# adam-kerrigan/pybader

Measured on AMD Instinct MI355X. Metric: Mvoxels/s neargrid assign+refine on 512^3 grid, higher is better.
Workload: dtype f64; 1 GPU; 512^3 synthetic 8-Gaussian-atom cubic cell (BASELINE config 3), neargrid assign + neargrid edge refinement changed:2, density resident in HBM; method=neargrid, device_driven_slab_step=False, basins=8

## Files before the change

### include/bader_hip.h

```cpp
#ifndef BADER_HIP_H
#define BADER_HIP_H

#include <stdint.h>

#ifdef __cplusplus
extern "C" {
#endif

typedef struct xb_ctx xb_ctx;

enum { XB_OK = 0, XB_E_ARG = -1, XB_E_HIP = -2, XB_E_STATE = -3, XB_E_LIMIT = -4, XB_E_COMM = -5,
       XB_E_SHORT = -6  };

enum { XB_I8 = 1, XB_I16 = 2, XB_I32 = 4, XB_I64 = 8 };

enum { XB_METHOD_ONGRID = 0, XB_METHOD_NEARGRID = 1 };
enum { XB_REFINE_ALL = 0, XB_REFINE_CHANGED = 1 };

const char *xb_last_error(void);
int xb_device_count(void);
int xb_create(int device, xb_ctx **out);
void xb_destroy(xb_ctx *c);
int xb_sync(xb_ctx *c);
void *xb_stream(xb_ctx *c);
// ... 55 lines not shown
int xb_walkers_fetch(xb_ctx *c, int64_t *walkers, int64_t *results);
int xb_walkers_continue(xb_ctx *c, const int64_t *walkers, int64_t n);
int xb_walkers_apply(xb_ctx *c, const int64_t *results, int64_t n, int64_t *changed, int64_t *stuck);
int xb_edge_check(xb_ctx *c, int64_t *checked, int64_t *edges);
int xb_edge_check_local(xb_ctx *c, int64_t *n_out);
int xb_edge_check_local_fetch(xb_ctx *c, int64_t *idx_out, int8_t *cls_out);
int xb_edge_check_global(xb_ctx *c, const int64_t *idx, const int8_t *cls, int64_t n, int64_t *checked, int64_t *edges);
int xb_refine(xb_ctx *c, int mode, int64_t iters, int64_t *log, int64_t log_capacity, int64_t *n_iters);
int xb_assign_refine(xb_ctx *c, int method, int mode, int64_t iters, int64_t *n_maxima, int64_t *log, int64_t log_capacity, int64_t *n_iters);

int xb_charge_sum(xb_ctx *c, double voxel_volume, int64_t n_labels, double *charge, double *volume);
int xb_moment_sum(xb_ctx *c, const double lattice[9], const double *centres_cart, int64_t n, double voxel_volume,
                  double *moments , double *volume );
int xb_adjacency(xb_ctx *c, const int32_t *dirs , int n_dirs, int64_t n, int64_t *n_pairs);
int xb_adjacency_fetch(xb_ctx *c, int32_t *a, int32_t *b, int64_t *facets , double *saddle,
                       int64_t *saddle_facet, int64_t capacity);
int xb_adjacency_release(xb_ctx *c);
int xb_weight_sum(xb_ctx *c, const double alpha[27], double voxel_volume, const double *q_host, int64_t *n_maxima);
int xb_weight_sum_device(xb_ctx *c, const double alpha[27], double voxel_volume, const void *dev_ptr, int dtype,
                         const int64_t stride[3], void *stream, int64_t *n_maxima);
int xb_weight_fetch(xb_ctx *c, int64_t *max_idx, double *charge, double *volume, int64_t capacity);
int xb_weight_stats(xb_ctx *c, int64_t out[7]);
int xb_weight_release(xb_ctx *c);
int xb_volume_assign(xb_ctx *c, const int64_t *swap, int64_t n_swap);
int xb_atom_assign(const double *bader_max_cart, int64_t n_max, const double *atoms_cart, int64_t n_atoms,
                   const double lattice[9], int64_t *atom_out, double *dist_out);

int xb_surface_distance(xb_ctx *c, const double lattice[9], const double *atoms_cart, int64_t n_atoms,
                        double *min_d2, int64_t *edges);
int xb_volume_mask(xb_ctx *c, int64_t vol_num, double *out_host);
int xb_label_sum(xb_ctx *c, int64_t value, double *sum, int64_t *count);

int xb_set_table_window(xb_ctx *c, int64_t margin);
int xb_table_build(xb_ctx *c, int64_t *n_local_seeds);
int xb_table_local_seeds(xb_ctx *c, int64_t *out, int64_t capacity);
int xb_brick_masks(xb_ctx *c, void **dev_ptr, int64_t *n_bricks, int64_t *own_first, int64_t *own_count);
int xb_table_ties(xb_ctx *c, int64_t *has_ties);
int xb_table_finish(xb_ctx *c, const int64_t *seeds, int64_t n_seeds, int64_t any_ties);

void *xb_labels_ptr(xb_ctx *c);
void *xb_known_ptr(xb_ctx *c);
void *xb_density_ptr(xb_ctx *c);
int64_t xb_plane_elems(xb_ctx *c);
int xb_copy_planes(xb_ctx *c, int which , int to_device, void *host, int64_t xa, int64_t xb);
int xb_label_wire(xb_ctx *c, int widen_to, int *wire_out);
int xb_brick_masks_copy(xb_ctx *c, int to_device, int32_t *host, int64_t first, int64_t count);
int xb_set_halo(xb_ctx *c, int64_t halo);

int xb_slab_supported(xb_ctx *c, int nranks, int64_t *ok);
int xb_slab_assign_masks(xb_ctx *c, int rank, int nranks);
int xb_slab_assign_trace(xb_ctx *c);
int xb_slab_assign_finish(xb_ctx *c, int64_t *n_maxima, int64_t *status);
int xb_slab_refine_pass(xb_ctx *c);
int xb_slab_walkers_round(xb_ctx *c, int src, int last);
int xb_slab_walk_layout(xb_ctx *c, int64_t out[5]);
int xb_slab_walk_send(xb_ctx *c, int64_t walkers);
enum {
    XB_XC_EDGES = 0,
    XB_XC_CHANGED = 1,
    XB_XC_ESCAPED = 2,
    XB_XC_TRAVELLING = 3,
    XB_XC_SLOW = 4,
    XB_XC_LOST = 5,
    XB_XC_MINE = 6,
    XB_XC_ROUNDS = 7,
    XB_XC_COUNT = 8
};
int xb_slab_refine_counts(xb_ctx *c, int64_t *local, int64_t *global);
int xb_slab_block(xb_ctx *c, int which, void **dev_ptr, int64_t *bytes_total, int64_t *own_offset, int64_t *own_bytes);
int xb_slab_block_copy(xb_ctx *c, int which, int to_device, void *host, int64_t off, int64_t bytes);
int xb_host_waits(int64_t *n);

int xb_kernel_time(xb_ctx *c, int which, double *ms_total, int64_t *launches);
int xb_kernel_time_reset(xb_ctx *c);
int xb_enable_timing(xb_ctx *c, int on);
int xb_set_option(xb_ctx *c, int key, int value);
int xb_host_alloc(int64_t bytes, void **out);
int xb_host_free(void *p);
int xb_memory_stats(xb_ctx *c, int64_t *bytes_total, int64_t *bytes_table, int64_t *bytes_scratch);
int xb_box_stats(xb_ctx *c, int64_t *n_boxes, int64_t *box_voxels);
int xb_brick_labels(xb_ctx *c, int32_t *out, int64_t capacity, int64_t dims[3]);
int xb_slow_path_stats(xb_ctx *c, int64_t *assign_total, int64_t *refine_total);
int xb_deferred_stats(xb_ctx *c, int64_t *refine_total);
int xb_growth_stats(xb_ctx *c, int64_t *retries, int64_t *kill_launches);

int xb_comm_unique_id(uint8_t id_out[128]);
int xb_comm_init(xb_ctx *c, int rank, int nranks, const uint8_t id_in[128]);
int xb_comm_destroy(xb_ctx *c);
int xb_comm_exchange_planes(xb_ctx *c, int which, int n_send, const int32_t *send_peer, const int64_t *send_xa,
                            const int64_t *send_xb, int n_recv, const int32_t *recv_peer, const int64_t *recv_xa,
                            const int64_t *recv_xb);
int xb_comm_allreduce_i64(xb_ctx *c, int64_t *inout, int64_t n, int op);
int xb_comm_allgather_i64(xb_ctx *c, const int64_t *in, int64_t n, int64_t *out);
int xb_comm_share_brick_masks(xb_ctx *c, const int64_t *first, const int64_t *count);
int xb_comm_allgather_block(xb_ctx *c, int which, const int64_t *first, const int64_t *count);
int xb_comm_allreduce_block(xb_ctx *c);
int xb_comm_info(xb_ctx *c, int64_t out[4]);
int xb_comm_stats(xb_ctx *c, int64_t *bytes_sent);

#ifdef __cplusplus
}
#endif
#endif
```

### pybader_amd/_lib.py

```python
import ctypes as C
import threading
import os

import numpy as np

HERE = os.path.dirname(os.path.abspath(__file__))
LIB_PATH = os.environ.get('XB_LIBRARY') or os.path.join(HERE, 'libbader_hip.so')

METHODS = {'ongrid': 0, 'neargrid': 1}
REFINE_MODES = {'all': 0, 'changed': 1}
DTYPE_CODE = {np.dtype(np.int8): 1, np.dtype(np.int16): 2, np.dtype(np.int32): 4, np.dtype(np.int64): 8}
(XB_XC_EDGES, XB_XC_CHANGED, XB_XC_ESCAPED, XB_XC_TRAVELLING, XB_XC_SLOW, XB_XC_LOST, XB_XC_MINE, XB_XC_ROUNDS,
 XB_XC_COUNT) = range(9)

_vp, _i64, _dbl, _int = C.c_void_p, C.c_int64, C.c_double, C.c_int
_pi64, _pdbl = C.POINTER(C.c_int64), C.POINTER(C.c_double)
SYMBOLS = {
    'xb_last_error': (C.c_char_p, []),
    'xb_device_count': (_int, []),
    'xb_create': (_int, [_int, C.POINTER(_vp)]),
    'xb_destroy': (None, [_vp]),
    'xb_sync': (_int, [_vp]),
    'xb_stream': (_vp, [_vp]),
    'xb_set_grid': (_int, [_vp, _pi64, _pdbl, _pdbl, _i64, _i64]),
# ... 2 lines not shown
    'xb_parse_density_text': (_int, [_vp, _vp, _i64, _dbl, _pi64, _pi64]),
    'xb_parse_cube_text': (_int, [_vp, _vp, _i64, _i64, _i64, _int, _dbl, _pi64, _pi64]),
    'xb_download_density': (_int, [_vp, _vp]),
    'xb_format_begin': (_int, [_vp, _vp, _pi64, _int, _dbl, _int, _int, _vp, _i64, _i64, _pi64]),
    'xb_format_host_values': (_int, [_vp, _vp, _vp]),
    'xb_format_set_host_text': (_int, [_vp, _vp, _vp]),
    'xb_format_next': (_int, [_vp, C.POINTER(_vp), _pi64]),
    'xb_format_times': (_int, [_vp, _pdbl, _pdbl]),
    'xb_format_end': (_int, [_vp]),
    'xb_upload_labels': (_int, [_vp, _vp, _int]),
    'xb_download_labels': (_int, [_vp, _vp, _int]),
    'xb_import_density': (_int, [_vp, _vp, _int, _pi64, _vp]),
    'xb_import_labels': (_int, [_vp, _vp, _int, _vp]),
    'xb_export_labels': (_int, [_vp, _vp, _int, _vp]),
    'xb_export_volume': (_int, [_vp, _i64, _vp, _int, _vp]),
    'xb_device_alloc': (_int, [_int, _i64, C.POINTER(_vp)]),
    'xb_device_free': (_int, [_vp]),
    'xb_device_read': (_int, [_vp, _vp, _vp, _i64, _vp]),
    'xb_upload_known': (_int, [_vp, _vp]),
    'xb_download_known': (_int, [_vp, _vp]),
    'xb_vacuum_assign': (_int, [_vp, _dbl, _dbl, _pdbl, _pdbl]),
    'xb_assign': (_int, [_vp, _int, _pi64]),
    'xb_get_maxima': (_int, [_vp, _vp, _i64]),
    'xb_assign_trace': (_int, [_vp, _int, _pi64]),
    'xb_assign_local_table': (_int, [_vp, _vp, _vp, _i64]),
    'xb_assign_finish': (_int, [_vp, _vp, _i64]),
    'xb_prepare_refine': (_int, [_vp]),
    'xb_edge_find': (_int, [_vp, _pi64]),
    'xb_refine_trace': (_int, [_vp, _pi64, _pi64]),
    'xb_refine_trace_escaped': (_int, [_vp, _pi64, _pi64]),
    'xb_escaped_paths': (_int, [_vp, _i64, _pi64, _pi64]),
    'xb_escaped_paths_fetch': (_int, [_vp, _vp, _vp, _vp, _vp]),
    'xb_gather_voxels': (_int, [_vp, _vp, _i64, _vp, _vp]),
    'xb_scatter_voxels': (_int, [_vp, _vp, _i64, _vp, _vp]),
    'xb_walkers_count': (_int, [_vp, _pi64, _pi64]),
    'xb_walkers_fetch': (_int, [_vp, _vp, _vp]),
    'xb_walkers_continue': (_int, [_vp, _vp, _i64]),
    'xb_walkers_apply': (_int, [_vp, _vp, _i64, _pi64, _pi64]),
    'xb_edge_check': (_int, [_vp, _pi64, _pi64]),
    'xb_edge_check_local': (_int, [_vp, _pi64]),
    'xb_edge_check_local_fetch': (_int, [_vp, _vp, _vp]),
    'xb_edge_check_global': (_int, [_vp, _vp, _vp, _i64, _pi64, _pi64]),
    'xb_refine': (_int, [_vp, _int, _i64, _vp, _i64, _pi64]),
    'xb_assign_refine': (_int, [_vp, _int, _int, _i64, _pi64, _vp, _i64, _pi64]),
    'xb_charge_sum': (_int, [_vp, _dbl, _i64, _vp, _vp]),
    'xb_moment_sum': (_int, [_vp, _pdbl, _pdbl, _i64, _dbl, _pdbl, _pdbl]),
    'xb_adjacency': (_int, [_vp, _vp, _int, _i64, _pi64]),
    'xb_adjacency_fetch': (_int, [_vp, _vp, _vp, _vp, _vp, _vp, _i64]),
    'xb_adjacency_release': (_int, [_vp]),
    'xb_weight_sum': (_int, [_vp, _pdbl, _dbl, _vp, _pi64]),
    'xb_weight_sum_device': (_int, [_vp, _pdbl, _dbl, _vp, _int, _pi64, _vp, _pi64]),
    'xb_weight_fetch': (_int, [_vp, _vp, _vp, _vp, _i64]),
    'xb_weight_stats': (_int, [_vp, _pi64]),
    'xb_weight_release': (_int, [_vp]),
    'xb_volume_assign': (_int, [_vp, _vp, _i64]),
    'xb_atom_assign': (_int, [_vp, _i64, _vp, _i64, _vp, _vp, _vp]),
    'xb_surface_distance': (_int, [_vp, _vp, _vp, _i64, _vp, _pi64]),
    'xb_volume_mask': (_int, [_vp, _i64, _vp]),
    'xb_label_sum': (_int, [_vp, _i64, _pdbl, _pi64]),
    'xb_set_table_window': (_int, [_vp, _i64]),
    'xb_table_build': (_int, [_vp, _pi64]),
    'xb_table_local_seeds': (_int, [_vp, _vp, _i64]),
    'xb_brick_masks': (_int, [_vp, C.POINTER(_vp), _pi64, _pi64, _pi64]),
    'xb_table_ties': (_int, [_vp, _pi64]),
    'xb_table_finish': (_int, [_vp, _vp, _i64, _i64]),
    'xb_labels_ptr': (_vp, [_vp]),
    'xb_known_ptr': (_vp, [_vp]),
    'xb_density_ptr': (_vp, [_vp]),
    'xb_plane_elems': (_i64, [_vp]),
    'xb_copy_planes': (_int, [_vp, _int, _int, _vp, _i64, _i64]),
    'xb_label_wire': (_int, [_vp, _int, _vp]),
    'xb_host_alloc': (_int, [_i64, _vp]),
    'xb_host_free': (_int, [_vp]),
    'xb_brick_masks_copy': (_int, [_vp, _int, _vp, _i64, _i64]),
    'xb_set_halo': (_int, [_vp, _i64]),
    'xb_kernel_time': (_int, [_vp, _int, _pdbl, _pi64]),
    'xb_kernel_time_reset': (_int, [_vp]),
    'xb_enable_timing': (_int, [_vp, _int]),
    'xb_set_option': (_int, [_vp, _int, _int]),
    'xb_box_stats': (_int, [_vp, _pi64, _pi64]),
    'xb_brick_labels': (_int, [_vp, _vp, _i64, _pi64]),
    'xb_slow_path_stats': (_int, [_vp, _pi64, _pi64]),
    'xb_deferred_stats': (_int, [_vp, _pi64]),
    'xb_growth_stats': (_int, [_vp, _pi64, _pi64]),
    'xb_comm_unique_id': (_int, [_vp]),
    'xb_comm_init': (_int, [_vp, _int, _int, _vp]),
    'xb_comm_destroy': (_int, [_vp]),
    'xb_comm_exchange_planes': (_int, [_vp, _int, _int, _vp, _pi64, _pi64, _int, _vp, _pi64, _pi64]),
    'xb_comm_allreduce_i64': (_int, [_vp, _pi64, C.c_int64, _int]),
    'xb_comm_allgather_i64': (_int, [_vp, _pi64, C.c_int64, _pi64]),
    'xb_comm_share_brick_masks': (_int, [_vp, _pi64, _pi64]),
    'xb_comm_allgather_block': (_int, [_vp, _int, _pi64, _pi64]),
    'xb_comm_allreduce_block': (_int, [_vp]),
    'xb_slab_supported': (_int, [_vp, _int, _pi64]),
    'xb_slab_assign_masks': (_int, [_vp, _int, _int]),
    'xb_slab_assign_trace': (_int, [_vp]),
    'xb_slab_assign_finish': (_int, [_vp, _pi64, _pi64]),
    'xb_slab_refine_pass': (_int, [_vp]),
    'xb_slab_walkers_round': (_int, [_vp, _int, _int]),
    'xb_slab_walk_layout': (_int, [_vp, _pi64]),
    'xb_slab_walk_send': (_int, [_vp, _i64]),
    'xb_slab_refine_counts': (_int, [_vp, _pi64, _pi64]),
    'xb_slab_block': (_int, [_vp, _int, C.POINTER(_vp), _pi64, _pi64, _pi64]),
    'xb_slab_block_copy': (_int, [_vp, _int, _int, _vp, _i64, _i64]),
    'xb_host_waits': (_int, [_pi64]),
    'xb_comm_stats': (_int, [_vp, _pi64]),
    'xb_comm_info': (_int, [_vp, _pi64]),
    'xb_memory_stats': (_int, [_vp, _pi64, _pi64, _pi64]),
}

_lib = None


class BaderHipError(RuntimeError):
    code = None


XB_E_ARG = -1
XB_E_STATE = -3
XB_E_LIMIT = -4
XB_E_SHORT = -6


def load():
    global _lib
    if _lib is None:
        if not os.path.exists(LIB_PATH):
            raise BaderHipError(f"{LIB_PATH} is missing: build it with `python -m pybader_amd.build` "
                                "(hipcc, gfx950); pybader_amd has no CPU fallback")
        lib = C.CDLL(LIB_PATH)
        for name, (res, args) in SYMBOLS.items():
            fn = getattr(lib, name)
            fn.restype = res
            fn.argtypes = args
        _lib = lib
    return _lib


_POOL_KEEP = 4
_POOL_MAX_BYTES = 4 << 30


class _PinnedBuf:
    __slots__ = ('ptr', 'nbytes', '__weakref__')

    def __init__(self, ptr, nbytes):
        self.ptr, self.nbytes = ptr, nbytes

    @property
    def __array_interface__(self):
        return {'shape': (self.nbytes,), 'typestr': '|u1', 'data': (self.ptr, False), 'version': 3}


_pool = {}
_pool_bytes = 0
_pool_lock = threading.Lock()


def _host_free(ptr):
    if _lib is not None:
        _lib.xb_host_free(C.c_void_p(ptr))


def _pool_evict(need):
    global _pool_bytes
    for size in list(_pool):
# ... 658 lines not shown
    def slab_refine_counts(self):
        loc, glo = np.zeros(XB_XC_COUNT, np.int64), np.zeros(XB_XC_COUNT, np.int64)
        check(self.lib.xb_slab_refine_counts(self.h, loc.ctypes.data_as(_pi64), glo.ctypes.data_as(_pi64)))
        return loc, glo

    def slab_block(self, which):
        p, a, b, d = _vp(), C.c_int64(0), C.c_int64(0), C.c_int64(0)
        check(self.lib.xb_slab_block(self.h, int(which), C.byref(p), C.byref(a), C.byref(b), C.byref(d)))
        return int(p.value or 0), int(a.value), int(b.value), int(d.value)

    def slab_block_copy(self, which, host, off, to_device):
        assert host.dtype == np.uint8 and host.flags.c_contiguous
        check(self.lib.xb_slab_block_copy(self.h, int(which), 1 if to_device else 0, _ptr(host), int(off), host.nbytes))

    def comm_allgather_block(self, which, first, count):
        f, n = np.array(first, np.int64), np.array(count, np.int64)
        check(self.lib.xb_comm_allgather_block(self.h, int(which), f.ctypes.data_as(_pi64), n.ctypes.data_as(_pi64)))

    def comm_allreduce_block(self):
        check(self.lib.xb_comm_allreduce_block(self.h))

    def host_waits(self):
        a = C.c_int64(0)
        check(self.lib.xb_host_waits(C.byref(a)))
        return int(a.value)

    def memory_stats(self):
        a, b, d = C.c_int64(0), C.c_int64(0), C.c_int64(0)
        check(self.lib.xb_memory_stats(self.h, C.byref(a), C.byref(b), C.byref(d)))
        return int(a.value), int(b.value), int(d.value)

    def comm_info(self):
        out = (C.c_int64 * 4)()
        check(self.lib.xb_comm_info(self.h, out))
        return {'nccl_comm_count': int(out[0]), 'nccl_user_rank': int(out[1]), 'nccl_device': int(out[2]), 'rccl_version': int(out[3])}

    def comm_bytes_sent(self):
        n = C.c_int64(0)
        check(self.lib.xb_comm_stats(self.h, C.byref(n)))
        return int(n.value)

    def enable_timing(self, on=True, only=None):
        mask = int(bool(on)) if only is None else sum(2 << int(k) for k in only)
        check(self.lib.xb_enable_timing(self.h, mask))

    def kernel_time(self, which):
        ms, n = C.c_double(), C.c_int64()
        check(self.lib.xb_kernel_time(self.h, int(which), C.byref(ms), C.byref(n)))
        return ms.value, n.value

    def kernel_time_reset(self):
        check(self.lib.xb_kernel_time_reset(self.h))

    def set_option(self, key, value):
        check(self.lib.xb_set_option(self.h, int(key), int(value)))

    def box_stats(self):
        a, b = C.c_int64(), C.c_int64()
        check(self.lib.xb_box_stats(self.h, C.byref(a), C.byref(b)))
        return a.value, b.value

    def brick_labels(self):
        dims = (C.c_int64 * 3)()
        check(self.lib.xb_brick_labels(self.h, None, 0, dims))
        out = np.zeros(tuple(int(d) for d in dims), np.int32)
        check(self.lib.xb_brick_labels(self.h, _ptr(out), out.size, dims))
        return out

    def slow_path_stats(self):
        a, b = C.c_int64(), C.c_int64()
        check(self.lib.xb_slow_path_stats(self.h, C.byref(a), C.byref(b)))
        return a.value, b.value

    def growth_stats(self):
        a, b = C.c_int64(), C.c_int64()
        check(self.lib.xb_growth_stats(self.h, C.byref(a), C.byref(b)))
        return a.value, b.value

    def deferred_stats(self):
        a = C.c_int64()
        check(self.lib.xb_deferred_stats(self.h, C.byref(a)))
        return a.value

    def sync(self):
        check(self.lib.xb_sync(self.h))


def atom_assign(bader_max_cart, atoms_cart, lattice):
    lib = load()
    bm, at, lat = _f64(bader_max_cart).reshape(-1, 3), _f64(atoms_cart).reshape(-1, 3), _f64(lattice).reshape(9)
    a, d = np.zeros(bm.shape[0], np.int64), np.zeros(bm.shape[0], np.float64)
    check(lib.xb_atom_assign(_ptr(bm), bm.shape[0], _ptr(at), at.shape[0], _ptr(lat), _ptr(a), _ptr(d)))
    return a, d


_default_ctx = {}


def default_context(device=None):
    if device is None:
        device = int(os.environ.get('PYBADER_AMD_DEVICE', os.environ.get('LOCAL_RANK', '0')))
        if load().xb_device_count() == 1:
            device = 0
    if device not in _default_ctx:
        _default_ctx[device] = Context(device)
    return _default_ctx[device]
```

### pybader_amd/csrc/bader_hip.hip

```cpp
#include "bader_kernels.h"
#include "../../include/bader_hip.h"

#include <algorithm>
#include <cmath>
#include <cstdarg>
#include <cstdio>
#include <cstring>
#include <string>
#include <thread>
#include <vector>

static thread_local long long xb_waits = 0;
static inline hipError_t xb_counted_sync(hipStream_t s) { xb_waits++; return (hipStreamSynchronize)(s); }
#define hipStreamSynchronize(s) xb_counted_sync(s)

#include "k_common.h"
#include "k_masks.h"
#include "k_fused.h"
#include "k_trace.h"
#include "k_ongrid.h"
#include "k_edges.h"
#include "k_sums.h"
#include "k_text.h"
#include "k_format.h"
// ... 25 lines not shown
    long long launches = 0;
};

namespace xbcomm { struct State; }
struct xb_ctx {
    int device = 0;
    xbcomm::State *comm = nullptr;
    struct FmtState *fmt = nullptr;
    hipStream_t stream = nullptr;
    Grid g{};
    bool has_grid = false;
    long long N = 0;
    int halo = 0;
    double *rho = nullptr;
    GradRec *grad = nullptr;
    long long grad_cap = 0;
    long long list_cap = 0;
    int *ec_buf = nullptr;
    long long ec_buf_cap = 0;
    double *dist_dev = nullptr;
    int *boxbuf = nullptr;
    int *box_max_tab = nullptr;
    int n_boxes = 0;
    long long box_voxels = 0;
    int opt_boxes = 1;
    int opt_bricks = 1;
    int opt_dbg = 0;
    int opt_ec_groups = 256;
    int opt_ec_share = 1;
    int *ec_share = nullptr;
    int opt_ec_qcap = EC_Q;
    std::vector<int64_t> esc_starts, esc_offsets, esc_vox;
    unsigned long long *ec_pend = nullptr;
    int8_t *ec_pflag = nullptr;
    std::vector<int8_t> esc_complete;
    bool has_vacuum = true;
    bool vac_by_tol = false;
    double vac_tol = 0.;
    bool regions_pending = false;
    bool buni_valid = false;
    bool buni_halo_safe = false;
    bool regions_neargrid = false;
    bool regions_labels = false;
    int n_walk = 0;
    int *walk = nullptr;
    int table_margin = -1;
    bool table_prebuilt = false;
    int table_stage = 0;
    std::vector<int> window_seeds;
    bool window_ties = true;
    bool slab_sparse = false;
    int ec_local_n = 0;
    int walk_n_out = 0;
    void *walk_out_dev = nullptr;
    std::vector<int64_t> walk_host, res_host;
    int walk_n_res = 0;
    void *walk_in = nullptr, *walk_out2 = nullptr, *walk_res = nullptr;
    long long walk_cap = 0;
    long long stat_deferred = 0;
    long long stat_ovf_assign = 0, stat_ovf_refine = 0;
    int *bres_last = nullptr;
    int *blab = nullptr;
    int nbk[3] = {0, 0, 0};
    bool grad_valid = false;
    bool brick_max_valid = false;
    int grad_cover = 0;
    unsigned char *brick_rec = nullptr;
    void *xbuf = nullptr;
    int slab_rank = 0, slab_nranks = 0, slab_stage = 0;
    void *wbuf[2] = {nullptr, nullptr};
    void *wk_in = nullptr;
    int wbuf_ranks = 0, walk_last = -1, walk_round = 0, wcap = 0;
    int walk_send = 0;
    int opt_async_comm = 0;
    int opt_tile_dilate = 1;
    int opt_self_exchange = 0;
    int opt_mask_diag = 1;
    int opt_narrow_halo = 1;
    int grow_kill_launches = 6;
    long long stat_grow_retries = 0;
    bool defer_wait = false;
    bool pending_assign = false;
    int64_t pending_n_maxima = 0;
    int opt_lean = 1;
    int opt_mirror = 1;
    int grad_rule = 0;
    int *labels = nullptr;
    int8_t *known = nullptr;
    int *first = nullptr;
    int *list = nullptr;
    int8_t *st = nullptr;
    void *stage = nullptr;
    size_t stage_bytes = 0;
    int *max_list = nullptr;
    int *max_aux = nullptr;
    int max_cap = 0;
    int *ovf_list = nullptr;
    int ovf_cap = 0;
    int *counters = nullptr;
    int *fs = nullptr;
    int *blab_buf = nullptr;
    long long blab_alloc = 0;
    bool labels_zero_pending = false;
    int zero_outside[3] = {-1, -1, -1};
    static constexpr int trace_waves = 8192;
    unsigned long long *counters64 = nullptr;
    double *dsum = nullptr;
    int *host_ints = nullptr;
    char *big_pin[2] = {nullptr, nullptr};
    hipEvent_t big_ev[2] = {nullptr, nullptr};
    hipEvent_t io_ev = nullptr;
    int opt_io_tiled = 1;
    char *pin = nullptr;
    size_t pin_bytes = 0;
    std::vector<int> maxima_sorted;
    int label_wire = 4;
    std::vector<int> local_max, local_first;
    bool first_clean = false;
    int chg_n = -1;
    int list_n = 0;
    bool list_valid = false;
    unsigned timing = 0;
    TimedKernel tk[10];
    long long n_alloc = 0;
    bool thin = false;
    double *w_A = nullptr, *w_V = nullptr, *w_S = nullptr;
    unsigned char *w_pending = nullptr;
    int *w_list[2] = {nullptr, nullptr};
    int *w_state = nullptr;
    long long w_cap = 0;
    long long w_stat[6] = {0, 0, 0, 0, 0, 0};
    bool w_have = false;
    bool w_ignore_labels = false;
    std::vector<int64_t> w_idx;
    std::vector<double> w_charge, w_volume;
    double *m_buf = nullptr;
    size_t m_cap = 0;
    unsigned long long *aj_buf = nullptr;
    size_t aj_bytes = 0;
    bool aj_have = false;
    int aj_dirs = 0;
    std::vector<int32_t> aj_a, aj_b;
    std::vector<int64_t> aj_facets, aj_sfacet;
    std::vector<double> aj_saddle;
    bool have_rho = false, have_labels = false;
};

static inline int label_wire_for(long long n) { return 2 * n <= 255 ? 1 : (2 * n <= 65535 ? 2 : 4); }
static inline int labels_fit_wire(const int32_t *lab, long long n) {
    int32_t lo = 0, hi = 0;
    for (long long i = 0; i < n; i++) { lo = std::min(lo, lab[i]); hi = std::max(hi, lab[i]); }
    return (lo >= -128 && hi <= 127) ? 1 : ((lo >= -32768 && hi <= 32767) ? 2 : 4);
}
static inline unsigned nblocks(long long n) { return (unsigned)((n + TPB - 1) / TPB); }
static GridL light(const Grid &g) {
    GridL l;
    l.nx = g.nx; l.ny = g.ny; l.nz = g.nz; l.nyz = g.nyz;
    l.x0 = g.x0; l.x1 = g.x1; l.vx0 = g.vx0; l.vlen = g.vlen;
    l.wx0 = g.wx0; l.wlen = g.wlen; l.wbase = g.wbase; l.ntot = g.ntot;
    l.use24 = ((long long)g.nx * g.ny < (1 << 24)) && g.nz < (1 << 24);
    l.main_ties = g.main_ties;
    return l;
}

template <typename T>
struct DevBuf {
// ... 11 lines not shown
    s.main_ties = g.main_ties;
    for (int k = 0; k < 9; k++) s.T[k] = g.T[k];
    auto at = [&](int idx) {
        const int ix = idx / 9, iy = (idx / 3) % 3, iz = idx % 3;
        return g.dist[((ix + 2) % 3) * 9 + ((iy + 2) % 3) * 3 + ((iz + 2) % 3)];
    };
    for (int idx = 0; idx <= 13; idx++) {
        const double a = at(idx), b = at(26 - idx);
        if (std::memcmp(&a, &b, sizeof a) != 0) return false;
        s.dsym[idx] = a;
    }
    return true;
}

static void mirror_prefilter(const Grid &g, int &mirror, double &mu_scale) {
    mirror = 0;
    double dmin = 0.;
    bool first = true;
    for (int i = 0; i < 27; i++)
        if (i != 0) { dmin = first ? g.dist[i] : std::min(dmin, g.dist[i]); first = false; }
    if (!(dmin > 0.) || !std::isfinite(dmin)) { mu_scale = 0.; return; }
    for (int ax = 0; ax < 3; ax++) {
        bool ok = true;
        for (int u = 0; u < 3 && ok; u++)
            for (int v = 0; v < 3 && ok; v++) {
                int ip[3], im[3];
                ip[ax] = 1; im[ax] = 2;
                ip[(ax + 1) % 3] = im[(ax + 1) % 3] = u;
                ip[(ax + 2) % 3] = im[(ax + 2) % 3] = v;
                const double a = g.dist[ip[0] * 9 + ip[1] * 3 + ip[2]], b = g.dist[im[0] * 9 + im[1] * 3 + im[2]];
                ok = std::memcmp(&a, &b, sizeof a) == 0;
            }
        if (ok) mirror |= 1 << ax;
    }
    mu_scale = std::ldexp(1. + 1. / dmin, -48);
}

struct ScopedTimer {
    xb_ctx *c;
    int which;
    hipEvent_t a = nullptr, b = nullptr;
    ScopedTimer(xb_ctx *c_, int w) : c(c_), which(w) {
        if ((c->timing >> which) & 1u) {
            hipEventCreate(&a);
            hipEventCreate(&b);
            hipEventRecord(a, c->stream);
        }
    }
    ~ScopedTimer() {
        if ((c->timing >> which) & 1u) {
            hipEventRecord(b, c->stream);
            c->tk[which].pending.push_back({a, b});
        }
    }
};

extern "C" {

const char *xb_last_error(void) { return g_err.c_str(); }

#include "host_context.h"
#include "host_stages.h"
#include "host_format.h"
#include "host_assign.h"
#include "host_refine.h"
#include "host_sums.h"
#include "host_slab_table.h"
#include "host_interop.h"
#include "host_weight.h"
#include "host_moments.h"
#include "host_adjacency.h"

int xb_set_option(xb_ctx *c, int key, int value) {
    if (!c) return fail(XB_E_ARG, "null ctx");
    if (key == 1) { c->opt_boxes = value & 1; c->opt_bricks = (value >> 1) & 1; }
    else if (key == 2) {
        c->opt_mirror = !(value & 1);
        c->opt_lean = !(value & 2);
        c->opt_mask_diag = !(value & 4);
        c->opt_tile_dilate = !(value & 8);
        c->opt_narrow_halo = !(value & 16);
        c->opt_ec_share = !(value & 32);
        c->opt_io_tiled = !(value & 64);
    }
    else if (key == 3) c->opt_dbg = value;
    else if (key == 4 && value >= 1 && value <= 4096) c->opt_ec_groups = value;
    else if (key == 5 && value >= 2 && value <= EC_Q) c->opt_ec_qcap = value;
    else if (key == 6) { c->grad_valid = false; if (value == 2) c->brick_max_valid = false; }
    else if (key == 17 && value >= 1) c->grow_kill_launches = value;
    else if (key == 19) c->opt_self_exchange = value != 0;
    else if (key == 24) c->opt_async_comm = value != 0;
    else if (key == 30) c->w_ignore_labels = value != 0;
    else return fail(XB_E_ARG, "xb_set_option: unknown key %d", key);
    return XB_OK;
}
int xb_growth_stats(xb_ctx *c, int64_t *retries, int64_t *kill_launches) {
    if (!c) return fail(XB_E_ARG, "null ctx");
    if (retries) *retries = c->stat_grow_retries;
    if (kill_launches) *kill_launches = c->grow_kill_launches;
    return XB_OK;
}
int xb_deferred_stats(xb_ctx *c, int64_t *refine_total) {
    if (!c) return fail(XB_E_ARG, "null ctx");
    if (refine_total) *refine_total = c->stat_deferred;
    return XB_OK;
}
int xb_slow_path_stats(xb_ctx *c, int64_t *assign_total, int64_t *refine_total) {
    if (!c) return fail(XB_E_ARG, "null ctx");
    if (assign_total) *assign_total = c->stat_ovf_assign;
    if (refine_total) *refine_total = c->stat_ovf_refine;
    return XB_OK;
}
int xb_memory_stats(xb_ctx *c, int64_t *bytes_total, int64_t *bytes_table, int64_t *bytes_scratch) {
    if (!c || !c->has_grid) return fail(XB_E_STATE, "xb_memory_stats: no grid");
    const long long N = c->N;
    const long long table = c->grad_cap * (long long)sizeof(GradRec);
    const long long scratch = c->list_cap * 4 + (long long)c->stage_bytes + c->ec_buf_cap * 4 + (c->ec_pend ? 8 * N + 16 : 0) +
                              (c->w_cap ? 25 * c->w_cap + (c->w_S ? 8 * c->w_cap : 0) : 0)  +
                              (long long)c->m_cap * 8  +
                              (long long)c->aj_bytes ;
    const long long fixed = 8 * N  + 4 * N  + (N + 16)  + 4 * N  + N  +
                            2LL * c->max_cap * 4 + (long long)c->ovf_cap * 4 + c->blab_alloc * 5 + (long long)c->walk_cap * 3 * 80 +
                            (1 << 22) ;
    if (bytes_total) *bytes_total = fixed + table + scratch;
    if (bytes_table) *bytes_table = table;
    if (bytes_scratch) *bytes_scratch = scratch;
    return XB_OK;
}
int xb_box_stats(xb_ctx *c, int64_t *n_boxes, int64_t *box_voxels) {
    if (!c) return fail(XB_E_ARG, "null ctx");
    if (n_boxes) *n_boxes = c->n_boxes;
    if (box_voxels) *box_voxels = c->box_voxels;
    return XB_OK;
}
int xb_brick_labels(xb_ctx *c, int32_t *out, int64_t capacity, int64_t dims[3]) {
    if (!c || !c->has_grid) return fail(XB_E_STATE, "xb_brick_labels: no grid");
    if (!c->blab) return fail(XB_E_STATE, "xb_brick_labels: no trapping regions on this context (no neargrid assignment yet)");
    const int64_t nbr = (int64_t)c->nbk[0] * c->nbk[1] * c->nbk[2];
    if (dims) { dims[0] = c->nbk[0]; dims[1] = c->nbk[1]; dims[2] = c->nbk[2]; }
    if (!out) return XB_OK;
    if (capacity < nbr) return fail(XB_E_ARG, "xb_brick_labels: capacity too small");
    HIPCHK(hipSetDevice(c->device));
    HIPCHK(hipMemcpyAsync(out, c->blab, nbr * sizeof(int), hipMemcpyDeviceToHost, c->stream));
    HIPCHK(hipStreamSynchronize(c->stream));
    return XB_OK;
}
#ifdef XB_DEBUG_COUNT
int xb_debug_steps(xb_ctx *c, int on, signed char *host_out) {
    static signed char *buf = nullptr;
    if (host_out && buf) {
        if (hipMemcpy(host_out, buf, (size_t)c->N, hipMemcpyDeviceToHost) != hipSuccess) return XB_E_HIP;
    }
    if (on && !buf && hipMalloc(&buf, (size_t)c->N) != hipSuccess) return XB_E_HIP;
    if (on && hipMemset(buf, 0, (size_t)c->N) != hipSuccess) return XB_E_HIP;
    signed char *p = on ? buf : nullptr;
    return hipMemcpyToSymbol(HIP_SYMBOL(xb_dbg_steps), &p, sizeof p) == hipSuccess ? XB_OK : XB_E_HIP;
}
int xb_debug_counts(unsigned long long *out, int reset) {
    hipDeviceSynchronize();
    if (out && hipMemcpyFromSymbol(out, HIP_SYMBOL(xb_dbg), sizeof(unsigned long long) * 65536) != hipSuccess) return XB_E_HIP;
    if (reset) {
        static unsigned long long z[65536];
        if (hipMemcpyToSymbol(HIP_SYMBOL(xb_dbg), z, sizeof z) != hipSuccess) return XB_E_HIP;
    }
    return XB_OK;
}
#endif
int xb_enable_timing(xb_ctx *c, int on) {
    if (!c) return fail(XB_E_ARG, "null ctx");
    c->timing = on == 0 ? 0u : (on == 1 ? 0xFFFFu : ((unsigned)on >> 1));
    return XB_OK;
}
int xb_kernel_time_reset(xb_ctx *c) {
    if (!c) return fail(XB_E_ARG, "null ctx");
    HIPCHK(hipSetDevice(c->device));
    HIPCHK(hipStreamSynchronize(c->stream));
    for (auto &t : c->tk) {
        for (auto &p : t.pending) { hipEventDestroy(p.first); hipEventDestroy(p.second); }
        t.pending.clear();
        t.ms = 0.;
        t.launches = 0;
    }
    return XB_OK;
}
int xb_kernel_time(xb_ctx *c, int which, double *ms_total, int64_t *launches) {
    if (!c || which < 0 || which > 9) return fail(XB_E_ARG, "xb_kernel_time: bad argument");
    HIPCHK(hipSetDevice(c->device));
// ... 21 lines not shown
```

### pybader_amd/csrc/host_assign.h

```cpp

static GridL light(const Grid &g);

static int ensure_brick_bytes(xb_ctx *c, int nbr) {
    if (c->blab_alloc < nbr) {
        hipFree(c->blab_buf); c->blab_buf = nullptr; c->blab_alloc = 0; c->brick_rec = nullptr; c->brick_max_valid = false;
        if (c->grad_cover) { c->grad_cover = 0; c->grad_valid = false; }
        HIPCHK(hipMalloc(&c->blab_buf, (size_t)nbr * sizeof(int) + (size_t)nbr + 16));
        c->blab_alloc = nbr;
        c->brick_rec = reinterpret_cast<unsigned char *>(c->blab_buf + nbr);
    }
    return XB_OK;
}

static int ensure_grad(xb_ctx *c, bool force, bool boxes, bool main_rule) {
    if (int rc = need_grad(c)) return rc;
    c->g.main_ties = main_rule ? 1 : 0;
    if (c->grad_valid && !force && (c->grad_rule == 2 || c->grad_rule == (main_rule ? 1 : 0))) return XB_OK;
    const Grid &g = c->g;
    if (c->grad_valid && !force && !boxes && c->grad_cover == 1 && c->brick_rec) {
        const int nb1r = (g.ny + BRK - 1) / BRK, nb2r = (g.nz + BRK - 1) / BRK, nbr = ((g.nx + BRK - 1) / BRK) * nb1r * nb2r;
        ScopedTimer t(c, 4);
        launch_brick_records(c, nullptr, nullptr, nbr, nb1r, nb2r);
        HIPCHK(hipGetLastError());
        c->grad_rule = main_rule ? 1 : 0;
// ... 331 lines not shown
    c->buni_valid = false; c->regions_labels = false;
    const bool regions = c->regions_pending && c->blab;
    int buni = BUNI_NONE;
    if (regions && g.x1 - g.x0 == g.nx)
        buni = BUNI_SCAN;
    else if (regions && !c->has_vacuum && g.nx % 8 == 0 && g.ny % 8 == 0 && g.nz % 8 == 0 && g.x0 % 8 == 0 && g.x1 % 8 == 0)
        buni = BUNI_MIXED;
    launch_relabel(c, nullptr, (int)n_global, regions, c->box_max_tab ? c->box_max_tab : c->boxbuf + BB_REGMAX, buni, nullptr);
    HIPCHK(hipGetLastError());
    if (buni != BUNI_NONE) {
        c->buni_valid = true;
        c->buni_halo_safe = buni == BUNI_MIXED;
    }
    c->regions_labels = regions && !c->has_vacuum && c->regions_neargrid;
    c->regions_pending = false;
    HIPCHK(hipStreamSynchronize(c->stream));
    c->first_clean = true;
    return XB_OK;
}


static bool fused_ok(const xb_ctx *c) {
    const Grid &g = c->g;
    return c->opt_boxes && c->opt_bricks && g.x0 == 0 && g.x1 == g.nx && !table_windowed(c) &&
           g.nx >= 16 && g.ny >= 16 && g.nz >= 16;
}
static int assign_neargrid_tail(xb_ctx *c, int64_t *n_maxima);

static int fused_numbering_launch(xb_ctx *c) {
    k_number_maxima<<<1, 1024, 0, c->stream>>>(c->fs, c->first, c->max_list, c->max_cap, c->max_aux, c->fs + FS_TOTAL);
    launch_relabel(c, c->fs, 0, c->regions_pending, c->box_max_tab, BUNI_SCAN, c->bres_last);
    HIPCHK(hipGetLastError());
    return XB_OK;
}
static int number_maxima_big(xb_ctx *c, int nmax) {
    const long long n_words = (c->N + 31) / 32, n_blocks = (n_words + 1023) / 1024;
    const size_t need = (size_t)(2 * n_words + n_blocks) * sizeof(int);
    DevBuf<int> own;
    int *scratch = (int *)c->stage;
    if (!c->stage || c->stage_bytes < need) {
        HIPCHK(own.alloc((size_t)(2 * n_words + n_blocks)));
        scratch = own.p;
    }
    unsigned *bits = reinterpret_cast<unsigned *>(scratch);
    int *wprefix = scratch + n_words, *bsum = scratch + 2 * n_words;
    HIPCHK(hipMemsetAsync(bits, 0, (size_t)n_words * sizeof(int), c->stream));
    k_rank_mark<<<(nmax + 255) / 256, 256, 0, c->stream>>>(c->first, c->max_list, nmax, bits);
    k_rank_scan<<<(unsigned)n_blocks, 1024, 0, c->stream>>>(bits, (int)n_words, wprefix, bsum);
    k_rank_blocks<<<1, 1024, 0, c->stream>>>(bsum, (int)n_blocks);
    k_rank_assign<<<(nmax + 255) / 256, 256, 0, c->stream>>>(c->first, c->max_list, nmax, bits, wprefix, bsum, c->max_aux, c->fs);
    HIPCHK(hipGetLastError());
    launch_relabel(c, c->fs, 0, c->regions_pending, c->box_max_tab, BUNI_SCAN, c->bres_last);
    HIPCHK(hipGetLastError());
    c->maxima_sorted.resize(nmax);
    HIPCHK(hipMemcpyAsync(c->maxima_sorted.data(), c->max_aux, (size_t)nmax * sizeof(int), hipMemcpyDeviceToHost, c->stream));
    HIPCHK(hipStreamSynchronize(c->stream));
    return XB_OK;
}

static int assign_neargrid_fused(xb_ctx *c, int64_t *n_maxima) {
    if (int rc = need_grad(c)) return rc;
    Grid &g = c->g;
    const int nb0 = (g.nx + BRK - 1) / BRK, nb1 = (g.ny + BRK - 1) / BRK, nb2 = (g.nz + BRK - 1) / BRK, nbr = nb0 * nb1 * nb2;
    const bool part = g.nx % BRK || g.ny % BRK || g.nz % BRK;
    if (int rc = ensure_brick_bytes(c, nbr)) return rc;
    int *fs = c->fs;
    int *seed = c->list, *bmask = c->list + nbr, *buf0 = c->list + 2 * nbr, *buf1 = c->list + 3 * nbr, *walk = c->list + 4 * nbr;
    int *box_max = c->boxbuf + BB_REGMAX, *box_first = c->boxbuf + BB_REGFIRST;
    int *bmaxv = walk;
    int *bpot = c->list + 5 * nbr;
    int *bres = nullptr;
    c->box_max_tab = box_max;
    auto stage_done = [&](const char *what) {
        if (c->opt_dbg & 32) {
            const hipError_t e = (hipStreamSynchronize)(c->stream);
            int h16[16] = {0};
            (void)hipMemcpy(h16, fs, sizeof h16, hipMemcpyDeviceToHost);
            fprintf(stderr, "[assign] %s: %s  seeds %d regions %d certain %d walk %d maxima %d ovf %d err %d\n", what, hipGetErrorString(e), h16[FS_N_SEEDS],
                    h16[FS_N_BOXES], h16[FS_N_CERTAIN], h16[FS_N_WALK], h16[FS_N_MAX], h16[FS_N_OVF], h16[FS_ERR]);
            fflush(stderr);
        }
    };
    if (int rc = begin_assignment(c, fs, FS_TOTAL, true)) return rc;
    g.main_ties = 1;
    const GridL gl = light(g);
    {
        ScopedTimer t4(c, 4);
        {
            ScopedTimer t5(c, 5);
            launch_brick_masks(c, part, true, bmask, bmaxv, bpot);
        }
        stage_done("brick masks");
        c->grad_valid = true;
        c->grad_rule = 1;
        c->grad_cover = 1;
        launch_region_growth(c, nb0, nb1, nb2, bmask, bmaxv, bpot, seed, buf0, buf1, box_max, box_first, true);
        HIPCHK(hipGetLastError());
        stage_done("region growth");
    }
    c->blab = c->blab_buf;
    c->regions_neargrid = true;
    c->walk = walk;
    c->nbk[0] = nb0; c->nbk[1] = nb1; c->nbk[2] = nb2;
    const long long own = c->N;
    {
        ScopedTimer t0(c, 0);
        {
            int bits = 0;
            while ((1 << bits) < std::max(std::max(nb0, nb1), nb2)) bits++;
            const unsigned n_codes = 1u << (3 * bits);
            const bool vac = c->has_vacuum && c->vac_by_tol;
            k_brick_walk_list_morton<<<(n_codes + 16 * TPB - 1) / (16 * TPB), TPB, 0, c->stream>>>(nb0, nb1, nb2, n_codes, c->blab, walk,
                                                                                                  fs + FS_N_WALK, fs + FS_GROW_RETRY,
                                                                                                  vac ? bpot : nullptr, c->vac_tol);
        }
        {
            ScopedTimer t7(c, 7);
            launch_brick_records(c, walk, fs + FS_N_WALK, nbr, nb1, nb2);
        }
        stage_done("walk list + records");
        if (c->has_vacuum)
            k_fill_certain<<<nblocks(own), TPB, 0, c->stream>>>(gl, c->blab, nb1, nb2, box_max, c->labels, c->first, c->max_list,
                                                                fs + FS_N_MAX, c->max_cap, fs + FS_GROW_RETRY);
        else {
            k_note_regions<<<1, XB_BOXES_MAX, 0, c->stream>>>(gl, nb1, nb2, fs, box_first, box_max, c->first, c->max_list, fs + FS_N_MAX, c->max_cap);
            c->regions_pending = true;
        }
        {
            ScopedTimer t6(c, 6);
            int *bres_buf = c->has_vacuum ? nullptr : c->list + 6 * nbr;
            if (launch_persistent_trace(c, true, part, box_max, walk, c->has_vacuum ? 1 : 0, bres_buf)) bres = bres_buf;
        }
        HIPCHK(hipGetLastError());
        stage_done("trace");
    }
    c->bres_last = bres;
    if (int rc = fused_numbering_launch(c)) return rc;
    stage_done("numbering + relabel");
    HIPCHK(hipMemcpyAsync(c->host_ints, fs, (FS_TOTAL + XB_SORT_MAX) * sizeof(int), hipMemcpyDeviceToHost, c->stream));
    if (c->defer_wait) {
        g.main_ties = 0;
        c->grad_rule = 2;
        c->regions_pending = false;
        c->buni_valid = !c->has_vacuum;
        c->regions_labels = !c->has_vacuum;
        c->pending_assign = true;
        return XB_OK;
    }
    HIPCHK(hipStreamSynchronize(c->stream));
    return assign_neargrid_tail(c, n_maxima);
}

static int assign_neargrid_tail(xb_ctx *c, int64_t *n_maxima) {
    Grid &g = c->g;
    int *fs = c->fs;
    const int nb1 = c->nbk[1], nb2 = c->nbk[2];
    int *walk = c->walk, *box_max = c->box_max_tab;
    const int *h = c->host_ints;
    g.main_ties = 0;
    const GridL gl = light(g);
    if (h[FS_GROW_RETRY]) {
        c->grow_kill_launches = 1 << 20;
        c->stat_grow_retries++;
        c->grad_valid = false;
        return assign_neargrid_fused(c, n_maxima);
    }
    if (h[FS_TIES] == 0) c->grad_rule = 2;
    c->n_boxes = h[FS_N_BOXES];
    c->box_voxels = (long long)h[FS_N_CERTAIN] * BRK * BRK * BRK;
    c->n_walk = h[FS_N_WALK];
    const int novf = h[FS_N_OVF];
    int nmax = h[FS_N_MAX];
    if (nmax > c->max_cap) return fail(XB_E_LIMIT, "%d maxima exceed the table capacity %d", nmax, c->max_cap);
    c->stat_ovf_assign += novf;
    const int *sorted = h[FS_SORT_OK] && novf == 0 ? h + FS_TOTAL : nullptr;
    if (novf > 0) {
        g.main_ties = 1;
        const GridL glt = light(g);
        const int maxsteps = trace_maxsteps(g);
        int *list2 = (int *)c->stage;
        const int cap2 = (int)std::min<size_t>(c->stage_bytes / sizeof(int), 0x7fffffffu);
        auto two_tiers = [&](int n_listed) -> int {
            c->host_ints[HI_UPLOAD] = n_listed;
            HIPCHK(hipMemcpyAsync(c->counters + CT_MID_LISTED, c->host_ints + HI_UPLOAD, sizeof(int), hipMemcpyHostToDevice, c->stream));
            HIPCHK(hipMemsetAsync(c->counters + CT_MID_LEFT, 0, sizeof(int), c->stream));
            k_ng_trace_list<XB_MID_K><<<512, TPB, 0, c->stream>>>(glt, c->grad, box_max, c->blab, nb1, nb2, c->ovf_list, c->counters + CT_MID_LISTED, c->labels, c->first,
                                                          c->max_list, fs + FS_N_MAX, c->max_cap, list2, c->counters + CT_MID_LEFT, cap2, maxsteps, c->rho, c->dist_dev,
                                                          c->has_vacuum ? 1 : 0);
            HIPCHK(hipGetLastError());
            if (c->opt_dbg & 4) {
                int m2 = 0;
                if (int rc2 = read_counter(c, CT_MID_LEFT, &m2)) return rc2;
                fprintf(stderr, "[assign] %d walkers listed, %d left for the exact slow kernel after the %d-voxel window\n", n_listed, m2, XB_MID_K);
            }
            if (n_listed > cap2) return fail(XB_E_LIMIT, "%d walkers for the exact slow path exceed its list (%d)", n_listed, cap2);
            return run_slow(c, n_listed, 0, fs + FS_N_MAX, nullptr, nullptr, list2, c->counters + CT_MID_LEFT, true);
        };
        int rc = two_tiers(std::min(novf, c->ovf_cap));
        for (int left = novf - c->ovf_cap; !rc && left > 0;) {
            HIPCHK(hipMemsetAsync(c->counters + CT_N_OVF, 0, sizeof(int), c->stream));
            k_list_unfinished<<<4096, TPB, 0, c->stream>>>(gl, walk, fs + FS_N_WALK, nb1, nb2, c->labels, c->ovf_list, c->counters + CT_N_OVF, c->ovf_cap);
            HIPCHK(hipGetLastError());
            int m = 0;
            if ((rc = read_counter(c, CT_N_OVF, &m))) break;
            if (m == 0) break;
            rc = two_tiers(std::min(m, c->ovf_cap));
            left = m - c->ovf_cap;
        }
        g.main_ties = 0;
        if (rc) return rc;
        HIPCHK(hipMemsetAsync(fs + FS_N_OVF, 0, sizeof(int), c->stream));
        if (int rc2 = fused_numbering_launch(c)) return rc2;
        HIPCHK(hipMemcpyAsync(c->host_ints, fs, (FS_TOTAL + XB_SORT_MAX) * sizeof(int), hipMemcpyDeviceToHost, c->stream));
        HIPCHK(hipStreamSynchronize(c->stream));
        nmax = h[FS_N_MAX];
        if (nmax > c->max_cap) return fail(XB_E_LIMIT, "%d maxima exceed the table capacity %d", nmax, c->max_cap);
        if (h[FS_SORT_OK]) sorted = h + FS_TOTAL;
    }
    if (!sorted) {
        if (int rc = number_maxima_big(c, nmax)) return rc;
    }
    numbering_done(c, sorted, nmax, n_maxima);
    c->buni_valid = !c->has_vacuum;
    c->regions_labels = !c->has_vacuum;
    return XB_OK;
}


static bool assign_neargrid_complete(xb_ctx *c, int64_t *n_maxima) {
    c->pending_assign = false;
    const int *h = c->host_ints;
    const int nmax = h[FS_N_MAX];
    if (h[FS_GROW_RETRY] || h[FS_TIES] != 0 || h[FS_N_OVF] != 0 || !h[FS_SORT_OK] || nmax > c->max_cap || nmax > XB_SORT_MAX) return false;
    c->n_boxes = h[FS_N_BOXES];
    c->box_voxels = (long long)h[FS_N_CERTAIN] * BRK * BRK * BRK;
    c->n_walk = h[FS_N_WALK];
    numbering_done(c, h + FS_TOTAL, nmax, n_maxima);
// ... 131 lines not shown
```

### pybader_amd/csrc/host_context.h

```cpp

int xb_device_count(void) {
    int n = 0;
    if (hipGetDeviceCount(&n) != hipSuccess) return 0;
    return n;
}

int xb_create(int device, xb_ctx **out) {
    if (!out) return fail(XB_E_ARG, "xb_create: null out");
    int n = 0;
    hipError_t e = hipGetDeviceCount(&n);
    if (e != hipSuccess || n <= 0)
        return fail(XB_E_HIP, "xb_create: no HIP device visible (%s); libbader_hip has no CPU fallback",
                    e == hipSuccess ? "device count 0" : hipGetErrorString(e));
    if (device < 0 || device >= n) return fail(XB_E_ARG, "xb_create: device %d out of range [0,%d)", device, n);
    HIPCHK(hipSetDevice(device));
    xb_ctx *c = new xb_ctx();
    c->device = device;
    HIPCHK(hipStreamCreate(&c->stream));
    HIPCHK(hipMalloc(&c->counters, (1024 + XB_SORT_MAX) * sizeof(int)));
    c->fs = c->counters + CT_FS;
    HIPCHK(hipMalloc(&c->counters64, 16 * sizeof(unsigned long long)));
    HIPCHK(hipMalloc(&c->dsum, 16 * sizeof(double)));
    HIPCHK(hipMalloc(&c->dist_dev, 36 * sizeof(double)));
    HIPCHK(hipMalloc(&c->boxbuf, (size_t)(1 << 20) * sizeof(int)));
    HIPCHK(hipHostMalloc(&c->host_ints, HI_TOTAL * sizeof(int)));
    *out = c;
    return XB_OK;
}

static void weight_free(xb_ctx *c);
static void moments_free(xb_ctx *c);
static void adjacency_free(xb_ctx *c);
static void free_grid(xb_ctx *c) {
    weight_free(c);
    moments_free(c);
    adjacency_free(c);
    c->have_rho = c->have_labels = false;
    hipFree(c->rho); hipFree(c->grad); hipFree(c->labels); hipFree(c->known); hipFree(c->first); hipFree(c->list);
    hipFree(c->st); hipFree(c->stage); hipFree(c->ec_pend); c->ec_pend = nullptr; hipFree(c->ec_share); c->ec_share = nullptr; hipFree(c->ec_pflag); c->ec_pflag = nullptr; hipFree(c->max_list); hipFree(c->max_aux); hipFree(c->ovf_list);
    hipFree(c->blab_buf); c->blab_buf = nullptr; c->blab_alloc = 0; c->labels_zero_pending = false;
    hipFree(c->ec_buf); c->ec_buf = nullptr; c->ec_buf_cap = 0; c->grad_cap = 0; c->list_cap = 0;
    c->brick_rec = nullptr; c->grad_cover = 0;
    c->rho = nullptr; c->grad = nullptr; c->grad_valid = false; c->brick_max_valid = false; c->labels = nullptr; c->known = nullptr; c->first = nullptr; c->list = nullptr;
    c->st = nullptr; c->stage = nullptr; c->max_list = nullptr; c->max_aux = nullptr; c->ovf_list = nullptr;
    c->n_alloc = 0; c->stage_bytes = 0;
}

int xb_comm_destroy(xb_ctx *c);
static void fmt_release(xb_ctx *c);
void xb_destroy(xb_ctx *c) {
    if (!c) return;
    hipSetDevice(c->device);
    hipStreamSynchronize(c->stream);
    xb_comm_destroy(c);
    fmt_release(c);
    for (auto &t : c->tk)
        for (auto &p : t.pending) { hipEventDestroy(p.first); hipEventDestroy(p.second); }
    free_grid(c);
    hipFree(c->counters); hipFree(c->counters64); hipFree(c->dsum); hipFree(c->dist_dev); hipFree(c->boxbuf);
    hipFree(c->walk_in); hipFree(c->walk_out2); hipFree(c->walk_res); hipFree(c->xbuf); hipFree(c->wbuf[0]); hipFree(c->wbuf[1]); hipFree(c->wk_in);
    hipHostFree(c->host_ints);
    hipHostFree(c->pin);
    for (int k = 0; k < 2; k++) { hipHostFree(c->big_pin[k]); if (c->big_ev[k]) hipEventDestroy(c->big_ev[k]); }
    if (c->io_ev) hipEventDestroy(c->io_ev);
    hipStreamDestroy(c->stream);
    delete c;
}

int xb_sync(xb_ctx *c) {
    HIPCHK(hipSetDevice(c->device));
    HIPCHK(hipStreamSynchronize(c->stream));
    return XB_OK;
}
void *xb_stream(xb_ctx *c) { return (void *)c->stream; }

#define XB_SYNTH_ATOMS_MAX 4096
#define XB_SURFACE_ATOMS_MAX 100000
#define XB_STAGE_FLOOR ((size_t)4 << 20)
static_assert((16 + 5 * (size_t)XB_SYNTH_ATOMS_MAX) * sizeof(double) <= XB_STAGE_FLOOR &&
              (16 + 4 * (size_t)XB_SURFACE_ATOMS_MAX) * sizeof(double) <= XB_STAGE_FLOOR, "stage floor below a documented atom maximum");
static int need_scratch(xb_ctx *c) {
    const Grid &g = c->g;
    const long long N = c->N ? c->N : (long long)g.nx * g.nyz;
    const int own = g.x1 - g.x0;
    long long planes = own + 2LL * (std::max(c->halo, 16) + 16);
    if (own == g.nx || planes >= g.nx) planes = g.nx;
    const long long list_want = planes == g.nx ? N : std::max<long long>(planes * g.nyz, 8 * (N / 512) + 4096);
    const size_t stage_want = planes == g.nx ? std::max<size_t>((size_t)N * 8, XB_STAGE_FLOOR) : std::max<size_t>((size_t)planes * g.nyz * 8, (size_t)64 << 20);
    if (c->list_cap < list_want) {
        HIPCHK(hipStreamSynchronize(c->stream));
        hipFree(c->list); c->list = nullptr; c->list_cap = 0;
        HIPCHK(hipMalloc(&c->list, (size_t)list_want * sizeof(int)));
        c->list_cap = list_want;
        c->list_valid = false; c->chg_n = -1; c->walk = nullptr; c->n_walk = 0;
    }
    if (c->stage_bytes < stage_want) {
        HIPCHK(hipStreamSynchronize(c->stream));
        hipFree(c->stage); c->stage = nullptr; c->stage_bytes = 0;
        HIPCHK(hipMalloc(&c->stage, stage_want));
        c->stage_bytes = stage_want;
    }
    return XB_OK;
// ... 475 lines not shown
```

### pybader_amd/csrc/host_refine.h

```cpp

static void plane_range(const Grid &g, int ext, int &xa, int &np) {
    const int own = g.x1 - g.x0;
    if (own + 2 * ext >= g.nx) { xa = 0; np = g.nx; }
    else { xa = ((g.x0 - ext) % g.nx + g.nx) % g.nx; np = own + 2 * ext; }
}

static int preset_known_planes(xb_ctx *c, int p0, int np) {
    const Grid &g = c->g;
    const int run1 = std::min(np, g.nx - p0);
    HIPCHK(hipMemsetAsync(c->known + (size_t)p0 * g.nyz, 2, (size_t)run1 * g.nyz, c->stream));
    if (np > run1) HIPCHK(hipMemsetAsync(c->known, 2, (size_t)(np - run1) * g.nyz, c->stream));
    return XB_OK;
}
static int *launch_brick_uniformity(xb_ctx *c, const GridL &gl, int b_off, int count, unsigned scan_grid) {
    const Grid &g = c->g;
    const int nb0 = (g.nx + 7) / 8, nb1 = (g.ny + 7) / 8, nb2 = (g.nz + 7) / 8, nbr = nb0 * nb1 * nb2;
    int *buni = reinterpret_cast<int *>(c->st);
    if (!c->buni_valid)
        k_label_uniform_list<<<scan_grid, TPB, 0, c->stream>>>(gl, c->labels, nb1, nb2, nullptr, count, nullptr, nullptr, buni, b_off, nbr);
    k_buni3<<<(nbr + 255) / 256, 256, 0, c->stream>>>(nb0, nb1, nb2, buni, buni + nbr);
    return buni + nbr;
}

static int edge_find_launch(xb_ctx *c, bool *dilate_owned) {
// ... 496 lines not shown
    const int chg_n = c->chg_n;
    c->list_valid = false; c->chg_n = -1;
    c->buni_valid = false;
    if (g.x1 - g.x0 != g.nx) return fail(XB_E_STATE, "xb_edge_check: one slab only; slabs use xb_edge_check_local + xb_edge_check_global");
    int n = 0;
    bool listed = false;
    if (chg_n >= 0) {
        n = chg_n;
        if (n) {
            HIPCHK(hipMemcpyAsync(c->list, (int *)c->stage + c->N, (size_t)n * sizeof(int), hipMemcpyDeviceToDevice, c->stream));
            HIPCHK(hipMemcpyAsync(c->host_ints + HI_EC_CHGLIST, c->fs + FS_N_CHGLIST, sizeof(int), hipMemcpyDeviceToHost, c->stream));
            listed = true;
        }
    } else if (int rc = compact(c, -2, &n)) return rc;
    if (int rc = edge_check_resolve(c, n, nullptr, 0, g.nx, 0, c->N, checked, edges)) return rc;
    if (listed && c->host_ints[HI_EC_CHGLIST] != n) return fail(XB_E_STATE, "xb_edge_check: %d voxels listed for %d relabelled ones", c->host_ints[HI_EC_CHGLIST], n);
    return XB_OK;
}

int xb_edge_check_local(xb_ctx *c, int64_t *n_out) {
    NEED_GRID("xb_edge_check_local");
    c->list_valid = false; c->chg_n = -1;
    int n = 0;
    if (int rc = compact(c, -2, &n)) return rc;
    if (n) {
        k_ec_class<<<nblocks(n), TPB, 0, c->stream>>>(c->g, c->rho, c->labels, c->list, n, c->st);
        HIPCHK(hipGetLastError());
    }
    c->ec_local_n = n;
    if (n_out) *n_out = n;
    return XB_OK;
}
int xb_edge_check_local_fetch(xb_ctx *c, int64_t *idx_out, int8_t *cls_out) {
    NEED_GRID("xb_edge_check_local_fetch");
    const int n = c->ec_local_n;
    if (!n) return XB_OK;
    std::vector<int> tmp(n);
    HIPCHK(hipMemcpyAsync(tmp.data(), c->list, n * sizeof(int), hipMemcpyDeviceToHost, c->stream));
    HIPCHK(hipMemcpyAsync(cls_out, c->st, n, hipMemcpyDeviceToHost, c->stream));
    HIPCHK(hipStreamSynchronize(c->stream));
    for (int i = 0; i < n; i++) idx_out[i] = tmp[i];
    return XB_OK;
}
int xb_edge_check_global(xb_ctx *c, const int64_t *idx, const int8_t *cls, int64_t n, int64_t *checked, int64_t *edges) {
    NEED_GRID("xb_edge_check_global");
    const Grid &g = c->g;
    c->list_valid = false; c->chg_n = -1;
    c->buni_valid = false;
    if (checked) *checked = 0;
    if (edges) *edges = 0;
    if (n < 0 || n > c->N) return fail(XB_E_ARG, "xb_edge_check_global: bad list length");
    if (c->halo < 3 && g.vlen < g.nx) return fail(XB_E_STATE, "xb_edge_check_global: needs a halo of at least 3 planes");
    if (!n) return XB_OK;
    std::vector<int> i32(n);
    for (int64_t k = 0; k < n; k++) {
        if (idx[k] < 0 || idx[k] >= c->N) return fail(XB_E_ARG, "xb_edge_check_global: voxel index out of range");
        i32[k] = (int)idx[k];
    }
    if (g.vlen < g.nx)
        if (int rc = preset_known_planes(c, (g.vx0 + g.vlen) % g.nx, g.nx - g.vlen)) return rc;
    int8_t *dcls = c->st + (c->N - n);
    if (2 * n > c->N || 2 * n > c->list_cap) return fail(XB_E_LIMIT, "xb_edge_check_global: list longer than half the grid / the list buffer");
    if (int rc = upload_pinned(c, c->list, i32.data(), n * sizeof(int))) return rc;
    if (int rc = upload_pinned(c, dcls, cls, n, (n * sizeof(int) + 255) & ~(size_t)255)) return rc;
    k_scatter_byte<<<(unsigned)((n + 255) / 256), 256, 0, c->stream>>>(c->known, c->list, (int)n, (int8_t)-2);
    HIPCHK(hipGetLastError());
    int near_xa = 0, near_np = g.nx;
    if (g.vlen + 4 < g.nx) { near_xa = (g.vx0 - 2 + g.nx) % g.nx; near_np = g.vlen + 4; }
    const int rc = edge_check_resolve(c, (int)n, dcls, near_xa, near_np, (long long)g.x0 * g.nyz, (long long)g.x1 * g.nyz, checked, edges);
    return rc;
}

int xb_prepare_refine(xb_ctx *c) {
    NEED_GRID("xb_prepare_refine");
    return ensure_grad(c, false, false, false);
}

#define XB_STEP_REDO 1000
static int refine_iteration_fused(xb_ctx *c, int64_t *edges, int64_t *changed, bool late_records = false) {
    const Grid &g = c->g;
    int *fs = c->fs;
    c->g.main_ties = 0;
    const GridL gl = light(g);
    static_assert(FS_N_CHGLIST == FS_N_EDGES + 6, "one memset clears the refinement's counters");
    HIPCHK(hipMemsetAsync(fs + FS_N_EDGES, 0, 7 * sizeof(int), c->stream));
    c->chg_n = -1;
    {
        ScopedTimer t(c, 2);
        const int small = small_grid(g);
        int *buni = nullptr;
        int ntiles_listed = 0;
        if (g.nx >= 16 && g.ny >= 16 && g.nz >= 16)
            buni = launch_brick_uniformity(c, gl, 0, ((g.nx + 7) / 8) * ((g.ny + 7) / 8) * ((g.nz + 7) / 8), 4096);
        const unsigned char *brec = (c->grad_valid && c->grad_cover == 1) || late_records ? c->brick_rec : nullptr;
        if (buni) {
            const int ntiles = ((g.nz + ET_Z - 1) / ET_Z) * ((g.ny + ET_Y - 1) / ET_Y) * ((g.nx + ET_X - 1) / ET_X);
            ntiles_listed = ntiles;
            int *tiles = (int *)c->stage;
            HIPCHK(hipMemsetAsync(c->known, 2, (size_t)c->N, c->stream));
            k_edge_tile_list<<<(ntiles + TPB - 1) / TPB, TPB, 0, c->stream>>>(gl, buni, tiles, fs + FS_N_TILES, 0, (g.nx + ET_X - 1) / ET_X,
                                                                              c->pending_assign ? fs : nullptr);
            k_edge_flag_listed<<<std::min(ntiles, 2048), TPB, 0, c->stream>>>(gl, c->rho, c->labels, c->known, c->list, fs + FS_N_EDGES, small,
                                                           c->grad_valid ? c->grad : nullptr, brec, c->has_vacuum ? 0 : 1, tiles, fs + FS_N_TILES);
        } else {
            dim3 grid((g.nz + ET_Z - 1) / ET_Z, (g.ny + ET_Y - 1) / ET_Y, (g.nx + ET_X - 1) / ET_X);
            k_edge_flag_tiled<<<grid, TPB, 0, c->stream>>>(gl, c->rho, c->labels, c->known, 0, g.nx, c->list, fs + FS_N_EDGES, small, buni,
                                                           c->grad_valid ? c->grad : nullptr, brec, c->has_vacuum ? 0 : 1);
        }
        if (buni && c->opt_tile_dilate && g.nz % ET_Z == 0) k_edge_dilate_tiles<<<std::min(ntiles_listed, 4096), TPB, 0, c->stream>>>(gl, c->known, (const int *)c->stage, fs + FS_N_TILES);
        else k_edge_dilate_list<<<nblocks(c->N / 16), TPB, 0, c->stream>>>(gl, c->known, c->list, 0, fs + FS_N_EDGES);
    }
    c->list_valid = false; c->chg_n = -1;
    c->buni_valid = false;
    if (late_records) {
        if (int rc = need_grad(c)) return rc;
        ScopedTimer t(c, 4);
        const int nb0 = (g.nx + 7) / 8, nb1 = (g.ny + 7) / 8, nb2 = (g.nz + 7) / 8, nbr = nb0 * nb1 * nb2;
        unsigned char *band = reinterpret_cast<unsigned char *>(c->blab_buf);
        HIPCHK(hipMemsetAsync(band, 0, (size_t)nbr, c->stream));
        k_flag_band_bricks<<<4096, TPB, 0, c->stream>>>(gl, c->known, (const int *)c->stage, fs + FS_N_TILES, band);
        k_rec_set_bit0<<<(nbr + 255) / 256, 256, 0, c->stream>>>(nbr, c->brick_rec, band);
        launch_brick_records(c, nullptr, nullptr, nbr, nb1, nb2);
        HIPCHK(hipGetLastError());
        c->grad_valid = true;
        c->grad_cover = 1;
        c->grad_rule = 0;
        c->regions_labels = false;
        c->blab = nullptr;
        c->table_stage = 0;
    }
    const unsigned char *brec = c->grad_cover == 1 ? c->brick_rec : nullptr;
    const int regions_ok = c->grad_cover == 1 && c->regions_labels && !c->has_vacuum ? 1 : 0;
    {
        ScopedTimer t(c, 3);
        int *defer = (int *)c->stage;
        WalkerIO wl{};
        constexpr int XB_RT_BLOCK = 128;
        launch_refine_trace<2, false>(c, (unsigned)((c->N / 16 + XB_RT_BLOCK - 1) / XB_RT_BLOCK), XB_RT_BLOCK, c->list, 0, fs + FS_N_EDGES,
                                      fs + FS_CHANGED, fs + FS_ESCAPED, c->ovf_list, fs + FS_R_OVF, c->ovf_cap, brec, defer, fs + FS_R_DEFER,
                                      regions_ok, nullptr, wl);
        if (c->grad_cover == 1 && !regions_ok)
            launch_refine_trace<2, true>(c, 512, TPB, (int *)c->stage, 0, fs + FS_R_DEFER, fs + FS_CHANGED, fs + FS_ESCAPED, c->ovf_list,
                                         fs + FS_R_OVF, c->ovf_cap, c->brick_rec, nullptr, nullptr, 0, nullptr, wl);
    }
    HIPCHK(hipGetLastError());
    int *hr = c->host_ints + HI_REFINE;
    HIPCHK(hipMemcpyAsync(hr, fs + FS_N_EDGES, 7 * sizeof(int), hipMemcpyDeviceToHost, c->stream));
    HIPCHK(hipStreamSynchronize(c->stream));
    if (c->pending_assign && !assign_neargrid_complete(c, &c->pending_n_maxima)) return XB_STEP_REDO;
    *edges = hr[0];
    *changed = hr[1];
    const int novf = hr[3];
    if (novf == 0 && hr[1] > 0 && c->stage_bytes >= 8 * (size_t)c->N && hr[1] <= (int)std::min<long long>(c->N, 0x7fffffffLL)) {
        k_list_changed<<<1024, TPB, 0, c->stream>>>(c->list, fs + FS_N_EDGES, c->known, (int *)c->stage + c->N, fs + FS_N_CHGLIST,
                                                    (int)std::min<long long>(c->N, 0x7fffffffLL), fs + FS_CHANGED);
        HIPCHK(hipGetLastError());
        c->chg_n = hr[1];
    } else if (novf == 0 && hr[1] == 0)
        c->chg_n = 0;
    c->stat_deferred += hr[4];
    if (hr[2]) return fail(XB_E_STATE, "xb_refine: %d traces left the grid", hr[2]);
    if (novf > c->ovf_cap) return fail(XB_E_LIMIT, "%d retraces need the slow path (cap %d)", novf, c->ovf_cap);
    c->stat_ovf_refine += novf;
    if (novf > 0) {
        const int *slow_list = nullptr, *slow_n_dev = nullptr;
        const int n_slow = novf;
        const bool can_defer = c->grad_cover == 1 && !regions_ok;
        if (!can_defer && c->stage_bytes >= sizeof(int) * (size_t)novf) {
            int *list2 = (int *)c->stage;
            HIPCHK(hipMemsetAsync(c->counters + CT_MID_LEFT, 0, sizeof(int), c->stream));
            launch_refine_trace<XB_MID_K, false>(c, nblocks(novf), TPB, c->ovf_list, novf, nullptr, fs + FS_CHANGED, fs + FS_ESCAPED, list2,
                                                 c->counters + CT_MID_LEFT, novf, brec, nullptr, nullptr, regions_ok, nullptr, WalkerIO{});
            HIPCHK(hipGetLastError());
            slow_list = list2;
            slow_n_dev = c->counters + CT_MID_LEFT;
            if (c->opt_dbg & 4) {
                int m2 = 0;
                if (int rc = read_counter(c, CT_MID_LEFT, &m2)) return rc;
                fprintf(stderr, "[refine] %d retraces listed, %d left for the exact slow kernel after the %d-voxel window\n", novf, m2, XB_MID_K);
            }
        }
        if (int rc = run_slow(c, n_slow, 1, nullptr, fs + FS_CHANGED, fs + FS_ESCAPED, slow_list, slow_n_dev, true)) return rc;
        HIPCHK(hipMemcpyAsync(hr, fs + FS_CHANGED, sizeof(int), hipMemcpyDeviceToHost, c->stream));
        HIPCHK(hipStreamSynchronize(c->stream));
        *changed = hr[0];
    }
    return XB_OK;
}

static int refine_impl(xb_ctx *c, int mode, int64_t iters, int64_t *log, int64_t log_capacity, int64_t *n_iters);
int xb_refine(xb_ctx *c, int mode, int64_t iters, int64_t *log, int64_t log_capacity, int64_t *n_iters) {
    const int rc = refine_impl(c, mode, iters, log, log_capacity, n_iters);
    if (c) c->chg_n = -1;
    return rc;
}
static int refine_impl(xb_ctx *c, int mode, int64_t iters, int64_t *log, int64_t log_capacity, int64_t *n_iters) {
    NEED_GRID("xb_refine");
    if (n_iters) *n_iters = 0;
    if (iters == 0) return XB_OK;
    int64_t edges = 0, changed = 0, esc = 0, checked = 0;
    const bool fused = c->g.x0 == 0 && c->g.x1 == c->g.nx && !table_windowed(c);
    const bool late = fused && !c->grad_valid && c->brick_max_valid && !c->has_vacuum && c->brick_rec && c->g.nx >= 16 && c->g.ny >= 16 && c->g.nz >= 16;
    if (!late)
        if (int rc = xb_prepare_refine(c)) return rc;
    int64_t k = 0;
    auto put = [&](int64_t e, int64_t ch) {
        if (log && 2 * k + 1 < log_capacity) { log[2 * k] = e; log[2 * k + 1] = ch; }
        k++;
        if (n_iters) *n_iters = k;
    };
    if (fused) {
        if (int rc = refine_iteration_fused(c, &edges, &changed, late)) return rc;
        if (edges == 0) return XB_OK;
    } else {
        if (int rc = xb_edge_find(c, &edges)) return rc;
        if (edges == 0) return XB_OK;
        if (int rc = xb_refine_trace(c, &changed, &esc)) return rc;
        if (esc) return fail(XB_E_STATE, "xb_refine: %lld traces left the valid slab", (long long)esc);
    }
    put(edges, changed);
    for (int64_t it = 2; iters < 0 || it <= iters; it++) {
        if (fused && mode != XB_REFINE_ALL && changed == 0) {
            put(0, 0);
            break;
        }
        if (fused && mode == XB_REFINE_ALL) {
            if (int rc = refine_iteration_fused(c, &edges, &changed)) return rc;
            put(edges, changed);
            if (changed == 0) break;
            continue;
        }
        if (mode == XB_REFINE_ALL) {
            if (int rc = xb_edge_find(c, &edges)) return rc;
        } else {
            if (int rc = xb_edge_check(c, &checked, &edges)) return rc;
        }
        if (int rc = xb_refine_trace(c, &changed, &esc)) return rc;
        if (esc) return fail(XB_E_STATE, "xb_refine: %lld traces left the valid slab", (long long)esc);
        put(edges, changed);
        if (changed == 0) break;
    }
    return XB_OK;
}

int xb_assign_refine(xb_ctx *c, int method, int mode, int64_t iters, int64_t *n_maxima, int64_t *log, int64_t log_capacity, int64_t *n_iters) {
    NEED_GRID_RAW("xb_assign_refine");
    c->have_labels = true;
    if (n_iters) *n_iters = 0;
    const bool fused = c->g.x0 == 0 && c->g.x1 == c->g.nx && !table_windowed(c);
    if (method == XB_METHOD_NEARGRID && fused && fused_ok(c) && !c->has_vacuum && iters != 0 && (mode == XB_REFINE_ALL || mode == XB_REFINE_CHANGED)) {
        c->labels_zero_pending = false;
        c->defer_wait = true;
        int rc = assign_neargrid_fused(c, nullptr);
        c->defer_wait = false;
        if (rc) { c->pending_assign = false; return rc; }
        rc = refine_impl(c, mode, iters, log, log_capacity, n_iters);
        c->chg_n = -1;
        const bool redo = rc == XB_STEP_REDO || c->pending_assign;
        const bool arrived = rc == XB_STEP_REDO;
        c->pending_assign = false;
        if (!redo) {
            if (n_maxima) *n_maxima = c->pending_n_maxima;
            return rc;
        }
        if (n_iters) *n_iters = 0;
        if (arrived) {
            c->grad_rule = 1;
            c->buni_valid = false; c->regions_labels = false;
            c->regions_pending = true;
            c->list_valid = false;
            if (int rc2 = assign_neargrid_tail(c, n_maxima)) return rc2;
            return xb_refine(c, mode, iters, log, log_capacity, n_iters);
        }
        c->grad_valid = false;
        c->first_clean = false;
        c->buni_valid = false; c->regions_labels = false;
        if (n_iters) *n_iters = 0;
    }
    if (int rc = xb_assign(c, method, n_maxima)) return rc;
    return xb_refine(c, mode, iters, log, log_capacity, n_iters);
}
```

### pybader_amd/csrc/host_stages.h

```cpp

enum { BB_TOTAL = 1 << 20, BB_REGMAX = 1 << 16, BB_REGFIRST = 1 << 17 };

static bool table_windowed(const xb_ctx *c) { return c->g.wlen < c->g.nx; }
static int small_grid(const Grid &g) { return g.nx < 16 || g.ny < 16 || g.nz < 80; }
static int trace_maxsteps(const Grid &g) { return 8 * (g.nx + g.ny + g.nz) + 64; }
static const int *slab_regions_of(const xb_ctx *c) {
    const Grid &g = c->g;
    return (table_windowed(c) && c->blab && c->regions_labels && !c->has_vacuum && (c->grad_rule == 2 || c->slab_sparse) &&
            g.nx % 8 == 0 && g.ny % 8 == 0 && g.nz % 8 == 0) ? c->blab : nullptr;
}

static_assert(CT_REDO == CT_N_MAX + 15, "a host-driven assignment zeroes CT_N_MAX .. CT_REDO at once");
static int begin_assignment(xb_ctx *c, int *counts, int n, bool invalidate) {
    HIPCHK(hipMemsetAsync(counts, 0, n * sizeof(int), c->stream));
    if (!c->first_clean) {
        k_fill<int><<<4096, TPB, 0, c->stream>>>(c->first, XB_INT_MAX, c->N);
        HIPCHK(hipGetLastError());
    }
    c->first_clean = false;
    c->regions_pending = false;
    if (invalidate) {
        c->buni_valid = false; c->regions_labels = false;
        c->list_valid = false; c->chg_n = -1;
    }
    return XB_OK;
}

static void launch_brick_masks(xb_ctx *c, bool part, bool allow_diag, int *bmask, int *bmaxv, int *bpot) {
    const Grid &g = c->g;
    const dim3 grid((g.nz + GT_Z - 1) / GT_Z, (g.ny + GT_Y - 1) / GT_Y, (g.x1 - g.x0 + GT_X - 1) / GT_X);
    GridS gs;
    const bool sym = sym_grid(g, gs);
    int mirror = 0;
    double mu_scale = 0.;
    if (sym && c->opt_mirror) mirror_prefilter(g, mirror, mu_scale);
    const bool diag = allow_diag && c->opt_mask_diag && g.T[1] == 0. && g.T[2] == 0. && g.T[3] == 0. && g.T[5] == 0. && g.T[6] == 0. && g.T[7] == 0.;
    auto launch = [&](auto kernel, const auto &gt) {
        kernel<<<grid, TPB, 0, c->stream>>>(gt, c->rho, small_grid(g), bmask, bmaxv, c->fs + FS_TIES, g.x0, mu_scale, mirror, bpot);
    };
    if (!sym) launch(part ? k_brick_masks<Grid, 1, false, true> : k_brick_masks<Grid, 1, false>, g);
    else if (part) launch(diag ? k_brick_masks<GridS, 1, true, true> : k_brick_masks<GridS, 1, false, true>, gs);
    else launch(diag ? k_brick_masks<GridS, 1, true> : k_brick_masks<GridS, 1, false>, gs);
}

static void launch_brick_records(xb_ctx *c, const int *list, const int *n_dev, int nbr, int nb1, int nb2) {
    const Grid &g = c->g;
    auto launch = [&](auto kernel, const auto &gt) {
        kernel<<<4096, TPB, 0, c->stream>>>(gt, c->rho, c->grad, list, n_dev, nbr, nb1, nb2, c->brick_rec, small_grid(g));
    };
    GridS gs;
    if (sym_grid(g, gs)) launch(k_brick_records<GridS>, gs);
    else launch(k_brick_records<Grid>, g);
}

static void launch_region_growth(xb_ctx *c, int nb0, int nb1, int nb2, int *bmask, int *bmaxv, int *bpot, int *seed, int *buf0,
                                 int *buf1, int *box_max, int *box_first, bool chase) {
    const int nbr = nb0 * nb1 * nb2;
    int *fs = c->fs;
    k_seed_bricks<<<(nbr + 255) / 256, 256, 0, c->stream>>>(nbr, bmask, bmaxv, fs, seed, buf0, box_max, box_first);
    if (chase) {
        k_grow_parent<<<(nbr + TPB - 1) / TPB, TPB, 0, c->stream>>>(nb0, nb1, nb2, bmask, bpot, seed, buf1);
        k_grow_chase<<<(nbr + TPB - 1) / TPB, TPB, 0, c->stream>>>(nbr, buf1, seed, buf0, 4 * (nb0 + nb1 + nb2) + 64, fs);
    } else
        k_seed_finish<<<1, 1, 0, c->stream>>>(fs);
    const int long_schedule = 2 * ((std::max(std::max(nb0, nb1), nb2) + BG - 1) / BG) + 12;
    const int launches = chase ? std::min(long_schedule, c->grow_kill_launches) : long_schedule;
    const dim3 ggrid((nb2 + BG - 1) / BG, (nb1 + BG - 1) / BG, (nb0 + BG - 1) / BG);
    for (int l = 0; l < launches; l++)
        k_brick_grow_dev<<<ggrid, BG * BG * BG, 0, c->stream>>>(nb0, nb1, nb2, bmask, seed, buf0, buf1, fs, BG, 0);
    k_grow_finish<<<64, TPB, 0, c->stream>>>(nbr, seed, buf0, buf1, fs, c->blab_buf, box_first, bmask, c->brick_rec, 0, chase && launches < long_schedule ? 1 : 0);
}

static void launch_window_bricks(xb_ctx *c, int *list, int *count, const int *skip) {
    const Grid &g = c->g;
    const int nb0 = c->nbk[0], per_plane = c->nbk[1] * c->nbk[2], nbr = nb0 * per_plane;
    const int w0 = g.wx0 / BRK, wn = g.wlen / BRK, run1 = std::min(wn, nb0 - w0);
    const unsigned grid = (nbr + 16 * TPB - 1) / (16 * TPB);
    k_brick_walk_list<<<grid, TPB, 0, c->stream>>>(nbr, w0 * per_plane, (w0 + run1) * per_plane, c->blab, list, count, skip);
    if (wn > run1) k_brick_walk_list<<<grid, TPB, 0, c->stream>>>(nbr, 0, (wn - run1) * per_plane, c->blab, list, count, skip);
}

static bool launch_persistent_trace(xb_ctx *c, bool lean_ok, bool part, const int *box_max, const int *walk, int has_vacuum, int *bres) {
    const Grid &g = c->g;
    const int groups = std::max(1, c->trace_waves / XB_TRACE_WAVES);
    const int lean = lean_ok && light(g).use24 && c->opt_lean ? ((long long)g.wlen * g.nyz <= (1LL << 27) ? 4 : 3) : 0;
    const bool window = table_windowed(c);
    int *ovf = window ? (int *)c->stage : c->ovf_list;
    const int ovf_cap = window ? (int)std::min<size_t>(c->stage_bytes / sizeof(int), 0x7fffffffu) : c->ovf_cap;
    auto kernel = !lean ? k_ng_trace_g<2, 0>
                : window ? (lean == 4 ? k_ng_trace_g<2, 4, true> : k_ng_trace_g<2, 3, true>)
                : part ? (lean == 4 ? k_ng_trace_g<2, 4, false, true> : k_ng_trace_g<2, 3, false, true>)
                : (lean == 4 ? k_ng_trace_g<2, 4> : k_ng_trace_g<2, 3>);
    kernel<<<groups, XB_WAVE * XB_TRACE_WAVES, 0, c->stream>>>(light(g), c->grad, box_max, c->blab, c->nbk[1], c->nbk[2], walk, c->fs, c->labels,
                                                               c->first, c->max_list, c->max_cap, ovf, ovf_cap, trace_maxsteps(g), has_vacuum,
                                                               8, 1, lean ? bres : nullptr);
    if (window)
        k_ng_trace_list<2><<<512, TPB, 0, c->stream>>>(light(g), c->grad, box_max, c->blab, c->nbk[1], c->nbk[2], ovf, c->fs + FS_N_OVF, c->labels,
                                                       c->first, c->max_list, c->fs + FS_N_MAX, c->max_cap, c->ovf_list, c->counters + CT_N_OVF,
                                                       c->ovf_cap, trace_maxsteps(g), c->rho, c->dist_dev, has_vacuum);
    return lean != 0;
}

enum { BUNI_NONE, BUNI_SCAN, BUNI_MIXED };
static void launch_relabel(xb_ctx *c, int *fs, int n_maxima, bool regions, const int *box_max, int buni, const int *bres) {
    const Grid &g = c->g;
    const GridL gl = light(g);
    const int nb1 = c->nbk[1], nb2 = c->nbk[2], nbr = c->nbk[0] * nb1 * nb2;
    const int *gate = fs ? fs + FS_SORT_OK : nullptr, *n_walk_dev = fs ? fs + FS_N_WALK : nullptr;
    int *ubuf = reinterpret_cast<int *>(c->st);
    if (regions) {
        const int v = g.nz % 4 == 0 ? 4 : 1;
        (v == 4 ? k_relabel_regions_brick<4> : k_relabel_regions_brick<1>)<<<dim3((g.nz / v + 63) / 64, nb1, (g.x1 - g.x0 + 3) / 4), TPB, 0, c->stream>>>(
            gl, c->labels, c->first, c->blab, nb1, nb2, box_max, fs, gate, fs ? -1 : c->n_boxes);
        if (buni == BUNI_MIXED) k_fill<int><<<(nbr + 4 * TPB - 1) / (4 * TPB), TPB, 0, c->stream>>>(ubuf, XB_MIXED, nbr);
        if (buni != BUNI_NONE && bres)
            k_buni_after_relabel<<<(nbr + 255) / 256, 256, 0, c->stream>>>(nbr, c->blab, box_max, c->first, ubuf, gate, c->walk, n_walk_dev, bres);
        else if (buni != BUNI_NONE) {
            k_buni_after_relabel<<<(nbr + 255) / 256, 256, 0, c->stream>>>(nbr, c->blab, box_max, c->first, ubuf, gate, nullptr, nullptr, nullptr);
            if (fs) k_label_uniform_list<<<2048, TPB, 0, c->stream>>>(gl, c->labels, nb1, nb2, c->walk, 0, n_walk_dev, gate, ubuf);
            else if (c->n_walk)
                k_label_uniform_list<<<(c->n_walk + 3) / 4, TPB, 0, c->stream>>>(gl, c->labels, nb1, nb2, c->walk, c->n_walk, nullptr, nullptr, ubuf);
        }
    } else
        k_relabel<<<nblocks((long long)(g.x1 - g.x0) * g.nyz), TPB, 0, c->stream>>>(g, c->labels, c->first, gate);
    if (fs) k_reset_first<<<8, 256, 0, c->stream>>>(c->first, c->max_aux, 0, fs + FS_N_MAX, gate);
    else if (n_maxima) k_reset_first<<<(unsigned)((n_maxima + 255) / 256), 256, 0, c->stream>>>(c->first, c->max_aux, n_maxima, nullptr, nullptr);
}

static void numbering_done(xb_ctx *c, const int *sorted, int nmax, int64_t *n_maxima) {
    if (sorted) c->maxima_sorted.assign(sorted, sorted + nmax);
    c->label_wire = label_wire_for(nmax);
    c->regions_pending = false;
    c->first_clean = true;
    if (n_maxima) *n_maxima = nmax;
}

extern "C++" template <int K, bool RHO, bool RESUME = false, bool EXPORT = false>
static void launch_refine_trace(xb_ctx *c, unsigned grid, int block, const int *list, int n_host, const int *n_dev, int *changed, int *escaped,
                                int *ovf_list, int *ovf_count, int ovf_cap, const unsigned char *brec, int *defer_list, int *defer_count,
                                int regions_ok, const int *region_blab, const WalkerIO &wio) {
    k_refine_trace<K, RHO, RESUME, EXPORT><<<grid, block, 0, c->stream>>>(light(c->g), c->grad, c->labels, c->known, list, n_host, n_dev, changed,
                                                                           escaped, ovf_list, ovf_count, ovf_cap, trace_maxsteps(c->g), c->rho,
                                                                           c->dist_dev, brec, defer_list, defer_count, regions_ok, region_blab, wio);
}
```

### pybader_amd/csrc/k_edges.h

```cpp
#pragma once

__device__ __forceinline__ void classify27(const Grid &g, const double *__restrict__ rho,
                                           const int *__restrict__ labels, int x, int y, int z, int v,
                                           bool &is_edge, bool &is_max) {
    const int vol_num = labels[v];
    is_edge = false;
    is_max = true;
    int nb[27];
    int k = 0;
#pragma unroll
    for (int ix = -1; ix < 2; ix++) {
        const int tx = wrapi(x + ix, g.nx);
#pragma unroll
        for (int iy = -1; iy < 2; iy++) {
            const int ty = wrapi(y + iy, g.ny);
#pragma unroll
            for (int iz = -1; iz < 2; iz++) {
                const int tz = wrapi(z + iz, g.nz);
                const int l = lin3(g, tx, ty, tz);
                const int nv = labels[l];
                nb[k++] = (nv == -1) ? -1 : l;
                if (nv != -1 && nv != vol_num) is_edge = true;
            }
        }
    }
    if (!is_edge) return;
    const double max_val = rho[v];
    double nr[27];
#pragma unroll
    for (k = 0; k < 27; k++) nr[k] = rho[nb[k] >= 0 ? nb[k] : v];
#pragma unroll
    for (k = 0; k < 27; k++) is_max &= !(nr[k] > max_val);
}

#define XB_MIXED (-2147483647 - 1)
__global__ __launch_bounds__(256) void k_buni_after_relabel(int nbr, const int *__restrict__ blab, const int *__restrict__ box_max,
                                                            const int *__restrict__ rank, int *__restrict__ buni, const int *gate,
                                                            const int *__restrict__ walk, const int *n_walk, const int *__restrict__ bres) {
    if (gate && !*gate) return;
    const int t = blockIdx.x * blockDim.x + threadIdx.x, nt = gridDim.x * blockDim.x;
    for (int b = t; b < nbr; b += nt) {
        const int l = blab[b];
        if (l > 0) buni[b] = rank[box_max[l - 1]];
    }
    if (!bres) return;
    const int n = *n_walk;
    for (int e = t; e < n; e += nt) {
        const int b = walk[e], r = bres[b];
        buni[b] = r == XB_MIXED ? XB_MIXED : rank[r];
    }
}

__global__ void k_buni3(int nb0, int nb1, int nb2, const int *__restrict__ buni, int *__restrict__ buni3) {
    const int b = blockIdx.x * blockDim.x + threadIdx.x;
    if (b >= nb0 * nb1 * nb2) return;
    const int b0 = b / (nb1 * nb2), b1 = (b / nb2) % nb1, b2 = b % nb2;
    const int l = buni[b];
    bool ok = l != XB_MIXED;
#pragma unroll
    for (int k = 0; k < 27; k++) {
        const int q = buni[(wrap_any(b0 + k / 9 - 1, nb0) * nb1 + wrap_any(b1 + (k / 3) % 3 - 1, nb1)) * nb2 + wrap_any(b2 + k % 3 - 1, nb2)];
        ok &= (q == l);
    }
    buni3[b] = ok ? l : XB_MIXED;
}
__global__ __launch_bounds__(TPB) void k_label_uniform_list(GridL g, const int *__restrict__ labels, int nb1, int nb2,
                                                            const int *__restrict__ walk, int n_walk, const int *n_dev,
                                                            const int *gate, int *__restrict__ buni, int b_off = 0, int nbr = 0) {
    if (gate && !*gate) return;
    const int n = n_dev ? *n_dev : n_walk;
    const int lane = threadIdx.x % XB_WAVE;
    for (int e = blockIdx.x * (TPB / XB_WAVE) + threadIdx.x / XB_WAVE; e < n; e += gridDim.x * (TPB / XB_WAVE)) {
        int b;
        if (walk) b = walk[e];
        else { b = e + b_off; if (b >= nbr) b -= nbr; }
        const int b0 = b / (nb1 * nb2), b1 = (b / nb2) % nb1, b2 = b % nb2;
        int lo = 2147483647, hi = XB_MIXED;
#pragma unroll
        for (int k = 0; k < 8; k++) {
            const int t = lane + k * XB_WAVE;
            const int x = b0 * 8 + t / 64, y = b1 * 8 + (t / 8) % 8, z = b2 * 8 + t % 8;
            if (x < g.nx && y < g.ny && z < g.nz) {
                const int l = labels[(x * g.ny + y) * g.nz + z];
                lo = min(lo, l); hi = max(hi, l);
            }
        }
        for (int o = 32; o > 0; o >>= 1) { lo = min(lo, __shfl_xor(lo, o)); hi = max(hi, __shfl_xor(hi, o)); }
        if (lane == 0) buni[b] = (lo == hi) ? lo : XB_MIXED;
    }
}

__global__ __launch_bounds__(TPB) void k_edge_dilate_list(GridL g, int8_t *known, const int *__restrict__ list, int n_host,
                                                          const int *n_dev) {
    const int n = n_dev ? *n_dev : n_host;
  for (int t = blockIdx.x * TPB + threadIdx.x; t < n; t += gridDim.x * TPB) {
    const int v = list[t];
    const int x = v / g.nyz;
    const int r = v - x * g.nyz;
    const int y = r / g.nz, z = r - y * g.nz;
    int row[9];
#pragma unroll
    for (int j = 0; j < 9; j++) row[j] = (wrapi(x + j / 3 - 1, g.nx) * g.ny + wrapi(y + j % 3 - 1, g.ny)) * g.nz;
    if (z >= 1 && z + 2 < g.nz) {
        unsigned int w[9];
#pragma unroll
        for (int j = 0; j < 9; j++) w[j] = *reinterpret_cast<const unsigned int *>(known + row[j] + z - 1);
#pragma unroll
        for (int j = 0; j < 27; j++)
            if (!((w[j / 3] >> (8 * (j % 3) + 7)) & 1u)) known[row[j / 3] + z - 1 + j % 3] = -1;
    } else {
        int8_t k[27];
#pragma unroll
        for (int j = 0; j < 27; j++) k[j] = known[row[j / 3] + wrapi(z + j % 3 - 1, g.nz)];
#pragma unroll
        for (int j = 0; j < 27; j++)
            if (k[j] >= 0) known[row[j / 3] + wrapi(z + j % 3 - 1, g.nz)] = -1;
    }
  }
}

#define ET_X 4
#define ET_Y 8
#define ET_Z 64
__device__ __forceinline__ void edge_tile(const GridL &g, const double *__restrict__ rho, const int *__restrict__ labels,
                                          int8_t *__restrict__ known, int xa, int nplanes, int *__restrict__ list,
                                          int *list_count, int small, const int *__restrict__ buni,
                                          const GradRec *__restrict__ G, const unsigned char *__restrict__ brick_rec,
                                          int no_vacuum, int tx0, int y0, int z0, int salt = 0) {
    const int tid = (int)threadIdx.x + salt;
    __shared__ int tile[ET_X + 2][ET_Y + 2][ET_Z + 2];
    if (buni) {
        __shared__ int s_lab, s_mixed;
        if (tid == 0) { s_lab = XB_MIXED; s_mixed = 0; }
        __syncthreads();
        const int nb1 = (g.ny + 7) >> 3, nb2 = (g.nz + 7) >> 3;
        int X0 = xa + tx0, X1 = xa + min(tx0 + ET_X, nplanes) - 1;
        if (X0 >= g.nx) X0 -= g.nx;
        if (X1 >= g.nx) X1 -= g.nx;
        const int bxa = X0 >> 3, bxb = X1 >> 3, nbz = min(ET_Z / 8, nb2 - (z0 >> 3));
        if ((int)tid < 2 * nbz) {
            const int bx = (tid & 1) ? bxb : bxa;
            const int l = buni[(bx * nb1 + (y0 >> 3)) * nb2 + (z0 >> 3) + (tid >> 1)];
            if (l == XB_MIXED) s_mixed = 1;
            else {
                const int old = atomicCAS(&s_lab, XB_MIXED, l);
                if (old != XB_MIXED && old != l) s_mixed = 1;
            }
        }
        __syncthreads();
        if (!s_mixed) {
            const int8_t o = (s_lab == -1) ? 0 : 2;
            if ((g.nz & 15) == 0 && z0 + ET_Z <= g.nz) {
                if (tid < 128) {
                    const int row = tid >> 2, seg = tid & 3;
                    const int xr = tx0 + (row >> 3), y = y0 + (row & 7);
                    if (xr < nplanes && y < g.ny) {
                        int x = xa + xr;
                        if (x >= g.nx) x -= g.nx;
                        const unsigned w = o ? 0x02020202u : 0u;
                        *reinterpret_cast<uint4 *>(known + ((size_t)(x * g.ny + y) * g.nz + z0 + seg * 16)) = make_uint4(w, w, w, w);
                    }
                }
                return;
            }
            const int tz = tid & 63, tyb = tid >> 6;
#pragma unroll
            for (int k = 0; k < 8; k++) {
                const int xr = tx0 + (k >> 1), y = y0 + tyb + ((k & 1) << 2), z = z0 + tz;
                if (xr < nplanes && y < g.ny && z < g.nz) {
                    int x = xa + xr;
                    if (x >= g.nx) x -= g.nx;
                    known[(x * g.ny + y) * g.nz + z] = o;
                }
            }
            return;
        }
    }
    __shared__ unsigned char s_binfo[ET_X][ET_Z / 8];
    {
        const int wv = __builtin_amdgcn_readfirstlane(tid / XB_WAVE), lane = tid % XB_WAVE;
        constexpr int NROW = (ET_X + 2) * (ET_Y + 2);
        static_assert(ET_Z == XB_WAVE && 2 * NROW <= TPB && TPB / XB_WAVE == 4 && ET_Y + 2 == 10, "tile shape");
        int Zc = z0 + lane;
        if (small) Zc %= g.nz;
        else Zc = wrap_u(Zc, g.nz);
        const int ey0 = wv < 2 ? 3 * wv : 2 * wv + 2, ney = wv < 2 ? 3 : 2;
        int yoff[3];
#pragma unroll
        for (int j = 0; j < 3; j++) {
            int Y = y0 + ey0 + j - 1;
            if (small) Y = ((Y % g.ny) + g.ny) % g.ny;
            else Y = wrap_u(Y, g.ny);
            yoff[j] = Y * g.nz;
        }
        int val[ET_X + 2][3];
#pragma unroll
        for (int ex = 0; ex < ET_X + 2; ex++) {
            int X = xa + tx0 + ex - 1;
            if (small) X = ((X % g.nx) + g.nx) % g.nx;
            else { X = wrap_u(X, g.nx); X = wrap_u(X, g.nx); }
            const int *plane = labels + (size_t)X * g.nyz;
#pragma unroll
            for (int j = 0; j < 3; j++) val[ex][j] = (j < ney) ? plane[yoff[j] + Zc] : 0;
        }
        int hv = 0;
        const int hr = tid >> 1, hside = tid & 1;
        const int hex = hr / (ET_Y + 2), hey = hr - hex * (ET_Y + 2);
        if (tid < 2 * NROW) {
            int X = xa + tx0 + hex - 1, Y = y0 + hey - 1, Z = hside ? z0 + ET_Z : z0 - 1;
            if (small) {
                X = ((X % g.nx) + g.nx) % g.nx; Y = ((Y % g.ny) + g.ny) % g.ny; Z = ((Z % g.nz) + g.nz) % g.nz;
            } else {
                X = wrap_u(X, g.nx); X = wrap_u(X, g.nx); Y = wrap_u(Y, g.ny); Z = wrap_u(Z, g.nz);
            }
            hv = labels[(X * g.ny + Y) * g.nz + Z];
        }
        if (tid >= TPB - ET_X * (ET_Z / 8)) {
            const int i = tid - (TPB - ET_X * (ET_Z / 8)), tx = i / (ET_Z / 8), zb = i % (ET_Z / 8);
            int x = xa + tx0 + tx;
            if (x >= g.nx) x -= g.nx;
            const int nb1 = (g.ny + 7) >> 3, nb2 = (g.nz + 7) >> 3, bz = (z0 >> 3) + zb;
            s_binfo[tx][zb] = (brick_rec && bz < nb2 && y0 < g.ny) ? brick_rec[((x >> 3) * nb1 + (y0 >> 3)) * nb2 + bz] : (unsigned char)1;
        }
#pragma unroll
        for (int ex = 0; ex < ET_X + 2; ex++)
#pragma unroll
            for (int j = 0; j < 3; j++)
                if (j < ney) tile[ex][ey0 + j][lane + 1] = val[ex][j];
        if (tid < 2 * NROW) tile[hex][hey][hside ? ET_Z + 1 : 0] = hv;
    }
    __syncthreads();
    const int tz = tid & 63, tyb = tid >> 6;
    unsigned ymin[ET_X + 2][2];
    int ymax[ET_X + 2][2];
#pragma unroll
    for (int ex = 0; ex < ET_X + 2; ex++) {
        unsigned rmin[6];
        int rmax[6];
#pragma unroll
        for (int r = 0; r < 6; r++) {
            const int ey = tyb + r + (r >= 3 ? 1 : 0);
            const int a = tile[ex][ey][tz], b = tile[ex][ey][tz + 1], c2 = tile[ex][ey][tz + 2];
            rmin[r] = min(min((unsigned)a, (unsigned)b), (unsigned)c2);
            rmax[r] = max(max(a, b), c2);
        }
        ymin[ex][0] = min(min(rmin[0], rmin[1]), rmin[2]); ymax[ex][0] = max(max(rmax[0], rmax[1]), rmax[2]);
        ymin[ex][1] = min(min(rmin[3], rmin[4]), rmin[5]); ymax[ex][1] = max(max(rmax[3], rmax[4]), rmax[5]);
        __builtin_amdgcn_sched_barrier(0);
    }
    unsigned cand = 0, inside = 0, vac = 0;
#pragma unroll
    for (int k = 0; k < 8; k++) {
        const int tx = k >> 1, ty = tyb + ((k & 1) << 2);
        if (tx0 + tx < nplanes && y0 + ty < g.ny && z0 + tz < g.nz) {
            inside |= 1u << k;
            const int lab = tile[tx + 1][ty + 1][tz + 1];
            if (lab == -1) vac |= 1u << k;
            else {
                const unsigned bmin = min(min(ymin[tx][k & 1], ymin[tx + 1][k & 1]), ymin[tx + 2][k & 1]);
                const int bmax = max(max(ymax[tx][k & 1], ymax[tx + 1][k & 1]), ymax[tx + 2][k & 1]);
                if (bmin < (unsigned)lab || bmax > lab) cand |= 1u << k;
            }
        }
    }
    unsigned edges = 0, full = 0;
#pragma unroll 1
    for (int h = 0; h < 2; h++) {
        if (!((cand >> (4 * h)) & 15u)) continue;
        unsigned pend = 0;
        double key[4];
#pragma unroll
        for (int q = 0; q < 4; q++) {
            const int k = 4 * h + q;
            key[q] = 0.;
            if ((cand >> k) & 1u) {
                const int tx = 2 * h + (q >> 1), ty = tyb + ((q & 1) << 2);
                const int binfo = s_binfo[tx][tz >> 3];
                if (brick_rec && no_vacuum && !(binfo & 2)) {
                    edges |= 1u << k;
                } else {
                    int x = xa + tx0 + tx;
                    if (x >= g.nx) x -= g.nx;
                    if (G && plane_in_window(g, x) && (binfo & 1)) {
                        key[q] = G[rec_slot(g, (x * g.ny + y0 + ty) * g.nz + z0 + tz)].key;
                        pend |= 1u << q;
                    } else
                        full |= 1u << k;
                }
            }
        }
#pragma unroll
        for (int q = 0; q < 4; q++)
            if ((pend >> q) & 1u) {
                const int k = 4 * h + q, tx = 2 * h + (q >> 1), ty = tyb + ((q & 1) << 2);
                const int og = key_og(key[q]);
                if (og != XB_OG_SELF && tile[tx + og / 9][ty + (og / 3) % 3][tz + og % 3] != -1) edges |= 1u << k;
                else full |= 1u << k;
            }
    }
#pragma unroll 1
    for (unsigned m = full; m; m &= m - 1) {
        const int k = __ffs(m) - 1;
        const int tx = k >> 1, ty = tyb + ((k & 1) << 2);
        int x = xa + tx0 + tx;
        if (x >= g.nx) x -= g.nx;
        const int y = y0 + ty, z = z0 + tz;
        const int v = (x * g.ny + y) * g.nz + z;
        bool is_max = true;
        const double c = rho[v];
        for (int dx = -1; dx < 2; dx++) {
            const int X = wrapi(x + dx, g.nx);
            for (int dy = -1; dy < 2; dy++) {
                const int Y = wrapi(y + dy, g.ny);
                for (int dz = -1; dz < 2; dz++) {
                    const int Z = wrapi(z + dz, g.nz);
                    if (tile[tx + 1 + dx][ty + 1 + dy][tz + 1 + dz] != -1 && rho[(X * g.ny + Y) * g.nz + Z] > c) is_max = false;
                }
            }
        }
        if (!is_max) edges |= 1u << k;
    }
    int vidx[8];
    int cnt = 0;
#pragma unroll
    for (int k = 0; k < 8; k++) {
        vidx[k] = -1;
        if ((inside >> k) & 1u) {
            const int tx = k >> 1, ty = tyb + ((k & 1) << 2);
            int x = xa + tx0 + tx;
            if (x >= g.nx) x -= g.nx;
            const int v = (x * g.ny + y0 + ty) * g.nz + z0 + tz;
            const bool e = (edges >> k) & 1u;
            known[v] = ((vac >> k) & 1u) ? 0 : (e ? -2 : 2);
            if (e && x >= g.x0 && x < g.x1) { vidx[k] = v; cnt++; }
        }
    }
    int total;
    const int off = block_scan_excl(cnt, total);
    __shared__ int base_s;
    if (tid == 0) base_s = total ? atomicAdd(list_count, total) : 0;
    __syncthreads();
    int w = base_s + off;
#pragma unroll
    for (int k = 0; k < 8; k++)
        if (vidx[k] >= 0) list[w++] = vidx[k];
}

__device__ __forceinline__ unsigned long long bytes_equal_fe(unsigned long long w) {
    const unsigned long long x = w ^ 0xFEFEFEFEFEFEFEFEull, m = 0x7F7F7F7F7F7F7F7Full;
    return ~(((x & m) + m) | x | m);
}
__global__ __launch_bounds__(TPB) void k_edge_dilate_tiles(GridL g, int8_t *known, const int *__restrict__ tiles, const int *n_tiles) {
    constexpr int ROW = ET_Z + 8;
    __shared__ __attribute__((aligned(16))) int8_t s[(ET_X + 2) * (ET_Y + 2) * ROW];
    static_assert(ET_X * ET_Y * (ET_Z / 8) == TPB && (ET_X + 2) * (ET_Y + 2) * 4 <= TPB, "one 8-voxel chunk per thread");
    const int ntz = g.nz / ET_Z, nty = (g.ny + ET_Y - 1) / ET_Y, n = *n_tiles;
    const int n_xcd = (gridDim.x % 8 == 0) ? 8 : 1;
    const int part = (n + n_xcd - 1) / n_xcd, part0 = (int)(blockIdx.x % n_xcd) * part, part1 = min(n, part0 + part);
  for (int item = part0 + blockIdx.x / n_xcd; item < part1; item += gridDim.x / n_xcd) {
    const int t = (int)((unsigned)tiles[item] & 0x7fffffffu);
    const int tx0 = (t / (ntz * nty)) * ET_X, y0 = ((t / ntz) % nty) * ET_Y, z0 = (t % ntz) * ET_Z;
    __syncthreads();
    if (threadIdx.x < (ET_X + 2) * (ET_Y + 2) * 4) {
        const int row = threadIdx.x >> 2, q = threadIdx.x & 3;
        const size_t base = (size_t)(wrapi(tx0 + row / (ET_Y + 2) - 1, g.nx) * g.ny + wrapi(y0 + row % (ET_Y + 2) - 1, g.ny)) * g.nz;
        const uint4 w = *reinterpret_cast<const uint4 *>(known + base + z0 + 16 * q);
        unsigned *d = reinterpret_cast<unsigned *>(s + row * ROW + 4 + 16 * q);
        d[0] = w.x; d[1] = w.y; d[2] = w.z; d[3] = w.w;
        if (q < 2) s[row * ROW + (q ? 4 + ET_Z : 3)] = known[base + wrapi(q ? z0 + ET_Z : z0 - 1, g.nz)];
    }
    __syncthreads();
    const int ex = threadIdx.x / (ET_Y * (ET_Z / 8)), ey = (threadIdx.x / (ET_Z / 8)) % ET_Y, ch = threadIdx.x % (ET_Z / 8);
    unsigned long long e0 = 0, e1 = 0, c0 = 0, c1 = 0;
#pragma unroll
    for (int j = 0; j < 9; j++) {
        const unsigned long long *p = reinterpret_cast<const unsigned long long *>(s + ((ex + j / 3) * (ET_Y + 2) + ey + j % 3) * ROW + 8 * ch);
        const unsigned long long w0 = p[0], w1 = p[1];
        e0 |= bytes_equal_fe(w0); e1 |= bytes_equal_fe(w1);
        if (j == 4) { c0 = w0; c1 = w1; }
    }
    const unsigned long long n0 = e0 | (e0 << 8) | (e0 >> 8) | (e1 << 56), n1 = e1 | (e1 << 8) | (e1 >> 8) | (e0 >> 56);
    unsigned long long old = (c0 >> 32) | (c1 << 32), near = (n0 >> 32) | (n1 << 32);
    const unsigned long long hit = near & ~old & 0x8080808080808080ull;
    if (hit && tx0 + ex < g.nx && y0 + ey < g.ny) {
        const unsigned long long fill = (hit >> 7) * 0xFFull;
        *reinterpret_cast<unsigned long long *>(known + ((size_t)(tx0 + ex) * g.ny + y0 + ey) * g.nz + z0 + 8 * ch) = old | fill;
    }
  }
}

__global__ __launch_bounds__(TPB) void k_edge_flag_tiled(GridL g, const double *__restrict__ rho,
                                                         const int *__restrict__ labels,
                                                         int8_t *__restrict__ known, int xa, int nplanes,
                                                         int *__restrict__ list, int *list_count, int small,
                                                         const int *__restrict__ buni,
                                                         const GradRec *__restrict__ G,
                                                         const unsigned char *__restrict__ brick_rec, int no_vacuum) {
    edge_tile(g, rho, labels, known, xa, nplanes, list, list_count, small, buni, G, brick_rec, no_vacuum, blockIdx.z * ET_X,
              blockIdx.y * ET_Y, blockIdx.x * ET_Z);
}
__global__ __launch_bounds__(TPB) void k_edge_tile_list(GridL g, const int *__restrict__ buni3, int *tiles, int *n_tiles, int tx_lo,
                                                        int tx_n, const int *gate = nullptr) {
    if (gate && (gate[FS_SORT_OK] == 0 || gate[FS_TIES] != 0)) return;
    const int ntz = (g.nz + ET_Z - 1) / ET_Z, nty = (g.ny + ET_Y - 1) / ET_Y, ntx = (g.nx + ET_X - 1) / ET_X;
    const int i = blockIdx.x * TPB + threadIdx.x;
    bool hit = false;
    unsigned entry = 0;
    if (i < tx_n * nty * ntz) {
        int tx = tx_lo + i / (ntz * nty);
        if (tx >= ntx) tx -= ntx;
        const int tz = i % ntz, ty = (i / ntz) % nty;
        const int t = (tx * nty + ty) * ntz + tz;
        const int nb1 = (g.ny + 7) >> 3, nb2 = (g.nz + 7) >> 3;
        const int bxa = (tx * ET_X) >> 3, bxb = (tx * ET_X + ET_X - 1) >> 3, nbz = min(ET_Z / 8, nb2 - ((tz * ET_Z) >> 3));
        int lab = XB_MIXED;
        bool mixed = false;
        for (int k = 0; k < 2 * nbz; k++) {
            const int l = buni3[(((k & 1) ? bxb : bxa) * nb1 + ((ty * ET_Y) >> 3)) * nb2 + ((tz * ET_Z) >> 3) + (k >> 1)];
            if (l == XB_MIXED) mixed = true;
            else if (lab == XB_MIXED) lab = l;
            else if (lab != l) mixed = true;
        }
        hit = mixed || lab == -1;
        entry = (unsigned)t | ((!mixed && lab == -1) ? 0x80000000u : 0u);
    }
    int total;
    const int off = block_scan_excl(hit ? 1 : 0, total);
    __shared__ int base_s;
    if (threadIdx.x == 0) base_s = total ? atomicAdd(n_tiles, total) : 0;
    __syncthreads();
    if (hit) tiles[base_s + off] = (int)entry;
}
__global__ __launch_bounds__(TPB) void k_edge_flag_listed(GridL g, const double *__restrict__ rho, const int *__restrict__ labels,
                                                          int8_t *__restrict__ known, int *__restrict__ list, int *list_count,
                                                          int small, const GradRec *__restrict__ G,
                                                          const unsigned char *__restrict__ brick_rec, int no_vacuum,
                                                          const int *__restrict__ tiles, const int *n_tiles) {
    const int n = *n_tiles;
    const int ntz = (g.nz + ET_Z - 1) / ET_Z, nty = (g.ny + ET_Y - 1) / ET_Y;
    const int n_xcd = (gridDim.x % 8 == 0) ? 8 : 1;
    const int part = (n + n_xcd - 1) / n_xcd, part0 = (int)(blockIdx.x % n_xcd) * part, part1 = min(n, part0 + part);
#pragma unroll 1
    for (int item = part0 + blockIdx.x / n_xcd; item < part1; item += gridDim.x / n_xcd) {
        const unsigned entry = (unsigned)tiles[item];
        const int t = (int)(entry & 0x7fffffffu);
        const int tx0 = (t / (ntz * nty)) * ET_X, y0 = ((t / ntz) % nty) * ET_Y, z0 = (t % ntz) * ET_Z;
        if (entry & 0x80000000u) {
            for (int i = threadIdx.x; i < ET_X * ET_Y * ET_Z; i += TPB) {
                const int z = z0 + (i % ET_Z), y = y0 + (i / ET_Z) % ET_Y, x = tx0 + i / (ET_Z * ET_Y);
                if (z < g.nz && y < g.ny && x < g.nx) known[(x * g.ny + y) * g.nz + z] = 0;
            }
            continue;
        }
        __syncthreads();
        int salt = 0;
        asm volatile("" : "+v"(salt));
        edge_tile(g, rho, labels, known, 0, g.nx, list, list_count, small, nullptr, G, brick_rec, no_vacuum, tx0, y0, z0, salt);
    }
}

__global__ __launch_bounds__(TPB) void k_list_changed(const int *__restrict__ list, const int *n_dev, const int8_t *__restrict__ known,
                                                      int *__restrict__ out, int *out_count, int out_cap, const int *n_changed) {
    __shared__ int s_buf[BlockAppender<1>::CAP], s_n[2];
    if (*n_changed == 0) return;
    BlockAppender<1> app;
    app.init(s_buf, s_n, out, out_count, out_cap);
    const int n = *n_dev;
    for (int base = blockIdx.x * TPB; base < n; base += gridDim.x * TPB) {
        const int t = base + threadIdx.x;
        const int v = t < n ? list[t] : 0;
        const bool hit = t < n && known[v] == -2;
        app.add(hit ? 1 : 0, [&](int) { return v; });
    }
    app.finish();
}
#define CK_CHUNKS 4
__global__ __launch_bounds__(TPB) void k_compact_known16(GridL g, const int8_t *__restrict__ known, int value,
                                                         int *__restrict__ list, int *count) {
    const long long vbeg = (long long)g.x0 * g.nyz, vend = (long long)g.x1 * g.nyz;
    long long base[CK_CHUNKS];
    int8_t b[CK_CHUNKS][16];
#pragma unroll
    for (int c = 0; c < CK_CHUNKS; c++) {
        base[c] = vbeg + (((long long)blockIdx.x * CK_CHUNKS + c) * TPB + threadIdx.x) * 16;
        if (base[c] + 16 <= vend && ((vbeg & 15) == 0)) {
            *reinterpret_cast<uint4 *>(b[c]) = *reinterpret_cast<const uint4 *>(known + base[c]);
        } else {
#pragma unroll
            for (int k = 0; k < 16; k++) b[c][k] = (base[c] + k < vend) ? known[base[c] + k] : (int8_t)(value + 1);
        }
    }
    int cnt = 0;
#pragma unroll
    for (int c = 0; c < CK_CHUNKS; c++)
#pragma unroll
        for (int k = 0; k < 16; k++) cnt += (b[c][k] == value);
    int total;
    const int off = block_scan_excl(cnt, total);
    __shared__ int base_s;
    if (threadIdx.x == 0) base_s = total ? atomicAdd(count, total) : 0;
    __syncthreads();
    int w = base_s + off;
#pragma unroll
    for (int c = 0; c < CK_CHUNKS; c++)
#pragma unroll
        for (int k = 0; k < 16; k++)
            if (b[c][k] == value) list[w++] = (int)(base[c] + k);
}

__global__ __launch_bounds__(TPB) void k_edge_dilate(Grid g, int8_t *known, int xa, int nplanes, int flag) {
    const long long vv = (long long)blockIdx.x * TPB + threadIdx.x;
    if (vv >= (long long)nplanes * g.nyz) return;
    const int xr = (int)(vv / g.nyz);
    const int r = (int)(vv - (long long)xr * g.nyz);
    int x = xa + xr;
    if (x >= g.nx) x -= g.nx;
    const int y = r / g.nz, z = r - y * g.nz;
    const int v = lin3(g, x, y, z);
    if (known[v] < 0) return;
    bool near = false;
#pragma unroll
    for (int ix = -1; ix < 2; ix++) {
        const int tx = wrapi(x + ix, g.nx);
#pragma unroll
        for (int iy = -1; iy < 2; iy++) {
            const int ty = wrapi(y + iy, g.ny);
#pragma unroll
            for (int iz = -1; iz < 2; iz++) {
                const int tz = wrapi(z + iz, g.nz);
                near |= (known[lin3(g, tx, ty, tz)] == flag);
            }
        }
    }
    if (near) known[v] = -1;
}

struct Walker {
    int v, vol_num;
    int lp, lq;
    double dr0, dr1, dr2;
    int widx[2];
    double wval[2];
    double m_old;
    int steps, og_move;
};
struct WalkerIO {
    const Walker *in;
    Walker *out;
    int *out_count;
    int out_cap;
    int *res;
    int *res_count;
    int own0, own1;
};
#define XB_WALKER_STUCK (-2147483647 - 1)

template <int K, bool RHO, bool RESUME = false, bool EXPORT = false>
__global__ __launch_bounds__(TPB) void k_refine_trace(GridL g, const GradRec *__restrict__ G, int *labels,
                                                      int8_t *known, const int *__restrict__ list, int n_host,
                                                      const int *n_dev, int *changed, int *escaped, int *ovf_list,
                                                      int *ovf_count, int ovf_cap, int maxsteps,
                                                      const double *__restrict__ rho, const double *__restrict__ gc,
                                                      const unsigned char *__restrict__ brick_rec, int *defer_list,
                                                      int *defer_count, int regions_ok, const int *__restrict__ region_blab,
                                                      WalkerIO wio) {
    static_assert(!RESUME || (RHO && K == 2), "walkers are carried on by the from-rho kernel");
    const int n = n_dev ? *n_dev : n_host;
    int n_ch = 0, n_es = 0;
  const XcdRange xr = xcd_range((n + (int)blockDim.x - 1) / (int)blockDim.x);
  for (int chunk = xr.begin; chunk < xr.end; chunk += xr.step) {
    const int t = chunk * (int)blockDim.x + threadIdx.x;
    bool valid = t < n;
    int v = (valid && !RESUME) ? list[t] : 0;
    bool moving = false;
    int result = -3;
    int px = 0, py = 0, pz = 0, lp = 0, steps = 0, vol_num = 0;
    double dr0 = 0., dr1 = 0., dr2 = 0.;
    GradRec rec = {0., 0., 0., 0.};
    PathWindow<K> w;
    w.init(0, 0.);
    bool arrive = false, og_in = false;
    int lq_in = 0;
    if (RESUME) {
        if (valid) {
            const Walker wk = wio.in[t];
            const int qx = wk.lq / g.nyz;
            valid = qx >= wio.own0 && qx < wio.own1;
            if (valid) {
                v = wk.v; vol_num = wk.vol_num; lp = wk.lp; lq_in = wk.lq;
                px = lp / g.nyz;
                const int r = lp - px * g.nyz;
                py = r / g.nz;
                pz = r - py * g.nz;
                dr0 = wk.dr0; dr1 = wk.dr1; dr2 = wk.dr2;
                w.idx[0] = wk.widx[0]; w.idx[K - 1] = wk.widx[1];
                w.val[0] = wk.wval[0]; w.val[K - 1] = wk.wval[1];
                w.m_old = wk.m_old;
                steps = wk.steps; og_in = wk.og_move != 0;
                arrive = true; moving = true;
            }
        }
    } else
    if (valid) {
        px = v / g.nyz;
        const int r = v - px * g.nyz;
        py = r / g.nz;
        pz = r - py * g.nz;
        lp = v;
        rec = fetch_rec_w(g, G, v);
        vol_num = labels[v];
        moving = true;
        if (region_blab && region_blab[((px >> 3) * ((g.ny + 7) >> 3) + (py >> 3)) * ((g.nz + 7) >> 3) + (pz >> 3)] > 0) {
            result = v; moving = false;
        } else
        if (!(plane_in_window(g, px) && rec_exists(brick_rec, g, px, py, pz))) {
            if (RHO) rec = make_rec_rho(g, rho, gc, px, py, pz);
            else { result = regions_ok ? v : -5; moving = false; }
        }
        w.init(v, rec.key);
    }
#ifdef XB_DEBUG_COUNT
    int dbg_it = 0;
#endif
    while (__any(moving)) {
        if (moving) {
#ifdef XB_DEBUG_COUNT
            dbg_it++;
#endif
            int qx = 0, qy = 0, qz = 0, lq = 0;
            bool og_move = false;
            if (RESUME && arrive) {
                arrive = false;
                lq = lq_in; og_move = og_in;
                qx = lq / g.nyz;
                const int r = lq - qx * g.nyz;
                qy = r / g.nz;
                qz = r - qy * g.nz;
            } else {
            const int bits = key_bits(rec.key);
            const int code = bits & 63;
            og_move = (code == XB_STAY_CODE);
            if (!og_move) {
                ng_move_t(g, px, py, pz, rec, code, dr0, dr1, dr2, qx, qy, qz);
                lq = lin3f(g, qx, qy, qz);
                og_move = w.contains(lq);
            }
            if (og_move) {
                const int og = (bits >> 6) & 31;
                if (og == XB_OG_SELF) { result = lp; moving = false; }
                else {
                    int ox, oy, oz;
                    og_offsets(og, ox, oy, oz);
                    dr0 = dr1 = dr2 = 0.;
                    qx = wrap_u(px + ox, g.nx); qy = wrap_u(py + oy, g.ny); qz = wrap_u(pz + oz, g.nz);
                    lq = lin3f(g, qx, qy, qz);
                }
// ... 612 lines not shown
```

### pybader_amd/csrc/k_fused.h

```cpp
#pragma once

enum {
    FS_N_SEEDS = 0,
    FS_TIES,
    FS_N_SEEDS_EFF,
    FS_N_BOXES,
    FS_GROW_PHASE,
    FS_GROW_CHANGED,
    FS_GROW_TICKET,
    FS_GROW_CUR,
    FS_GROW_CONVERGED,
    FS_N_CERTAIN,
    FS_N_WALK,
    FS_N_MAX,
    FS_N_OVF,
    FS_SORT_OK,
    FS_ERR,
    FS_N_EDGES,
    FS_CHANGED, FS_ESCAPED, FS_R_OVF,
    FS_R_DEFER,
    FS_N_TILES,
    FS_N_CHGLIST,
    FS_GROW_RETRY,
    FS_N_RECL,
    FS_N_REDO,
    FS_COUNT = 64,
    FS_CURSOR0 = 64, FS_CURSOR_STRIDE = 32,
    FS_TOTAL = FS_CURSOR0 + 8 * FS_CURSOR_STRIDE
};

enum {
    CT_N_MAX = 0,
    CT_N_OVF = 1,
    CT_MID_LEFT = CT_N_OVF,
    CT_CHANGED = 2,
    CT_ESCAPED = 3,
    CT_OG_MOVED = 4,
    CT_N_EDGES = 5,
    CT_N_COMPACT = CT_N_EDGES,
    CT_HALO_EDGES = 6,
    CT_EC_SEEDS_A = CT_HALO_EDGES,
    CT_TEXT_TODO = CT_HALO_EDGES,
    CT_EC_NEW = 7,
    CT_ESC_ERR = 8,
    CT_N_WALK = 13,
    CT_ANY_EQUAL = 14,
    CT_REDO = 15,
    CT_DEFER = CT_REDO,
    CT_MID_LISTED = CT_REDO,
    CT_WALK_OUT = 16,
    CT_WALK_RES = 17,
    CT_WALK_CHANGED = 18,
    CT_WALK_STUCK = 19,
    CT_WALK_LOST = 20,
    CT_WALK_ROUNDS = 21,
    CT_TILES_OWN = 22,
    CT_TILES_HALO = 23,
    CT_EC_SEEDS_B = 24,
    CT_EC_UNDECIDED = 25,
    CT_EC_NEXT = 26,
    CT_EC_DONE = 27,
    CT_COUNT = 28,
    CT_FS = 128
};
static_assert(CT_COUNT <= CT_FS, "fs lies behind the counters");
#define CT_INTS(first, last) ((last) - (first) + 1)
static_assert(CT_ESCAPED == CT_CHANGED + 1 && CT_WALK_RES == CT_WALK_OUT + 1 && CT_WALK_STUCK == CT_WALK_CHANGED + 1 &&
              CT_TILES_HALO == CT_TILES_OWN + 1 && CT_EC_NEXT == CT_EC_UNDECIDED + 1, "slots cleared or read back as a pair");
enum { C64_EC_EDGES = 0, C64_EC_CHECKED = 1 };
static_assert(C64_EC_CHECKED == C64_EC_EDGES + 1, "cleared and read back as a pair");
enum {
    HI_EC_SEEDS0 = 1,
    HI_EC_SHARE_ERR = 2,
    HI_EC_CHGLIST = 8,
    HI_SLAB_DBG = 64,
    HI_REFINE = 3000,
    HI_UPLOAD = 3100,
    HI_TOTAL = 4096
};

#define XB_REGIONS_MAX 65535

#define XB_BOXES_MAX 1024
__global__ __launch_bounds__(BG * BG * BG) void k_brick_grow_dev(int nb0, int nb1, int nb2, const int *__restrict__ bmask,
                                                                 const int *__restrict__ seed, int *buf0, int *buf1, int *fs,
                                                                 int inner, int seeds_fixed) {
    __shared__ int lab[2][BG + 2][BG + 2][BG + 2];
    __shared__ int s_any;
    const int phase = fs[FS_GROW_PHASE];
    if (phase >= 2) return;
    const int curbuf = fs[FS_GROW_CUR];
    const int *in = curbuf ? buf1 : buf0;
    int *out = curbuf ? buf0 : buf1;
    if (threadIdx.x == 0) s_any = 0;
    const int c0 = blockIdx.z * BG, c1 = blockIdx.y * BG, c2 = blockIdx.x * BG;
    for (int i = threadIdx.x; i < (BG + 2) * (BG + 2) * (BG + 2); i += BG * BG * BG) {
        const int e2 = i % (BG + 2), e1 = (i / (BG + 2)) % (BG + 2), e0 = i / ((BG + 2) * (BG + 2));
        const int l = in[(wrap_any(c0 + e0 - 1, nb0) * nb1 + wrap_any(c1 + e1 - 1, nb1)) * nb2 + wrap_any(c2 + e2 - 1, nb2)];
        lab[0][e0][e1][e2] = l;
        lab[1][e0][e1][e2] = l;
    }
    const int t2 = threadIdx.x % BG, t1 = (threadIdx.x / BG) % BG, t0 = threadIdx.x / (BG * BG);
    const int b0 = c0 + t0, b1 = c1 + t1, b2 = c2 + t2;
    const bool active = b0 < nb0 && b1 < nb1 && b2 < nb2;
    const int b = active ? (b0 * nb1 + b1) * nb2 + b2 : 0;
    const int m = active ? bmask[b] : 0;
    const int sd = active ? seed[b] : 0;
    const bool fixed = !active || (phase == 0 && (m >> 27)) || (phase == 1 && seeds_fixed && sd != 0);
    const bool own_seed_ok = !seeds_fixed && sd != 0 && !((m >> 28) & 1);
    __syncthreads();
    const int first = lab[0][t0 + 1][t1 + 1][t2 + 1];
    int l = first, cur = 0;
    for (int it = 0; it < inner; it++) {
        int nl = l;
        if (!fixed) {
            if (phase == 0) {
                if (l == 0) {
                    int best = 0;
                    for (unsigned mm = (unsigned)m & 0x7ffffffu; mm; mm &= mm - 1) {
                        const int k = __ffs(mm) - 1;
                        const int q = lab[cur][t0 + k / 9][t1 + (k / 3) % 3][t2 + k % 3];
                        if (q > 0 && (best == 0 || q < best)) best = q;
                    }
                    nl = best;
                }
            } else if (l > 0) {
                bool ok = !(m >> 27) || (own_seed_ok && sd == l);
                for (unsigned mm = (unsigned)m & 0x7ffffffu; mm && ok; mm &= mm - 1) {
                    const int k = __ffs(mm) - 1;
                    ok = (lab[cur][t0 + k / 9][t1 + (k / 3) % 3][t2 + k % 3] == l);
                }
                if (!ok) nl = 0;
            }
        }
        lab[cur ^ 1][t0 + 1][t1 + 1][t2 + 1] = nl;
        const int any = __syncthreads_or(nl != l);
        l = nl;
        cur ^= 1;
        if (!any) break;
    }
    if (active) out[b] = l;
    if (active && l != first) s_any = 1;
    __syncthreads();
    if (threadIdx.x == 0) {
        const int nblk = gridDim.x * gridDim.y * gridDim.z;
        const int old = atomicAdd(&fs[FS_GROW_TICKET], 1 + (s_any ? 0x10000 : 0));
        if ((old & 0xffff) == nblk - 1) {
// ... 27 lines not shown
}
__global__ __launch_bounds__(TPB) void k_grow_chase(int nbr, const int *__restrict__ parent, const int *__restrict__ seed, int *__restrict__ lab,
                                                    int limit, int *fs) {
    const int b = blockIdx.x * TPB + threadIdx.x;
    if (b == 0) {
        const int n = min(fs[FS_N_SEEDS], XB_REGIONS_MAX);
        fs[FS_N_SEEDS_EFF] = n;
        fs[FS_N_BOXES] = n;
        fs[FS_GROW_PHASE] = n ? 1 : 2;
        fs[FS_GROW_CONVERGED] = 0;
        fs[FS_GROW_CUR] = 0;
    }
    if (b >= nbr) return;
    int p = b, l = 0;
    for (int it = 0; it < limit; it++) {
        const int pp = parent[p];
        if (pp < 0) break;
        if (pp == p) { l = seed[p]; break; }
        p = pp;
    }
    lab[b] = l;
}
__global__ __launch_bounds__(TPB) void k_grow_finish(int nbr, const int *__restrict__ seed, const int *__restrict__ buf0,
                                                     const int *__restrict__ buf1, int *fs, int *__restrict__ blab,
                                                     int *box_first, const int *__restrict__ bmask, unsigned char *brick_rec,
                                                     int seeds_fixed, int verdict) {
    __shared__ int s_first[XB_BOXES_MAX];
    const bool retry = verdict ? (fs[FS_GROW_PHASE] == 1 && !fs[FS_GROW_CONVERGED]) : fs[FS_GROW_RETRY] != 0;
    if (verdict && blockIdx.x == 0 && threadIdx.x == 0) fs[FS_GROW_RETRY] = retry ? 1 : 0;
    if (retry) return;
    const int *src = fs[FS_GROW_CONVERGED] ? (fs[FS_GROW_CUR] ? buf1 : buf0) : seed;
    const int nbx = (fs[FS_GROW_CONVERGED] || seeds_fixed) ? fs[FS_N_BOXES] : 0;
    for (int i = threadIdx.x; i < XB_BOXES_MAX; i += TPB) s_first[i] = XB_INT_MAX;
    __syncthreads();
    int cnt = 0;
    for (int b = blockIdx.x * TPB + threadIdx.x; b < nbr; b += gridDim.x * TPB) {
        const int l = nbx ? src[b] : 0;
        blab[b] = l;
        if (brick_rec) brick_rec[b] = (unsigned char)(((bmask[b] >> 27) & 1) << 1);
        cnt += (l > 0);
        if (l > 0 && l <= XB_BOXES_MAX) { if (s_first[l - 1] > b) atomicMin(&s_first[l - 1], b); }
        else if (l > XB_BOXES_MAX) atomicMin(&box_first[l - 1], b);
    }
    __syncthreads();
    for (int i = threadIdx.x; i < XB_BOXES_MAX; i += TPB)
        if (s_first[i] != XB_INT_MAX) atomicMin(&box_first[i], s_first[i]);
    int total;
    block_scan_excl(cnt, total);
    if (threadIdx.x == 0 && total) atomicAdd(&fs[FS_N_CERTAIN], total);
}
__global__ __launch_bounds__(XB_BOXES_MAX) void k_note_regions(GridL g, int nb1, int nb2, const int *__restrict__ fs, const int *__restrict__ box_first,
                                                     const int *__restrict__ box_max, int *first, int *max_list, int *max_count,
                                                     int max_cap) {
    if (fs[FS_GROW_RETRY]) return;
    for (int t = threadIdx.x; t < fs[FS_N_BOXES]; t += blockDim.x) {
        if (box_first[t] == XB_INT_MAX) continue;
        const int b = box_first[t];
        const int b0 = b / (nb1 * nb2), b1 = (b / nb2) % nb1, b2 = b % nb2;
        note_maximum(box_max[t], ((b0 * 8) * g.ny + b1 * 8) * g.nz + b2 * 8, first, max_list, max_count, max_cap);
    }
}
__global__ void k_seed_bricks(int nbr, const int *__restrict__ bmask, const int *__restrict__ bmaxv, int *fs, int *seed, int *buf0,
                              int *box_max, int *box_first) {
    const int b = blockIdx.x * blockDim.x + threadIdx.x;
    for (int i = b; i < XB_REGIONS_MAX; i += gridDim.x * blockDim.x) box_first[i] = XB_INT_MAX;
    if (b >= nbr) return;
    int id = 0;
    if (((bmask[b] >> 27) & 3) == 1) {
        const int k = atomicAdd(&fs[FS_N_SEEDS], 1);
        if (k < XB_REGIONS_MAX) { id = k + 1; box_max[k] = bmaxv[b]; }
    }
    seed[b] = id;
    buf0[b] = id;
}
__global__ void k_seed_finish(int *fs) {
    const int n = min(fs[FS_N_SEEDS], XB_REGIONS_MAX);
    fs[FS_N_SEEDS_EFF] = n;
    fs[FS_N_BOXES] = n;
    fs[FS_GROW_PHASE] = n ? 0 : 2;
    fs[FS_GROW_CONVERGED] = 0;
}
#define XB_SORT_MAX 2048
static_assert(FS_TOTAL + XB_SORT_MAX <= HI_REFINE && HI_UPLOAD < HI_TOTAL, "host_ints: the far corners lie behind an assignment's block");
__global__ __launch_bounds__(1024) void k_number_maxima(int *fs, int *first, const int *__restrict__ max_list, int max_cap,
                                                        int *sorted, int *sorted2 = nullptr) {
    __shared__ unsigned long long key[XB_SORT_MAX];
    const int n = fs[FS_N_MAX];
    if (n > XB_SORT_MAX || n > max_cap || fs[FS_N_OVF] > 0 || fs[FS_GROW_RETRY]) { if (threadIdx.x == 0) fs[FS_SORT_OK] = 0; return; }
    int len = 64;
    while (len < n) len <<= 1;
    for (int i = threadIdx.x; i < len; i += 1024)
        key[i] = i < n ? ((unsigned long long)(unsigned)first[max_list[i]] << 32) | (unsigned)max_list[i] : ~0ull;
    __syncthreads();
    for (int k = 2; k <= len; k <<= 1)
        for (int j = k >> 1; j > 0; j >>= 1) {
            for (int i = threadIdx.x; i < len; i += 1024) {
                const int p = i ^ j;
                if (p > i) {
                    const unsigned long long a = key[i], b = key[p];
                    const bool up = (i & k) == 0;
                    if ((a > b) == up) { key[i] = b; key[p] = a; }
                }
            }
            __syncthreads();
        }
    for (int i = threadIdx.x; i < n; i += 1024) {
        const int m = (int)(key[i] & 0xffffffffu);
        sorted[i] = m;
        if (sorted2) sorted2[i] = m;
        first[m] = i;
    }
    if (threadIdx.x == 0) fs[FS_SORT_OK] = 1;
}

__global__ void k_rank_mark(const int *__restrict__ first, const int *__restrict__ max_list, int n, unsigned *bits) {
    const int i = blockIdx.x * blockDim.x + threadIdx.x;
    if (i >= n) return;
    const unsigned v = (unsigned)first[max_list[i]];
    atomicOr(&bits[v >> 5], 1u << (v & 31));
}
__device__ __forceinline__ int scan1024_excl(int x, int &total) {
    __shared__ int wsum[1024 / XB_WAVE];
    const int lane = threadIdx.x % XB_WAVE, w = threadIdx.x / XB_WAVE;
    int incl = x;
#pragma unroll
    for (int o = 1; o < XB_WAVE; o <<= 1) {
        const int t = __shfl_up(incl, o);
        if (lane >= o) incl += t;
    }
    if (lane == XB_WAVE - 1) wsum[w] = incl;
    __syncthreads();
    int base = 0;
    total = 0;
#pragma unroll
    for (int q = 0; q < 1024 / XB_WAVE; q++) {
        if (q < w) base += wsum[q];
        total += wsum[q];
    }
    __syncthreads();
    return base + incl - x;
}
__global__ __launch_bounds__(1024) void k_rank_scan(const unsigned *__restrict__ bits, int n_words, int *__restrict__ wprefix, int *__restrict__ bsum) {
    const int w = blockIdx.x * 1024 + threadIdx.x;
    const int cnt = w < n_words ? __popc(bits[w]) : 0;
    int total;
    const int excl = scan1024_excl(cnt, total);
    if (w < n_words) wprefix[w] = excl;
    if (threadIdx.x == 0) bsum[blockIdx.x] = total;
}
__global__ __launch_bounds__(1024) void k_rank_blocks(int *bsum, int n_blocks) {
    int carry = 0;
    for (int base = 0; base < n_blocks; base += 1024) {
        const int i = base + threadIdx.x;
        const int x = i < n_blocks ? bsum[i] : 0;
        int total;
        const int excl = scan1024_excl(x, total);
        if (i < n_blocks) bsum[i] = carry + excl;
        carry += total;
    }
}
__global__ void k_rank_assign(int *first, const int *__restrict__ max_list, int n, const unsigned *__restrict__ bits,
                              const int *__restrict__ wprefix, const int *__restrict__ bsum, int *__restrict__ sorted, int *fs) {
    const int i = blockIdx.x * blockDim.x + threadIdx.x;
    if (i == 0) fs[FS_SORT_OK] = 1;
    if (i >= n) return;
    const int m = max_list[i];
// ... 7 lines not shown
```

### pybader_amd/csrc/k_trace.h

```cpp
#pragma once

__global__ __launch_bounds__(TPB) void k_fill_certain(GridL g, const int *__restrict__ blab, int nb1, int nb2,
                                                      const int *__restrict__ box_max, int *labels, int *first,
                                                      int *max_list, int *max_count, int max_cap, const int *skip = nullptr) {
    if (skip && *skip) return;
    const int vbeg = g.x0 * g.nyz, vend = g.x1 * g.nyz;
    const int v = vbeg + blockIdx.x * TPB + threadIdx.x;
    const bool in = v < vend;
    int result = -1;
    bool has = false;
    if (in) {
        const int x = v / g.nyz;
        const int r = v - x * g.nyz;
        const int y = r / g.nz, z = r - y * g.nz;
        const int b = blab[((x >> 3) * nb1 + (y >> 3)) * nb2 + (z >> 3)];
        if (b > 0 && labels[v] != -1) {
            result = box_max[b - 1];
            if (result != v && labels[result] == -1) result = -1;
            labels[v] = result;
            has = result >= 0;
        }
    }
    note_maximum_wave(has, result, in ? v : 0, first, max_list, max_count, max_cap);
}
// ... 141 lines not shown
        const int lab0 = has_vacuum ? labels[v] : 0;
        int b = (blab && !in_walk) ? blab[((sx >> 3) * nb1 + (sy >> 3)) * nb2 + (sz >> 3)] : 0;
        rec = fetch_rec_w(g, G, v);
        if (lab0 != -1) {
            px = sx; py = sy; pz = sz;
            lp = v;
            if (b <= 0) b = key_box(rec.key);
            if (b > 0) result = box_max[b - 1];
            else { w.init(v, rec.key); moving = true; }
        }
    }
    while (__any(moving)) {
        if (moving) {
            const int bits = key_bits(rec.key);
            const int code = bits & 63;
            int qx, qy, qz, lq = 0;
            bool og_move = (code == XB_STAY_CODE);
            if (!og_move) {
                ng_move_t(g, px, py, pz, rec, code, dr0, dr1, dr2, qx, qy, qz);
                lq = lin3f(g, qx, qy, qz);
                og_move = w.contains(lq);
            }
            if (og_move) {
                const int og = (bits >> 6) & 31;
                if (og == XB_OG_SELF) { result = lp; moving = false; }
                else {
                    int ox, oy, oz;
                    og_offsets(og, ox, oy, oz);
                    dr0 = dr1 = dr2 = 0.;
                    qx = wrap_u(px + ox, g.nx); qy = wrap_u(py + oy, g.ny); qz = wrap_u(pz + oz, g.nz);
                    lq = lin3f(g, qx, qy, qz);
                }
            }
            if (moving) {
                const bool in_win = plane_in_window(g, qx);
                GradRec nr = fetch_rec(G, in_win ? rec_slot(g, lq) : 0);
                const int bl = blab ? blab[((qx >> 3) * nb1 + (qy >> 3)) * nb2 + (qz >> 3)] : 0;
                if (WIN && !in_win && bl <= 0) nr = make_rec_rho(g, rho, gc, qx, qy, qz);
                const int b = bl > 0 ? bl : key_box(nr.key);
                if (bl == XB_NOREC) {
                    result = -2;
                    moving = false;
                } else if (b) {
                    result = box_max[b - 1];
                    moving = false;
                } else if ((!WIN && !in_win) || (!og_move && nr.key <= w.m_old) || ++steps > maxsteps) {
                    result = -2;
                    moving = false;
                } else {
                    w.push(lq, nr.key);
                    px = qx; py = qy; pz = qz; lp = lq; rec = nr;
                }
            }
        }
    }
    if (has_vacuum && valid && result >= 0 && result != v && labels[result] == -1) result = -1;
    if (valid) labels[v] = result;
    note_maximum_wave(valid && result >= 0, result, v, first, max_list, max_count, max_cap);
    if (valid && result == -2) {
        const int k = atomicAdd(ovf_count, 1);
        if (k < ovf_cap) ovf_list[k] = v;
    }
}
__device__ __forceinline__ int wrap3(int q, int n) {
    return (int)min(min((unsigned)q, (unsigned)(q + n)), (unsigned)(q - n));
}
__device__ __forceinline__ int mad24(int a, int b, int c) {
    int r;
    asm("v_mad_u32_u24 %0, %1, %2, %3" : "=v"(r) : "v"(a), "s"(b), "v"(c));
    return r;
}
__device__ __forceinline__ int lin24(const GridL &g, int x, int y, int z) { return mad24(mad24(x, g.ny, y), g.nz, z); }
template <bool OFF32>
__device__ __forceinline__ GradRec fetch_rec_o(const GradRec *__restrict__ G, int l) {
    if (OFF32) return *reinterpret_cast<const GradRec *>(reinterpret_cast<const char *>(G) + ((unsigned)l << 5));
    return fetch_rec(G, l);
}
constexpr int XB_TRACE_WAVES = 4;
__shared__ GradRec xb_s_rec[512];
template <bool OFF32, bool CACHE, bool WINDOW = false>
__device__ __forceinline__ int ng_walk_lean(const GridL &g, const GradRec *__restrict__ G, const int *__restrict__ box_max,
                                             const int *__restrict__ blab, int nb1, int nb2, int sx, int sy, int sz,
                                             int *labels, int *first, int *max_list, int *max_count, int max_cap,
                                             int *ovf_list, int *ovf_count, int ovf_cap, int maxsteps, bool has_vacuum) {
    const int v = lin24(g, sx, sy, sz);
    const int lab0 = has_vacuum ? labels[v] : 0;
    const int ox8 = sx & ~7, oy8 = sy & ~7, oz8 = sz & ~7;
    GradRec rec = CACHE ? xb_s_rec[((sx & 7) << 6) | ((sy & 7) << 3) | (sz & 7)] : fetch_rec_o<OFF32>(G, WINDOW ? rec_slot(g, v) : v);
    int result = -1;
    int px = sx, py = sy, pz = sz, steps = 0;
    double dr0 = 0., dr1 = 0., dr2 = 0.;
    int i0 = v, i1 = -1;
    double k0 = rec.key, k1 = -1.7976931348623157e308, m_old = -1.7976931348623157e308;
#ifdef XB_DEBUG_COUNT
    int dbg_lane_steps = 0;
#endif
    if (lab0 != -1) for (;;) {
        const int bits = key_bits(rec.key);
        const double t0 = dr0 + rec.r0, t1 = dr1 + rec.r1, t2 = dr2 + rec.r2;
        const int id0 = rha_cs(t0), id1 = rha_cs(t1), id2 = rha_cs(t2);
        const int m0 = (bits & 3) + id0 - 1, m1 = ((bits >> 2) & 3) + id1 - 1, m2 = ((bits >> 4) & 3) + id2 - 1;
        px += m0; py += m1; pz += m2;
        dr0 = t0 - (double)id0; dr1 = t1 - (double)id1; dr2 = t2 - (double)id2;
        if (__builtin_amdgcn_ballot_w64((unsigned)px >= (unsigned)g.nx || (unsigned)py >= (unsigned)g.ny || (unsigned)pz >= (unsigned)g.nz) != 0) {
            px = wrap3(px, g.nx); py = wrap3(py, g.ny); pz = wrap3(pz, g.nz);
        }
        int lq = lin24(g, px, py, pz);
        const bool og_move = (bits & 63) == XB_STAY_CODE || lq == i0 || lq == i1;
        bool at_max = false;
        if (__builtin_amdgcn_ballot_w64(og_move) != 0) {
            if (og_move) {
                const int og = (bits >> 6) & 31;
                int ox, oy, oz;
                og_offsets(og, ox, oy, oz);
                at_max = og == XB_OG_SELF;
                dr0 = dr1 = dr2 = 0.;
                px = wrap3(wrap3(px - m0, g.nx) + ox, g.nx);
                py = wrap3(wrap3(py - m1, g.ny) + oy, g.ny);
                pz = wrap3(wrap3(pz - m2, g.nz) + oz, g.nz);
                lq = lin24(g, px, py, pz);
            }
        }
        int bl = 0;
        const bool own = CACHE && (unsigned)((px ^ ox8) | (py ^ oy8) | (pz ^ oz8)) < 8u;
        const bool in_win = !WINDOW || own || plane_in_window(g, px);
        if (own) rec = xb_s_rec[((px & 7) << 6) | ((py & 7) << 3) | (pz & 7)];
        else {
            rec = fetch_rec_o<OFF32>(G, WINDOW ? (in_win ? rec_slot(g, lq) : 0) : lq);
            const unsigned bidx = (unsigned)mad24(mad24(px >> 3, nb1, py >> 3), nb2, pz >> 3);
            bl = *reinterpret_cast<const int *>(reinterpret_cast<const char *>(blab) + (bidx << 2));
        }
        steps++;
#ifdef XB_DEBUG_COUNT
        dbg_lane_steps++;
#endif
        const bool arrived = bl > 0 && !at_max;
        const bool undecided = (!og_move && rec.key <= m_old) || steps > maxsteps || (WINDOW && !in_win) || bl == XB_NOREC;
        if (arrived) result = box_max[bl - 1];
        else if (at_max) result = i0;
        else if (undecided) result = -2;
        if (arrived || at_max || undecided) break;
        m_old = max_raw(m_old, k1);
        i1 = i0; k1 = k0;
        i0 = lq; k0 = rec.key;
    }
#ifdef XB_DEBUG_COUNT
    if (xb_dbg_steps) xb_dbg_steps[v] = (signed char)min(dbg_lane_steps, 127);
#endif
    if (has_vacuum && result >= 0 && result != v && labels[result] == -1) result = -1;
    labels[v] = result;
    note_maximum_wave(result >= 0, result, v, first, max_list, max_count, max_cap);
    if (result == -2) {
        const int k = atomicAdd(ovf_count, 1);
        if (k < ovf_cap) ovf_list[k] = v;
    }
    return result;
}
__device__ __forceinline__ void brick_sub_voxel(int b, int sub, int lane, int nb1, int nb2, int &sx, int &sy, int &sz) {
    const int b0 = b / (nb1 * nb2), b1 = (b / nb2) % nb1, b2 = b % nb2;
    sx = b0 * 8 + ((sub >> 2) << 2) + (lane >> 4);
    sy = b1 * 8 + ((sub & 3) << 1) + ((lane >> 3) & 1);
    sz = b2 * 8 + (lane & 7);
}
template <int K, bool WIN>
__global__ __launch_bounds__(TPB) void k_ng_trace(GridL g, const GradRec *__restrict__ G,
                                                  const int *__restrict__ box_max, const int *__restrict__ blab,
                                                  int nb1, int nb2, const int *__restrict__ walk, int n_walk,
                                                  int *labels, int *first,
                                                  int *max_list, int *max_count, int max_cap, int *ovf_list,
                                                  int *ovf_count, int ovf_cap, int maxsteps, int opt,
                                                  const double *__restrict__ rho, const double *__restrict__ gc, int has_vacuum) {
    int blk = blockIdx.x;
    if (opt & 2) {
        const int per = gridDim.x >> 3;
        if (blk < (per << 3)) blk = (blk & 7) * per + (blk >> 3);
    }
    const int wpb = blockDim.x / XB_WAVE;
    const int wave = blk * wpb + threadIdx.x / XB_WAVE;
    const int lane = threadIdx.x % XB_WAVE;
    int sx, sy, sz;
    if (walk) {
        if ((wave >> 3) >= n_walk) return;
        brick_sub_voxel(walk[wave >> 3], wave & 7, lane, nb1, nb2, sx, sy, sz);
        if (sx < g.x0 || sx >= g.x1) return;
    } else if (opt & 1) {
        const int bz_n = (g.nz + 3) >> 2, by_n = (g.ny + 3) >> 2;
        const int bx = wave / (by_n * bz_n);
        const int brem = wave - bx * (by_n * bz_n);
        const int by = brem / bz_n, bz = brem - by * bz_n;
        sx = g.x0 + bx * 4 + (lane >> 4); sy = by * 4 + ((lane >> 2) & 3); sz = bz * 4 + (lane & 3);
    } else {
        const int rz_n = (g.nz + 63) >> 6;
        const int row = wave / rz_n;
        sz = (wave - row * rz_n) * 64 + lane;
        sx = g.x0 + row / g.ny;
        sy = row - (row / g.ny) * g.ny;
    }
    ng_walk_wave<K, WIN>(g, G, box_max, blab, nb1, nb2, walk != nullptr, sx, sy, sz, labels, first, max_list, max_count,
                         max_cap, ovf_list, ovf_count, ovf_cap, maxsteps, rho, gc, has_vacuum != 0);
}
template <int K>
__global__ __launch_bounds__(TPB) void k_ng_trace_list(GridL g, const GradRec *__restrict__ G, const int *__restrict__ box_max,
                                                       const int *__restrict__ blab, int nb1, int nb2,
                                                       const int *__restrict__ vox, const int *n_dev, int *labels, int *first,
                                                       int *max_list, int *max_count, int max_cap, int *ovf_list,
                                                       int *ovf_count, int ovf_cap, int maxsteps,
                                                       const double *__restrict__ rho, const double *__restrict__ gc, int has_vacuum) {
    const int n = *n_dev;
    for (int base = blockIdx.x * TPB; base < n; base += gridDim.x * TPB) {
        const int t = base + threadIdx.x;
        int sx = g.x1, sy = 0, sz = 0;
        if (t < n) {
            const int v = vox[t];
            sx = v / g.nyz;
            const int r = v - sx * g.nyz;
            sy = r / g.nz;
            sz = r - sy * g.nz;
        }
        ng_walk_wave<K, true>(g, G, box_max, blab, nb1, nb2, true, sx, sy, sz, labels, first, max_list, max_count, max_cap,
                              ovf_list, ovf_count, ovf_cap, maxsteps, rho, gc, has_vacuum != 0);
    }
}
__device__ __forceinline__ int xcc_id() {
    int x;
    asm volatile("s_getreg_b32 %0, hwreg(HW_REG_XCC_ID)" : "=s"(x));
    return x & 7;
}

template <int K, int LEAN, bool WINDOW = false, bool PART = false>
__global__ __launch_bounds__(XB_WAVE * XB_TRACE_WAVES, 8) void k_ng_trace_g(GridL g, const GradRec *__restrict__ G, const int *__restrict__ box_max,
                                                       const int *__restrict__ blab, int nb1, int nb2,
                                                       const int *__restrict__ walk, int *fs, int *labels, int *first,
                                                       int *max_list, int max_cap, int *ovf_list, int ovf_cap, int maxsteps,
                                                       int has_vacuum, int CH, int xcd_split, int *__restrict__ bres = nullptr) {
    __shared__ int s_base, s_next;
    __shared__ int s_w[8], s_mixed;
    constexpr bool CACHE = LEAN >= 3;
    int prev_brick = -1;
#ifdef XB_DEBUG_COUNT
    const long long pr_t0 = clock64();
    long long pr_walk = 0, pr_wait = 0, pr_load = 0;
    int pr_bricks = 0;
    const unsigned long long pr_e0 = wall_clock64();
#endif
    const int n_items = fs[FS_N_WALK] * 8;
    const int per = (((n_items + 7) >> 3) + 7) & ~7;
    const int home = xcd_split ? xcc_id() : (blockIdx.x & 7);
    const int lane = threadIdx.x & (XB_WAVE - 1);
    auto verdict = [&]() {
        if (CACHE && bres && prev_brick >= 0) {
            int r0 = s_mixed ? -1 : s_w[0];
#pragma unroll
            for (int k = 1; k < 8; k++) r0 = (s_w[k] == r0) ? r0 : -1;
            bres[prev_brick] = r0 >= 0 ? r0 : (-2147483647 - 1);
        }
        prev_brick = -1;
    };
    for (int r = 0; r < 8; r++) {
        const int q = (home + r) & 7;
        const int beg = q * per, end = min(beg + per, n_items);
        for (;;) {
#ifdef XB_DEBUG_COUNT
            const long long pr_a = clock64();
#endif
            __syncthreads();
#ifdef XB_DEBUG_COUNT
            pr_wait += clock64() - pr_a;
#endif
            if (threadIdx.x == 0) {
                verdict();
                s_mixed = 0;
                s_base = beg + atomicAdd(&fs[FS_CURSOR0 + q * FS_CURSOR_STRIDE], CH);
                s_next = 0;
            }
            __syncthreads();
            const int base = s_base;
            if (base >= end) break;
            const int stop = min(base + CH, end);
#ifdef XB_DEBUG_COUNT
            const long long pr_b = clock64();
            pr_bricks++;
#endif
            if (CACHE) {
                constexpr int PER = 512 / (XB_WAVE * XB_TRACE_WAVES);
                const int b = walk[base >> 3];
                prev_brick = b;
                const int b0 = b / (nb1 * nb2), b1 = (b / nb2) % nb1, b2 = b % nb2;
                GradRec tmp[PER];
#pragma unroll
                for (int k = 0; k < PER; k++) {
                    const int t = threadIdx.x + k * XB_WAVE * XB_TRACE_WAVES;
                    int cx = b0 * 8 + (t >> 6), cy = b1 * 8 + ((t >> 3) & 7), cz = b2 * 8 + (t & 7);
                    if (PART) { cx = min(cx, g.nx - 1); cy = min(cy, g.ny - 1); cz = min(cz, g.nz - 1); }
                    const int lt = lin24(g, cx, cy, cz);
                    tmp[k] = fetch_rec(G, WINDOW ? rec_slot(g, lt) : lt);
                }
#pragma unroll
                for (int k = 0; k < PER; k++) xb_s_rec[threadIdx.x + k * XB_WAVE * XB_TRACE_WAVES] = tmp[k];
                __syncthreads();
            }
#ifdef XB_DEBUG_COUNT
            pr_load += clock64() - pr_b;
#endif
            for (;;) {
                int i = 0;
                if (lane == 0) i = atomicAdd(&s_next, 1);
                const int item = base + __builtin_amdgcn_readfirstlane(i);
                if (item >= stop) break;
                int sx, sy, sz;
                brick_sub_voxel(walk[item >> 3], item & 7, lane, nb1, nb2, sx, sy, sz);
                if (PART) { sx = min(sx, g.nx - 1); sy = min(sy, g.ny - 1); sz = min(sz, g.nz - 1); }
                if (LEAN) {
#ifdef XB_DEBUG_COUNT
                    const long long pr_c = clock64();
#endif
                    const int res = ng_walk_lean<LEAN == 4, CACHE, WINDOW>(g, G, box_max, blab, nb1, nb2, sx, sy, sz, labels, first, max_list, &fs[FS_N_MAX],
                                                                max_cap, ovf_list, &fs[FS_N_OVF], ovf_cap, maxsteps, has_vacuum != 0);
#ifdef XB_DEBUG_COUNT
                    pr_walk += clock64() - pr_c;
#endif
                    if (CACHE && bres) {
                        volatile int *w = s_w;
                        if (lane == 0) w[item - base] = res;
                        if (w[item - base] != res) *(volatile int *)&s_mixed = 1;
                    }
                }
                else
                    ng_walk_wave<K, false>(g, G, box_max, blab, nb1, nb2, true, sx, sy, sz, labels, first, max_list, &fs[FS_N_MAX],
                                           max_cap, ovf_list, &fs[FS_N_OVF], ovf_cap, maxsteps, nullptr, nullptr, has_vacuum != 0);
            }
        }
    }
#ifdef XB_DEBUG_COUNT
    if (lane == 0 && blockIdx.x < 2048) {
        unsigned long long *o = xb_dbg + 64 + 6 * (blockIdx.x * XB_TRACE_WAVES + (threadIdx.x >> 6));
        o[0] = (unsigned long long)pr_walk; o[1] = (unsigned long long)(clock64() - pr_t0); o[2] = (unsigned long long)pr_wait;
        o[3] = (unsigned long long)pr_load; o[4] = pr_e0; o[5] = (unsigned long long)wall_clock64();
        if (threadIdx.x == 0) xb_dbg[64 + 6 * 8192 + blockIdx.x] = (unsigned long long)pr_bricks;
    }
#endif
    if (CACHE && bres) {
        __syncthreads();
        if (threadIdx.x == 0) verdict();
    }
}

__global__ __launch_bounds__(TPB) void k_list_unfinished(GridL g, const int *__restrict__ walk, const int *n_walk, int nb1, int nb2,
                                                         const int *__restrict__ labels, int *out, int *out_count, int out_cap) {
    __shared__ int s_buf[BlockAppender<2>::CAP], s_n[2];
    BlockAppender<2> app;
    app.init(s_buf, s_n, out, out_count, out_cap);
    const int n = *n_walk;
    for (int e = blockIdx.x; e < n; e += gridDim.x) {
        const int b = walk[e];
        const int b0 = b / (nb1 * nb2), b1 = (b / nb2) % nb1, b2 = b % nb2;
        int v[2];
        int cnt = 0;
#pragma unroll
        for (int k = 0; k < 2; k++) {
            const int t = threadIdx.x + k * TPB;
            const int x = b0 * 8 + (t >> 6), y = b1 * 8 + ((t >> 3) & 7), z = b2 * 8 + (t & 7);
            if (x < g.nx && y < g.ny && z < g.nz) {
                const int l = (x * g.ny + y) * g.nz + z;
                if (labels[l] == -2) v[cnt++] = l;
            }
        }
        app.add(cnt, [&](int k) { return v[k]; });
    }
    app.finish();
}

__global__ void k_path_pack(const int *__restrict__ path, int lmax, const int *__restrict__ off, const int *__restrict__ len,
                            const int *__restrict__ first, int *__restrict__ packed) {
    const int t = blockIdx.x;
    const int *P = path + (size_t)t * lmax;
    if (threadIdx.x == 0) packed[off[t]] = P[0];
    for (int k = first[t] + threadIdx.x; k < len[t]; k += blockDim.x) packed[off[t] + 1 + k - first[t]] = P[k];
}
template <bool SCATTER>
__global__ void k_move_voxels(const int *__restrict__ idx, int n, int *labels, int8_t *known, int *lab_buf, int8_t *kn_buf) {
    const int t = blockIdx.x * blockDim.x + threadIdx.x;
    if (t >= n) return;
    if (SCATTER) { labels[idx[t]] = lab_buf[t]; known[idx[t]] = kn_buf[t]; }
    else { lab_buf[t] = labels[idx[t]]; kn_buf[t] = known[idx[t]]; }
}

__global__ void k_trace_slow(Grid g, const double *__restrict__ rho, int *labels, const int8_t *known_ro,
                             int8_t *known, const int *list, int n, int *path, int lmax, int refine, int *first,
                             int *max_list, int *max_count, int max_cap, int *changed, int *escaped, int *err,
                             int *lens, int has_vacuum = 1, long long sk = 1, long long st = -1, int *retry = nullptr, int *retry_count = nullptr,
                             const int *n_dev = nullptr) {
    const int t = blockIdx.x * blockDim.x + threadIdx.x;
    if (t >= n || (n_dev && t >= *n_dev)) return;
    const int v = list[t];
    if (st < 0) st = lmax;
    int *P0 = path + (size_t)t * st;
#define P(k) P0[(size_t)(k) * sk]
    int np = 0;
    int px = v / g.nyz;
    int r = v - px * g.nyz;
// ... 57 lines not shown
```

Before: 42560 Mvoxels/s.

## Bin refinement edge voxels by assign-trace step count to balance retrace work

During the assign trace, each voxel's walk length is recorded as a byte hint in spare stage memory. Edge flagging then sorts edge voxels into per-partition, per-bin sub-lists keyed on that hint. The refine-trace kernel reads these sub-lists so that wavefronts hold voxels with similar walk lengths, which is meant to reduce lane divergence in the retrace. In exchange it adds a byte store per traced voxel, per-block shared and global atomics during flagging, segmented list handling in the dilate and changed-list kernels, and a full redo of the refinement iteration when a bin overflows.

```diff
diff --git a/include/bader_hip.h b/include/bader_hip.h
--- a/include/bader_hip.h
+++ b/include/bader_hip.h
@@ -161,6 +161,7 @@
 int xb_brick_labels(xb_ctx *c, int32_t *out, int64_t capacity, int64_t dims[3]);
 int xb_slow_path_stats(xb_ctx *c, int64_t *assign_total, int64_t *refine_total);
 int xb_deferred_stats(xb_ctx *c, int64_t *refine_total);
+int xb_retrace_bin_stats(xb_ctx *c, int64_t *binned_total, int64_t *redo_total);
 int xb_growth_stats(xb_ctx *c, int64_t *retries, int64_t *kill_launches);
 
 int xb_comm_unique_id(uint8_t id_out[128]);
diff --git a/pybader_amd/_lib.py b/pybader_amd/_lib.py
--- a/pybader_amd/_lib.py
+++ b/pybader_amd/_lib.py
@@ -108,6 +108,7 @@
     'xb_brick_labels': (_int, [_vp, _vp, _i64, _pi64]),
     'xb_slow_path_stats': (_int, [_vp, _pi64, _pi64]),
     'xb_deferred_stats': (_int, [_vp, _pi64]),
+    'xb_retrace_bin_stats': (_int, [_vp, _pi64, _pi64]),
     'xb_growth_stats': (_int, [_vp, _pi64, _pi64]),
     'xb_comm_unique_id': (_int, [_vp]),
     'xb_comm_init': (_int, [_vp, _int, _int, _vp]),
@@ -932,6 +933,11 @@
         check(self.lib.xb_deferred_stats(self.h, C.byref(a)))
         return a.value
 
+    def retrace_bin_stats(self):
+        a, b = C.c_int64(), C.c_int64()
+        check(self.lib.xb_retrace_bin_stats(self.h, C.byref(a), C.byref(b)))
+        return a.value, b.value
+
     def sync(self):
         check(self.lib.xb_sync(self.h))
 
diff --git a/pybader_amd/csrc/bader_hip.hip b/pybader_amd/csrc/bader_hip.hip
--- a/pybader_amd/csrc/bader_hip.hip
+++ b/pybader_amd/csrc/bader_hip.hip
@@ -131,6 +131,9 @@
     bool defer_wait = false;
     bool pending_assign = false;
     int64_t pending_n_maxima = 0;
+    int opt_bins = 1;
+    unsigned char *hint = nullptr;
+    long long stat_bin_steps = 0, stat_bin_redo = 0;
     int opt_lean = 1;
     int opt_mirror = 1;
     int grad_rule = 0;
@@ -308,6 +311,7 @@
         c->opt_narrow_halo = !(value & 16);
         c->opt_ec_share = !(value & 32);
         c->opt_io_tiled = !(value & 64);
+        c->opt_bins = !(value & 128);
     }
     else if (key == 3) c->opt_dbg = value;
     else if (key == 4 && value >= 1 && value <= 4096) c->opt_ec_groups = value;
@@ -329,6 +333,12 @@
 int xb_deferred_stats(xb_ctx *c, int64_t *refine_total) {
     if (!c) return fail(XB_E_ARG, "null ctx");
     if (refine_total) *refine_total = c->stat_deferred;
+    return XB_OK;
+}
+int xb_retrace_bin_stats(xb_ctx *c, int64_t *binned_total, int64_t *redo_total) {
+    if (!c) return fail(XB_E_ARG, "null ctx");
+    if (binned_total) *binned_total = c->stat_bin_steps;
+    if (redo_total) *redo_total = c->stat_bin_redo;
     return XB_OK;
 }
 int xb_slow_path_stats(xb_ctx *c, int64_t *assign_total, int64_t *refine_total) {
diff --git a/pybader_amd/csrc/host_assign.h b/pybader_amd/csrc/host_assign.h
--- a/pybader_amd/csrc/host_assign.h
+++ b/pybader_amd/csrc/host_assign.h
@@ -437,6 +437,7 @@
         }
     };
     if (int rc = begin_assignment(c, fs, FS_TOTAL, true)) return rc;
+    c->hint = nullptr;
     g.main_ties = 1;
     const GridL gl = light(g);
     {
@@ -484,7 +485,8 @@
         {
             ScopedTimer t6(c, 6);
             int *bres_buf = c->has_vacuum ? nullptr : c->list + 6 * nbr;
-            if (launch_persistent_trace(c, true, part, box_max, walk, c->has_vacuum ? 1 : 0, bres_buf)) bres = bres_buf;
+            unsigned char *hint = c->defer_wait && c->opt_bins && !c->has_vacuum && c->stage_bytes >= 8 * (size_t)c->N ? (unsigned char *)c->stage + 4 * (size_t)c->N : nullptr;
+            if (launch_persistent_trace(c, true, part, box_max, walk, c->has_vacuum ? 1 : 0, bres_buf, hint)) { bres = bres_buf; c->hint = hint; }
         }
         HIPCHK(hipGetLastError());
         stage_done("trace");
@@ -508,6 +510,7 @@
 
 static int assign_neargrid_tail(xb_ctx *c, int64_t *n_maxima) {
     Grid &g = c->g;
+    c->hint = nullptr;
     int *fs = c->fs;
     const int nb1 = c->nbk[1], nb2 = c->nbk[2];
     int *walk = c->walk, *box_max = c->box_max_tab;
diff --git a/pybader_amd/csrc/host_context.h b/pybader_amd/csrc/host_context.h
--- a/pybader_amd/csrc/host_context.h
+++ b/pybader_amd/csrc/host_context.h
@@ -17,7 +17,7 @@
     xb_ctx *c = new xb_ctx();
     c->device = device;
     HIPCHK(hipStreamCreate(&c->stream));
-    HIPCHK(hipMalloc(&c->counters, (1024 + XB_SORT_MAX) * sizeof(int)));
+    HIPCHK(hipMalloc(&c->counters, CT_TOTAL * sizeof(int)));
     c->fs = c->counters + CT_FS;
     HIPCHK(hipMalloc(&c->counters64, 16 * sizeof(unsigned long long)));
     HIPCHK(hipMalloc(&c->dsum, 16 * sizeof(double)));
diff --git a/pybader_amd/csrc/host_refine.h b/pybader_amd/csrc/host_refine.h
--- a/pybader_amd/csrc/host_refine.h
+++ b/pybader_amd/csrc/host_refine.h
@@ -602,9 +602,16 @@
     int *fs = c->fs;
     c->g.main_ties = 0;
     const GridL gl = light(g);
-    static_assert(FS_N_CHGLIST == FS_N_EDGES + 6, "one memset clears the refinement's counters");
-    HIPCHK(hipMemsetAsync(fs + FS_N_EDGES, 0, 7 * sizeof(int), c->stream));
+    static_assert(FS_BIN_OVF == FS_N_EDGES + 7, "one memset clears the refinement's counters");
+    HIPCHK(hipMemsetAsync(fs + FS_N_EDGES, 0, 8 * sizeof(int), c->stream));
     c->chg_n = -1;
+    const unsigned char *hint = c->hint;
+    c->hint = nullptr;
+    const int bin_cap = (int)std::min<long long>(c->list_cap / (XB_RB_PARTS * XB_RB_BINS), (c->opt_dbg & 128) ? 16 : 0x7fffffff / (XB_RB_PARTS * XB_RB_BINS));
+    const bool bins = hint && c->pending_assign && c->opt_bins && !late_records && c->grad_valid && c->grad_cover == 1 && c->brick_rec && bin_cap >= 1 &&
+                      g.nx >= 16 && g.ny >= 16 && g.nz >= 16;
+    int *bin_counts = c->counters + CT_BINS;
+    if (bins) HIPCHK(hipMemsetAsync(bin_counts, 0, XB_RB_PARTS * XB_RB_BINS * CT_BIN_STRIDE * sizeof(int), c->stream));
     {
         ScopedTimer t(c, 2);
         const int small = small_grid(g);
@@ -620,6 +627,10 @@
             HIPCHK(hipMemsetAsync(c->known, 2, (size_t)c->N, c->stream));
             k_edge_tile_list<<<(ntiles + TPB - 1) / TPB, TPB, 0, c->stream>>>(gl, buni, tiles, fs + FS_N_TILES, 0, (g.nx + ET_X - 1) / ET_X,
                                                                               c->pending_assign ? fs : nullptr);
+            if (bins)
+                k_edge_flag_listed<true><<<std::min(ntiles, 2048), TPB, 0, c->stream>>>(gl, c->rho, c->labels, c->known, c->list, nullptr, small, c->grad, brec,
+                                                               c->has_vacuum ? 0 : 1, tiles, fs + FS_N_TILES, EdgeBins{hint, bin_counts, fs + FS_BIN_OVF, bin_cap});
+            else
             k_edge_flag_listed<<<std::min(ntiles, 2048), TPB, 0, c->stream>>>(gl, c->rho, c->labels, c->known, c->list, fs + FS_N_EDGES, small,
                                                            c->grad_valid ? c->grad : nullptr, brec, c->has_vacuum ? 0 : 1, tiles, fs + FS_N_TILES);
         } else {
@@ -628,6 +639,7 @@
                                                            c->grad_valid ? c->grad : nullptr, brec, c->has_vacuum ? 0 : 1);
         }
         if (buni && c->opt_tile_dilate && g.nz % ET_Z == 0) k_edge_dilate_tiles<<<std::min(ntiles_listed, 4096), TPB, 0, c->stream>>>(gl, c->known, (const int *)c->stage, fs + FS_N_TILES);
+        else if (bins) k_edge_dilate_list<<<nblocks(c->N / 16), TPB, 0, c->stream>>>(gl, c->known, c->list, 0, bin_counts, XB_RB_PARTS * XB_RB_BINS, bin_cap, CT_BIN_STRIDE);
         else k_edge_dilate_list<<<nblocks(c->N / 16), TPB, 0, c->stream>>>(gl, c->known, c->list, 0, fs + FS_N_EDGES);
     }
     c->list_valid = false; c->chg_n = -1;
@@ -656,7 +668,13 @@
         int *defer = (int *)c->stage;
         WalkerIO wl{};
         constexpr int XB_RT_BLOCK = 128;
-        launch_refine_trace<2, false>(c, (unsigned)((c->N / 16 + XB_RT_BLOCK - 1) / XB_RT_BLOCK), XB_RT_BLOCK, c->list, 0, fs + FS_N_EDGES,
+        const unsigned rt_grid = (unsigned)((c->N / 16 + XB_RT_BLOCK - 1) / XB_RT_BLOCK);
+        if (bins)
+            launch_refine_trace<2, false, false, false, true>(c, (rt_grid + XB_RB_PARTS - 1) / XB_RB_PARTS * XB_RB_PARTS, XB_RT_BLOCK, c->list, 0, nullptr,
+                                                              fs + FS_CHANGED, fs + FS_ESCAPED, c->ovf_list, fs + FS_R_OVF, c->ovf_cap, brec, defer, fs + FS_R_DEFER,
+                                                              regions_ok, nullptr, wl, RetraceBins{bin_counts, fs + FS_BIN_OVF, fs + FS_N_EDGES, bin_cap});
+        else
+        launch_refine_trace<2, false>(c, rt_grid, XB_RT_BLOCK, c->list, 0, fs + FS_N_EDGES,
                                       fs + FS_CHANGED, fs + FS_ESCAPED, c->ovf_list, fs + FS_R_OVF, c->ovf_cap, brec, defer, fs + FS_R_DEFER,
                                       regions_ok, nullptr, wl);
         if (c->grad_cover == 1 && !regions_ok)
@@ -665,13 +683,22 @@
     }
     HIPCHK(hipGetLastError());
     int *hr = c->host_ints + HI_REFINE;
-    HIPCHK(hipMemcpyAsync(hr, fs + FS_N_EDGES, 7 * sizeof(int), hipMemcpyDeviceToHost, c->stream));
+    HIPCHK(hipMemcpyAsync(hr, fs + FS_N_EDGES, 8 * sizeof(int), hipMemcpyDeviceToHost, c->stream));
     HIPCHK(hipStreamSynchronize(c->stream));
     if (c->pending_assign && !assign_neargrid_complete(c, &c->pending_n_maxima)) return XB_STEP_REDO;
+    if (bins && hr[7]) {
+        c->stat_bin_redo++;
+        return refine_iteration_fused(c, edges, changed, late_records);
+    }
+    if (bins) c->stat_bin_steps++;
     *edges = hr[0];
     *changed = hr[1];
     const int novf = hr[3];
     if (novf == 0 && hr[1] > 0 && c->stage_bytes >= 8 * (size_t)c->N && hr[1] <= (int)std::min<long long>(c->N, 0x7fffffffLL)) {
+        if (bins)
+            k_list_changed<<<1024, TPB, 0, c->stream>>>(c->list, bin_counts, c->known, (int *)c->stage + c->N, fs + FS_N_CHGLIST,
+                                                        (int)std::min<long long>(c->N, 0x7fffffffLL), fs + FS_CHANGED, XB_RB_PARTS * XB_RB_BINS, bin_cap, CT_BIN_STRIDE);
+        else
         k_list_changed<<<1024, TPB, 0, c->stream>>>(c->list, fs + FS_N_EDGES, c->known, (int *)c->stage + c->N, fs + FS_N_CHGLIST,
                                                     (int)std::min<long long>(c->N, 0x7fffffffLL), fs + FS_CHANGED);
         HIPCHK(hipGetLastError());
@@ -776,6 +803,7 @@
         if (rc) { c->pending_assign = false; return rc; }
         rc = refine_impl(c, mode, iters, log, log_capacity, n_iters);
         c->chg_n = -1;
+        c->hint = nullptr;
         const bool redo = rc == XB_STEP_REDO || c->pending_assign;
         const bool arrived = rc == XB_STEP_REDO;
         c->pending_assign = false;
diff --git a/pybader_amd/csrc/host_stages.h b/pybader_amd/csrc/host_stages.h
--- a/pybader_amd/csrc/host_stages.h
+++ b/pybader_amd/csrc/host_stages.h
@@ -80,7 +80,8 @@
     if (wn > run1) k_brick_walk_list<<<grid, TPB, 0, c->stream>>>(nbr, 0, (wn - run1) * per_plane, c->blab, list, count, skip);
 }
 
-static bool launch_persistent_trace(xb_ctx *c, bool lean_ok, bool part, const int *box_max, const int *walk, int has_vacuum, int *bres) {
+static bool launch_persistent_trace(xb_ctx *c, bool lean_ok, bool part, const int *box_max, const int *walk, int has_vacuum, int *bres,
+                                    unsigned char *hint = nullptr) {
     const Grid &g = c->g;
     const int groups = std::max(1, c->trace_waves / XB_TRACE_WAVES);
     const int lean = lean_ok && light(g).use24 && c->opt_lean ? ((long long)g.wlen * g.nyz <= (1LL << 27) ? 4 : 3) : 0;
@@ -93,7 +94,7 @@
                 : (lean == 4 ? k_ng_trace_g<2, 4> : k_ng_trace_g<2, 3>);
     kernel<<<groups, XB_WAVE * XB_TRACE_WAVES, 0, c->stream>>>(light(g), c->grad, box_max, c->blab, c->nbk[1], c->nbk[2], walk, c->fs, c->labels,
                                                                c->first, c->max_list, c->max_cap, ovf, ovf_cap, trace_maxsteps(g), has_vacuum,
-                                                               8, 1, lean ? bres : nullptr);
+                                                               8, 1, lean ? bres : nullptr, lean ? hint : nullptr);
     if (window)
         k_ng_trace_list<2><<<512, TPB, 0, c->stream>>>(light(g), c->grad, box_max, c->blab, c->nbk[1], c->nbk[2], ovf, c->fs + FS_N_OVF, c->labels,
                                                        c->first, c->max_list, c->fs + FS_N_MAX, c->max_cap, c->ovf_list, c->counters + CT_N_OVF,
@@ -135,11 +136,11 @@
     if (n_maxima) *n_maxima = nmax;
 }
 
-extern "C++" template <int K, bool RHO, bool RESUME = false, bool EXPORT = false>
+extern "C++" template <int K, bool RHO, bool RESUME = false, bool EXPORT = false, bool BINS = false>
 static void launch_refine_trace(xb_ctx *c, unsigned grid, int block, const int *list, int n_host, const int *n_dev, int *changed, int *escaped,
                                 int *ovf_list, int *ovf_count, int ovf_cap, const unsigned char *brec, int *defer_list, int *defer_count,
-                                int regions_ok, const int *region_blab, const WalkerIO &wio) {
-    k_refine_trace<K, RHO, RESUME, EXPORT><<<grid, block, 0, c->stream>>>(light(c->g), c->grad, c->labels, c->known, list, n_host, n_dev, changed,
+                                int regions_ok, const int *region_blab, const WalkerIO &wio, const RetraceBins &rb = RetraceBins{}) {
+    k_refine_trace<K, RHO, RESUME, EXPORT, BINS><<<grid, block, 0, c->stream>>>(light(c->g), c->grad, c->labels, c->known, list, n_host, n_dev, changed,
                                                                            escaped, ovf_list, ovf_count, ovf_cap, trace_maxsteps(c->g), c->rho,
-                                                                           c->dist_dev, brec, defer_list, defer_count, regions_ok, region_blab, wio);
+                                                                           c->dist_dev, brec, defer_list, defer_count, regions_ok, region_blab, wio, rb);
 }
diff --git a/pybader_amd/csrc/k_edges.h b/pybader_amd/csrc/k_edges.h
--- a/pybader_amd/csrc/k_edges.h
+++ b/pybader_amd/csrc/k_edges.h
@@ -91,10 +91,11 @@
 }
 
 __global__ __launch_bounds__(TPB) void k_edge_dilate_list(GridL g, int8_t *known, const int *__restrict__ list, int n_host,
-                                                          const int *n_dev) {
-    const int n = n_dev ? *n_dev : n_host;
+                                                          const int *n_dev, int nseg = 1, int seg_cap = 0, int seg_stride = 0) {
+ for (int sg = 0; sg < nseg; sg++) {
+    const int n = n_dev ? n_dev[sg * seg_stride] : n_host;
   for (int t = blockIdx.x * TPB + threadIdx.x; t < n; t += gridDim.x * TPB) {
-    const int v = list[t];
+    const int v = list[(size_t)sg * seg_cap + t];
     const int x = v / g.nyz;
     const int r = v - x * g.nyz;
     const int y = r / g.nz, z = r - y * g.nz;
@@ -117,16 +118,28 @@
             if (k[j] >= 0) known[row[j / 3] + wrapi(z + j % 3 - 1, g.nz)] = -1;
     }
   }
+ }
 }
 
 #define ET_X 4
 #define ET_Y 8
 #define ET_Z 64
+struct EdgeBins {
+    const unsigned char *hint;
+    int *counts, *ovf;
+    int cap;
+};
+__device__ __forceinline__ int retrace_bin(int h) {
+    return (h >= 2) + (h >= 4) + (h >= 6) + (h >= 8) + (h >= 12) + (h >= 16) + (h >= 24);
+}
+static_assert(XB_RB_BINS == 8, "retrace_bin has seven thresholds");
+template <bool BINS = false>
 __device__ __forceinline__ void edge_tile(const GridL &g, const double *__restrict__ rho, const int *__restrict__ labels,
                                           int8_t *__restrict__ known, int xa, int nplanes, int *__restrict__ list,
                                           int *list_count, int small, const int *__restrict__ buni,
                                           const GradRec *__restrict__ G, const unsigned char *__restrict__ brick_rec,
-                                          int no_vacuum, int tx0, int y0, int z0, int salt = 0) {
+                                          int no_vacuum, int tx0, int y0, int z0, int salt = 0, const EdgeBins &eb = EdgeBins{},
+                                          int part = 0) {
     const int tid = (int)threadIdx.x + salt;
     __shared__ int tile[ET_X + 2][ET_Y + 2][ET_Z + 2];
     if (buni) {
@@ -177,6 +190,8 @@
         }
     }
     __shared__ unsigned char s_binfo[ET_X][ET_Z / 8];
+    __shared__ int s_bn[XB_RB_BINS], s_bb[XB_RB_BINS];
+    if (BINS && tid < XB_RB_BINS) s_bn[tid] = 0;
     {
         const int wv = __builtin_amdgcn_readfirstlane(tid / XB_WAVE), lane = tid % XB_WAVE;
         constexpr int NROW = (ET_X + 2) * (ET_Y + 2);
@@ -334,6 +349,35 @@
             known[v] = ((vac >> k) & 1u) ? 0 : (e ? -2 : 2);
             if (e && x >= g.x0 && x < g.x1) { vidx[k] = v; cnt++; }
         }
+    }
+    if (BINS) {
+        int slot[8];
+#pragma unroll
+        for (int k = 0; k < 8; k++) slot[k] = (vidx[k] >= 0 && (s_binfo[k >> 1][tz >> 3] & 1)) ? (int)eb.hint[vidx[k]] : 0;
+#pragma unroll
+        for (int k = 0; k < 8; k++)
+            if (vidx[k] >= 0) {
+                const int b = retrace_bin(slot[k]);
+                slot[k] = (atomicAdd(&s_bn[b], 1) << 3) | b;
+            }
+        __syncthreads();
+        if (tid < XB_RB_BINS) {
+            const int n = s_bn[tid];
+            int base = 0;
+            if (n) {
+                base = atomicAdd(eb.counts + (part * XB_RB_BINS + tid) * CT_BIN_STRIDE, n);
+                if (base + n > eb.cap) *eb.ovf = 1;
+            }
+            s_bb[tid] = base;
+        }
+        __syncthreads();
+#pragma unroll
+        for (int k = 0; k < 8; k++)
+            if (vidx[k] >= 0) {
+                const int b = slot[k] & 7, pos = s_bb[b] + (slot[k] >> 3);
+                if (pos < eb.cap) list[(size_t)(part * XB_RB_BINS + b) * eb.cap + pos] = vidx[k];
+            }
+        return;
     }
     int total;
     const int off = block_scan_excl(cnt, total);
@@ -431,11 +475,12 @@
     __syncthreads();
     if (hit) tiles[base_s + off] = (int)entry;
 }
+template <bool BINS = false>
 __global__ __launch_bounds__(TPB) void k_edge_flag_listed(GridL g, const double *__restrict__ rho, const int *__restrict__ labels,
                                                           int8_t *__restrict__ known, int *__restrict__ list, int *list_count,
                                                           int small, const GradRec *__restrict__ G,
                                                           const unsigned char *__restrict__ brick_rec, int no_vacuum,
-                                                          const int *__restrict__ tiles, const int *n_tiles) {
+                                                          const int *__restrict__ tiles, const int *n_tiles, EdgeBins eb = EdgeBins{}) {
     const int n = *n_tiles;
     const int ntz = (g.nz + ET_Z - 1) / ET_Z, nty = (g.ny + ET_Y - 1) / ET_Y;
     const int n_xcd = (gridDim.x % 8 == 0) ? 8 : 1;
@@ -455,22 +500,27 @@
         __syncthreads();
         int salt = 0;
         asm volatile("" : "+v"(salt));
-        edge_tile(g, rho, labels, known, 0, g.nx, list, list_count, small, nullptr, G, brick_rec, no_vacuum, tx0, y0, z0, salt);
+        edge_tile<BINS>(g, rho, labels, known, 0, g.nx, list, list_count, small, nullptr, G, brick_rec, no_vacuum, tx0, y0, z0, salt, eb,
+                        (int)(blockIdx.x % n_xcd));
     }
 }
 
 __global__ __launch_bounds__(TPB) void k_list_changed(const int *__restrict__ list, const int *n_dev, const int8_t *__restrict__ known,
-                                                      int *__restrict__ out, int *out_count, int out_cap, const int *n_changed) {
+                                                      int *__restrict__ out, int *out_count, int out_cap, const int *n_changed,
+                                                      int nseg = 1, int seg_cap = 0, int seg_stride = 0) {
     __shared__ int s_buf[BlockAppender<1>::CAP], s_n[2];
     if (*n_changed == 0) return;
     BlockAppender<1> app;
     app.init(s_buf, s_n, out, out_count, out_cap);
-    const int n = *n_dev;
-    for (int base = blockIdx.x * TPB; base < n; base += gridDim.x * TPB) {
-        const int t = base + threadIdx.x;
-        const int v = t < n ? list[t] : 0;
-        const bool hit = t < n && known[v] == -2;
-        app.add(hit ? 1 : 0, [&](int) { return v; });
+    for (int sg = 0; sg < nseg; sg++) {
+        const int n = n_dev[sg * seg_stride];
+        const int *seg = list + (size_t)sg * seg_cap;
+        for (int base = blockIdx.x * TPB; base < n; base += gridDim.x * TPB) {
+            const int t = base + threadIdx.x;
+            const int v = t < n ? seg[t] : 0;
+            const bool hit = t < n && known[v] == -2;
+            app.add(hit ? 1 : 0, [&](int) { return v; });
+        }
     }
     app.finish();
 }
@@ -555,7 +605,12 @@
 };
 #define XB_WALKER_STUCK (-2147483647 - 1)
 
-template <int K, bool RHO, bool RESUME = false, bool EXPORT = false>
+struct RetraceBins {
+    const int *counts, *ovf;
+    int *n_total;
+    int cap;
+};
+template <int K, bool RHO, bool RESUME = false, bool EXPORT = false, bool BINS = false>
 __global__ __launch_bounds__(TPB) void k_refine_trace(GridL g, const GradRec *__restrict__ G, int *labels,
                                                       int8_t *known, const int *__restrict__ list, int n_host,
                                                       const int *n_dev, int *changed, int *escaped, int *ovf_list,
@@ -563,15 +618,46 @@
                                                       const double *__restrict__ rho, const double *__restrict__ gc,
                                                       const unsigned char *__restrict__ brick_rec, int *defer_list,
                                                       int *defer_count, int regions_ok, const int *__restrict__ region_blab,
-                                                      WalkerIO wio) {
+                                                      WalkerIO wio, RetraceBins rb = RetraceBins{}) {
     static_assert(!RESUME || (RHO && K == 2), "walkers are carried on by the from-rho kernel");
-    const int n = n_dev ? *n_dev : n_host;
+    static_assert(!BINS || (!RHO && !RESUME && !EXPORT), "the hinted sub-lists are the lean one-GPU kernel's");
+    int n = 0;
+    XcdRange xr;
+    const int *part_counts = nullptr;
+    if (BINS) {
+        if (*rb.ovf) return;
+        if (blockIdx.x == gridDim.x - 1 && threadIdx.x == 0) {
+            int sum = 0;
+            for (int s = 0; s < XB_RB_PARTS * XB_RB_BINS; s++) sum += rb.counts[s * CT_BIN_STRIDE];
+            *rb.n_total = sum;
+        }
+        part_counts = rb.counts + (int)(blockIdx.x % XB_RB_PARTS) * (XB_RB_BINS * CT_BIN_STRIDE);
+#pragma unroll
+        for (int b = 0; b < XB_RB_BINS; b++) n += part_counts[b * CT_BIN_STRIDE];
+        xr.begin = (int)(blockIdx.x / XB_RB_PARTS);
+        xr.end = (n + (int)blockDim.x - 1) / (int)blockDim.x;
+        xr.step = (int)(gridDim.x / XB_RB_PARTS);
+    } else {
+        n = n_dev ? *n_dev : n_host;
+        xr = xcd_range((n + (int)blockDim.x - 1) / (int)blockDim.x);
+    }
     int n_ch = 0, n_es = 0;
-  const XcdRange xr = xcd_range((n + (int)blockDim.x - 1) / (int)blockDim.x);
   for (int chunk = xr.begin; chunk < xr.end; chunk += xr.step) {
     const int t = chunk * (int)blockDim.x + threadIdx.x;
     bool valid = t < n;
-    int v = (valid && !RESUME) ? list[t] : 0;
+    int v = 0;
+    if (BINS) {
+        int idx = -1, rem = t;
+#pragma unroll
+        for (int b = XB_RB_BINS - 1; b >= 0; b--) {
+            const int nb = part_counts[b * CT_BIN_STRIDE];
+            if ((unsigned)rem < (unsigned)nb) idx = ((int)(blockIdx.x % XB_RB_PARTS) * XB_RB_BINS + b) * rb.cap + rem;
+            rem -= nb;
+        }
+        valid = idx >= 0;
+        if (valid) v = list[idx];
+    } else
+        v = (valid && !RESUME) ? list[t] : 0;
     bool moving = false;
     int result = -3;
     int px = 0, py = 0, pz = 0, lp = 0, steps = 0, vol_num = 0;
diff --git a/pybader_amd/csrc/k_fused.h b/pybader_amd/csrc/k_fused.h
--- a/pybader_amd/csrc/k_fused.h
+++ b/pybader_amd/csrc/k_fused.h
@@ -21,6 +21,7 @@
     FS_R_DEFER,
     FS_N_TILES,
     FS_N_CHGLIST,
+    FS_BIN_OVF,
     FS_GROW_RETRY,
     FS_N_RECL,
     FS_N_REDO,
@@ -61,8 +62,13 @@
     CT_EC_NEXT = 26,
     CT_EC_DONE = 27,
     CT_COUNT = 28,
-    CT_FS = 128
+    CT_FS = 128,
+    CT_BINS = 3072, CT_BIN_STRIDE = 32,
+    CT_TOTAL = CT_BINS + 8 * 8 * CT_BIN_STRIDE
 };
+#define XB_RB_PARTS 8
+#define XB_RB_BINS 8
+static_assert(CT_TOTAL == CT_BINS + XB_RB_PARTS * XB_RB_BINS * CT_BIN_STRIDE, "one length per sub-list");
 static_assert(CT_COUNT <= CT_FS, "fs lies behind the counters");
 #define CT_INTS(first, last) ((last) - (first) + 1)
 static_assert(CT_ESCAPED == CT_CHANGED + 1 && CT_WALK_RES == CT_WALK_OUT + 1 && CT_WALK_STUCK == CT_WALK_CHANGED + 1 &&
@@ -256,6 +262,7 @@
 }
 #define XB_SORT_MAX 2048
 static_assert(FS_TOTAL + XB_SORT_MAX <= HI_REFINE && HI_UPLOAD < HI_TOTAL, "host_ints: the far corners lie behind an assignment's block");
+static_assert(CT_FS + FS_TOTAL + XB_SORT_MAX <= CT_BINS, "the sub-list lengths lie behind fs and the sorted maxima");
 __global__ __launch_bounds__(1024) void k_number_maxima(int *fs, int *first, const int *__restrict__ max_list, int max_cap,
                                                         int *sorted, int *sorted2 = nullptr) {
     __shared__ unsigned long long key[XB_SORT_MAX];
diff --git a/pybader_amd/csrc/k_trace.h b/pybader_amd/csrc/k_trace.h
--- a/pybader_amd/csrc/k_trace.h
+++ b/pybader_amd/csrc/k_trace.h
@@ -247,7 +247,8 @@
 __device__ __forceinline__ int ng_walk_lean(const GridL &g, const GradRec *__restrict__ G, const int *__restrict__ box_max,
                                              const int *__restrict__ blab, int nb1, int nb2, int sx, int sy, int sz,
                                              int *labels, int *first, int *max_list, int *max_count, int max_cap,
-                                             int *ovf_list, int *ovf_count, int ovf_cap, int maxsteps, bool has_vacuum) {
+                                             int *ovf_list, int *ovf_count, int ovf_cap, int maxsteps, bool has_vacuum,
+                                             unsigned char *__restrict__ hint = nullptr) {
     const int v = lin24(g, sx, sy, sz);
     const int lab0 = has_vacuum ? labels[v] : 0;
     const int ox8 = sx & ~7, oy8 = sy & ~7, oz8 = sz & ~7;
@@ -312,6 +313,7 @@
 #ifdef XB_DEBUG_COUNT
     if (xb_dbg_steps) xb_dbg_steps[v] = (signed char)min(dbg_lane_steps, 127);
 #endif
+    if (hint) hint[v] = (unsigned char)(result == -2 ? 255 : min(steps, 255));
     if (has_vacuum && result >= 0 && result != v && labels[result] == -1) result = -1;
     labels[v] = result;
     note_maximum_wave(result >= 0, result, v, first, max_list, max_count, max_cap);
@@ -397,7 +399,8 @@
                                                        const int *__restrict__ blab, int nb1, int nb2,
                                                        const int *__restrict__ walk, int *fs, int *labels, int *first,
                                                        int *max_list, int max_cap, int *ovf_list, int ovf_cap, int maxsteps,
-                                                       int has_vacuum, int CH, int xcd_split, int *__restrict__ bres = nullptr) {
+                                                       int has_vacuum, int CH, int xcd_split, int *__restrict__ bres = nullptr,
+                                                       unsigned char *__restrict__ hint = nullptr) {
     __shared__ int s_base, s_next;
     __shared__ int s_w[8], s_mixed;
     constexpr bool CACHE = LEAN >= 3;
@@ -480,7 +483,7 @@
                     const long long pr_c = clock64();
 #endif
                     const int res = ng_walk_lean<LEAN == 4, CACHE, WINDOW>(g, G, box_max, blab, nb1, nb2, sx, sy, sz, labels, first, max_list, &fs[FS_N_MAX],
-                                                                max_cap, ovf_list, &fs[FS_N_OVF], ovf_cap, maxsteps, has_vacuum != 0);
+                                                                max_cap, ovf_list, &fs[FS_N_OVF], ovf_cap, maxsteps, has_vacuum != 0, hint);
 #ifdef XB_DEBUG_COUNT
                     pr_walk += clock64() - pr_c;
 #endif
```

Measured after the change: 41170 Mvoxels/s. 0.967x the previous value.
